# cgbur/llama2.zig

Hardware: AMD Instinct MI355X
Metric: tokens/s (argmax, -t 0) (higher is better)
Workload: dtype f32; 1 GPU; llama2-7b shape, fp32 llama2.c-v0 checkpoint (dim 4096, hidden 11008, L 32, H 32, kv 32, V 32000, S 2048), greedy from BOS, seeded synthetic weights; parallelism=1 GPU

## Files before the change

llama2.zig_amd/csrc/forward.cpp:

```cpp
#include <algorithm>
#include <cmath>
#include <cstdlib>
#include <cstring>
#include <mutex>

#include "batch_host.h"
#include "l2z_state.h"

namespace l2z {

struct Prof {
    std::vector<hipEvent_t> ev;
    std::vector<int> kind;
};

#define L2Z_LAUNCH(kind_id, expr)                                                         \
    do {                                                                                  \
        hipEvent_t _a = nullptr, _b = nullptr;                                            \
        if (prof) {                                                                       \
            L2Z_HIP(hipEventCreate(&_a));                                                 \
            L2Z_HIP(hipEventCreate(&_b));                                                 \
            L2Z_HIP(hipEventRecord(_a, st));                                              \
        }                                                                                 \
        L2Z_HIP(expr);                                                                    \
        if (prof) {                                                                       \
            L2Z_HIP(hipEventRecord(_b, st));                                              \
            prof->ev.push_back(_a);                                                       \
            prof->ev.push_back(_b);                                                       \
            prof->kind.push_back(kind_id);                                                \
        }                                                                                 \
    } while (0)

int check_pair(const l2z_config *config, const l2z_runstate *s, const l2z_weights *w, bool paged_ok, bool q8_ok)
{
    L2Z_CHECK(config && s && w, L2Z_ERR_INVALID, "null config / runstate / weights");
    L2Z_CHECK(q8_ok || !w->is_q8(), L2Z_ERR_INVALID,
              "int8 group-quantized weights (l2z_weights_init_q8) are taken by the single-sequence decode only: "
              "l2z_transformer, l2z_greedy_run, l2z_sample_run, l2z_time_kind, l2z_profile_forward");
    L2Z_CHECK(!w->is_q8() || (s->comm == nullptr && s->sh.world == 1), L2Z_ERR_INVALID,
              "int8 group-quantized weights are unsharded: the runstate belongs to a shard group");
    L2Z_CHECK(paged_ok || s->pool == nullptr, L2Z_ERR_INVALID,
              "a paged runstate (l2z_runstate_init_paged) is taken by the wide family only: l2z_prefill_batch, "
              "l2z_transformer_wide, l2z_wide_run, l2z_verify_wide");
    L2Z_CHECK(memcmp(config, &s->cfg, sizeof *config) == 0 &&
                  memcmp(config, &w->cfg, sizeof *config) == 0,
              L2Z_ERR_INVALID, "config does not match the one RunState / Weights were built with");
    L2Z_CHECK(s->device == w->device && s->sh.rank == w->sh.rank && s->sh.world == w->sh.world,
              L2Z_ERR_INVALID, "RunState and Weights live on different devices / shards");
    L2Z_CHECK(s->sh.scheme_b == w->sh.scheme_b, L2Z_ERR_INVALID,
              "RunState and Weights were built under different sharding schemes (L2Z_SCHEME_B changed in between)");
    return L2Z_OK;
}

namespace {

hipError_t set_state(l2z_runstate *s, const l2z_weights *w, int token, int pos)
{
    if (w->is_q8()) return launch_set_state_q8(token, pos, s->d_token, s->d_pos, w->q8_emb(), s->x, s->cfg.dim, s->stream);
    return launch_set_state(token, pos, s->d_token, s->d_pos, w->tok_emb, s->x, s->cfg.dim, s->stream);
}

int enqueue_forward_q8(l2z_runstate *s, const l2z_weights *w, StepKind step, Prof *prof, int only_stage, int variant,
                       int only_kind)
{
    L2Z_CHECK(only_stage < 0 && s->sh.world == 1, L2Z_ERR_INVALID, "int8 group-quantized weights: unsharded passes only");
    const bool with_step = step != STEP_NONE;
    const bool split = variant == ATTN_SPLIT || variant == ATTN_SPLIT_S;
    const l2z_config &c = s->cfg;
    const Shard &sh = s->sh;
    hipStream_t st = s->stream;
    const size_t dim = c.dim, hid = c.hidden_dim, kvd = sh.kvd_loc;
    const int mb = s->max_blocks, gs = w->q8_gs;
    const size_t gd = dim / gs, gh = hid / gs;
    auto kind = [&](int k) { return only_kind < 0 || only_kind == k; };
    for (int l = 0; l < c.n_layers; l++) {
        float *kc = s->key_cache + (size_t)l * c.seq_len * kvd;
        float *vc = s->value_cache + (size_t)l * c.seq_len * kvd;
        const size_t kvh_stride = (size_t)c.seq_len * sh.hs;
        if (kind(KIND_QKV)) {
            Q8MatvecArgs a = {};
            a.gs = gs;
            a.q0 = w->q_wq.q + (size_t)l * dim * dim; a.s0 = w->q_wq.s + (size_t)l * dim * gd;
            a.q1 = w->q_wk.q + (size_t)l * kvd * dim; a.s1 = w->q_wk.s + (size_t)l * kvd * gd;
            a.q2 = w->q_wv.q + (size_t)l * kvd * dim; a.s2 = w->q_wv.s + (size_t)l * kvd * gd;
            a.b.out0 = s->q; a.b.out1 = kc; a.b.out2 = vc;
            a.b.rows0 = c.dim; a.b.rows1 = sh.kvd_loc; a.b.rows2 = sh.kvd_loc;
            a.b.pos_stride1 = sh.hs; a.b.pos_stride2 = sh.hs; a.b.kv_head_stride = kvh_stride;
            a.b.n = c.dim; a.b.x = s->x; a.b.rms_w = w->rms_att + (size_t)l * dim;
            a.b.pos_ptr = s->d_pos; a.b.rope = s->rope; a.b.head_size = sh.hs; a.b.rope_segs = 2;
            L2Z_LAUNCH(KIND_QKV, launch_q8_matvec(a, EPI_ROPE, mb, g_cus, st));
        }
        if (kind(KIND_ATTN)) {
            AttnArgs a = {};
            a.q = s->q; a.kcache = kc; a.vcache = vc; a.xb = s->xb;
            a.pos_ptr = s->d_pos; a.head_size = sh.hs; a.kv_row = sh.hs; a.kv_head = kvh_stride;
            a.kv_mul = c.n_heads / c.n_kv_heads; a.seq_len = c.seq_len;
            a.tl_seq = s->tl_attn_seq++;
            if (split && s->attn_nch > 1 && attention_split_supported(a))
                L2Z_LAUNCH(KIND_ATTN, launch_attention_split(a, sh.heads_loc, s->attn_nch, s->d_attn_part, s->d_attn_cnt, st,
                                                             variant == ATTN_SPLIT_S));
            else
                L2Z_LAUNCH(KIND_ATTN, launch_attention(a, sh.heads_loc, st, variant == ATTN_SHORT ? 1 : 0));
        }
        if (kind(KIND_WO)) {
            Q8MatvecArgs a = {};
            a.gs = gs;
            a.q0 = w->q_wo.q + (size_t)l * dim * dim; a.s0 = w->q_wo.s + (size_t)l * dim * gd;
            a.b.out0 = s->x; a.b.resid = s->x; a.b.rows0 = c.dim; a.b.n = c.dim; a.b.x = s->xb;
            L2Z_LAUNCH(KIND_WO, launch_q8_matvec(a, EPI_RESID, mb, g_cus, st));
        }
        if (kind(KIND_FFN13)) {
            Q8MatvecArgs a = {};
            a.gs = gs;
            a.q0 = w->q_w13.q + (size_t)l * 2 * hid * dim; a.s0 = w->q_w13.s + (size_t)l * 2 * hid * gd;
            a.b.out0 = s->hb; a.b.rows0 = c.hidden_dim; a.b.rows1 = c.hidden_dim; a.b.n = c.dim; a.b.x = s->x;
            a.b.rms_w = w->rms_ffn + (size_t)l * dim;
            L2Z_LAUNCH(KIND_FFN13, launch_q8_matvec(a, EPI_SWIGLU, mb, g_cus, st));
        }
        if (kind(KIND_FFN2)) {
            Q8MatvecArgs a = {};
            a.gs = gs;
            a.q0 = w->q_w2.q + (size_t)l * dim * hid; a.s0 = w->q_w2.s + (size_t)l * dim * gh;
            a.b.out0 = s->x; a.b.resid = s->x; a.b.rows0 = c.dim; a.b.n = c.hidden_dim; a.b.x = s->hb;
            L2Z_LAUNCH(KIND_FFN2, launch_q8_matvec(a, EPI_RESID, mb, g_cus, st));
        }
    }
    if (kind(KIND_CLS)) {
        Q8MatvecArgs a = {};
        a.gs = gs;
        a.q0 = w->q_cls.q; a.s0 = w->q_cls.s;
        a.b.out0 = s->logits; a.b.rows0 = c.vocab_size; a.b.n = c.dim; a.b.x = s->x; a.b.rms_w = w->rms_final;
        a.b.part_val = s->d_part_val; a.b.part_idx = s->d_part_idx;
        int grid = 0;
        L2Z_LAUNCH(KIND_CLS, launch_q8_matvec(a, EPI_ARGMAX, mb, g_cus, st, &grid));
        s->n_part = grid;
        if (only_kind < 0) (with_step ? s->n_part_step : s->n_part_fwd) = s->n_part;
    }
    if (step == STEP_GREEDY && kind(KIND_ARGMAX)) {
        ArgmaxArgs a = {};
        a.logits = s->logits; a.vocab = c.vocab_size; a.token_ptr = s->d_token;
        if (s->n_part > 0) { a.part_val = s->d_part_val; a.part_idx = s->d_part_idx; a.n_part = s->n_part; }
        a.pos_ptr = s->d_pos; a.prompt = s->d_prompt; a.n_prompt_ptr = s->d_n_prompt;
        a.out_tokens = s->d_out_tokens; a.argmax_out = s->d_argmax; a.emb_q8 = w->q8_emb();
        a.x = s->x; a.dim = c.dim; a.advance = 1;
        L2Z_LAUNCH(KIND_ARGMAX, launch_argmax(a, st));
    }
    if (step == STEP_SAMPLE && kind(KIND_ARGMAX)) {
        L2Z_CHECK(s->d_smp_ctl != nullptr && s->d_smp_scratch != nullptr, L2Z_ERR_STATE,
                  "sampled step on a runstate l2z_sample_run has not prepared");
        SampleStepArgs a = {};
        a.logits = s->logits; a.vocab = c.vocab_size; a.seq_len = c.seq_len;
        a.params = (const SampleStepParams *)s->d_smp_ctl; a.coins = s->d_smp_ctl + 2; a.scratch = s->d_smp_scratch;
        a.token_ptr = s->d_token; a.pos_ptr = s->d_pos; a.prompt = s->d_prompt; a.n_prompt_ptr = s->d_n_prompt;
        a.out_tokens = s->d_out_tokens; a.emb_q8 = w->q8_emb(); a.x = s->x; a.dim = c.dim;
        L2Z_LAUNCH(KIND_ARGMAX, launch_sample_step(a, st));
    }
    return L2Z_OK;
}

}

int enqueue_forward(l2z_runstate *s, const l2z_weights *w, StepKind step, Prof *prof,
                    int only_stage, int variant, int only_kind)
{
    if (w->is_q8()) return enqueue_forward_q8(s, w, step, prof, only_stage, variant, only_kind);
    const bool with_step = step != STEP_NONE;
    const bool split = variant == ATTN_SPLIT || variant == ATTN_SPLIT_S;
    const l2z_config &c = s->cfg;
    const Shard &sh = s->sh;
    hipStream_t st = s->stream;
    const l2z_comm *lc = s->comm;
    const size_t dim = c.dim, hid = c.hidden_dim;
    const int mb = s->max_blocks;
    int stage = 0;
    auto want = [&]() { return only_stage < 0 || only_stage == stage; };
    auto kind = [&](int k) { return only_kind < 0 || only_kind == k; };
    const bool p2p = s->d_push != nullptr && only_stage < 0 && sh.world > 1;
    const bool consume = p2p && s->ll_consume;
    const bool can_push = p2p && consume;
    const bool sb = sh.scheme_b;
    const bool xchg = step == STEP_GREEDY && p2p && s->xchg_steps;
    const int n_g = s->n_gathers;
    int gi = 0;
    bool pushed = false;
    const int *ctl = lc ? lc->d_ctl : nullptr;
    auto gather = [&](float *buf, size_t count_per_rank) -> int {
        stage++;
        gi++;
        if (only_stage >= 0 || only_kind >= 0) return L2Z_OK;
        const bool was_pushed = pushed;
        pushed = false;
        if (consume) {
            L2Z_CHECK(was_pushed, L2Z_ERR_STATE, "consumer-side gather %d: the producer did not push", gi);
            if (gi < n_g) return L2Z_OK;
        }
        hipEvent_t ea = nullptr, eb = nullptr;
        const bool timed = prof != nullptr && s->comm != nullptr && s->comm->world > 1;
        if (timed) {
            L2Z_HIP(hipEventCreate(&ea));
            L2Z_HIP(hipEventCreate(&eb));
            L2Z_HIP(hipEventRecord(ea, st));
        }
        L2Z_TRY(comm_allgather_inplace(s->comm, buf, count_per_rank, gi, n_g, was_pushed, st));
        if (timed) {
            L2Z_HIP(hipEventRecord(eb, st));
            prof->ev.push_back(ea);
            prof->ev.push_back(eb);
            prof->kind.push_back(KIND_GATHER);
        }
        return L2Z_OK;
    };
    auto reduce = [&]() -> int {
        stage++;
        gi++;
        if (only_stage >= 0 || only_kind >= 0) return L2Z_OK;
        const bool was_pushed = pushed;
        pushed = false;
        hipEvent_t ea = nullptr, eb = nullptr;
        if (prof != nullptr) {
            L2Z_HIP(hipEventCreate(&ea));
            L2Z_HIP(hipEventCreate(&eb));
            L2Z_HIP(hipEventRecord(ea, st));
        }
        L2Z_TRY(comm_allreduce(s->comm, s->part, s->x, dim, gi, was_pushed, st));
        if (prof != nullptr) {
            L2Z_HIP(hipEventRecord(eb, st));
            prof->ev.push_back(ea);
            prof->ev.push_back(eb);
            prof->kind.push_back(KIND_GATHER);
        }
        return L2Z_OK;
    };
    auto x_in = [&](MatvecArgs &a, const float *plain, int g, size_t count_per_rank) {
        a.x = plain;
        if (consume && g >= 1) a.xin = comm_ll_in(s->comm, g, count_per_rank);
    };
    auto push_to = [&](MatvecArgs &a, int which) {
        if (!can_push) return;
        a.push = s->d_push + which;
        a.push_ctl = ctl;
        a.push_gi = comm_gi(lc, gi + 1);
    };
    auto col_shard = [&](MatvecArgs &a, const float *wcols, const float *x_loc, int n_pad, int *epi) {
        a.w0 = wcols;
        a.x = x_loc;
        a.n = n_pad;
        a.rows0 = c.dim;
        a.out0 = s->part;
        a.resid = sh.rank == 0 ? s->x : nullptr;
        *epi = sh.rank == 0 ? EPI_RESID : EPI_STORE;
        push_to(a, 1);
    };
    const bool pk = s->packed_w && !sb && sh.world == 1 && !consume;
    const auto pk_slot = [&](int k, int l, int j = 0) -> const l2z_weights::PkMat * {
        return pk && ((s->packed_kinds >> k) & 1) ? w->pk_slot(k, l, j) : nullptr;
    };
    for (int l = 0; l < c.n_layers; l++) {
        float *kc = s->key_cache + (size_t)l * c.seq_len * sh.kvd_loc;
        float *vc = s->value_cache + (size_t)l * c.seq_len * sh.kvd_loc;
        const size_t kvh_stride = (size_t)c.seq_len * sh.hs;
        const bool fused = s->fused_qkv_attn && !split && only_stage < 0;
        if (fused && kind(KIND_QKV)) {
            FusedQkvAttnArgs a = {};
            a.wq = w->wq + (size_t)l * dim * dim;
            a.wk = w->wk + (size_t)l * dim * dim;
            a.wv = w->wv + (size_t)l * dim * dim;
            a.rms_w = w->rms_att + (size_t)l * dim; a.x = s->x; a.q_out = s->q;
            a.kcache = kc; a.vcache = vc; a.xb = s->xb; a.pos_ptr = s->d_pos; a.rope = s->rope;
            a.n = c.dim; a.head_size = sh.hs; a.seq_len = c.seq_len; a.kv_dim = sh.kvd_loc;
            a.kv_row = sh.hs; a.kv_head = kvh_stride;
            L2Z_LAUNCH(KIND_QKV, launch_fused_qkv_attn(a, c.n_heads, st));
        }
        if (!fused && want() && kind(KIND_QKV)) {
            MatvecArgs a = {};
            a.w0 = w->wq + (size_t)l * sh.dim_loc * dim;
            a.w1 = w->wk + (size_t)l * sh.kvd_loc * dim;
            a.w2 = w->wv + (size_t)l * sh.kvd_loc * dim;
            a.out0 = s->q; a.out1 = kc; a.out2 = vc;
            a.rows0 = sh.dim_loc; a.rows1 = sh.kvd_loc; a.rows2 = sh.kvd_loc;
            a.pos_stride1 = sh.hs; a.pos_stride2 = sh.hs; a.kv_head_stride = kvh_stride;
            a.n = c.dim; a.rms_w = w->rms_att + (size_t)l * dim;
            x_in(a, s->x, gi, sh.dim_loc);
            a.pos_ptr = s->d_pos; a.rope = s->rope; a.head_size = sh.hs; a.rope_segs = 2;
            const auto *pq = pk_slot(KIND_QKV, l, 0), *pkk = pk_slot(KIND_QKV, l, 1), *pv = pk_slot(KIND_QKV, l, 2);
            if (pq && pkk && pv) {
                a.pk = pq->p; a.pk_e = pq->e;
                a.pk1 = pkk->p; a.pk_e1 = pkk->e;
                a.pk2 = pv->p; a.pk_e2 = pv->e;
            }
            L2Z_LAUNCH(KIND_QKV, launch_matvec(a, PRO_RMS, EPI_ROPE, mb, g_cus, st));
        }
        if (!fused && want() && kind(KIND_ATTN)) {
            AttnArgs a = {};
            a.q = s->q; a.kcache = kc; a.vcache = vc; a.xb = s->xb + sh.dim0;
            a.pos_ptr = s->d_pos; a.head_size = sh.hs; a.kv_row = sh.hs; a.kv_head = kvh_stride;
            a.kv_mul = c.n_heads / c.n_kv_heads; a.seq_len = c.seq_len;
            a.tl_seq = s->tl_attn_seq++;
            if (!sb && can_push && attention_push_supported(a)) {
                a.push = s->d_push + 0;
                a.push_ctl = ctl;
                a.push_gi = comm_gi(lc, gi + 1);
                pushed = true;
            }
            if (split && s->attn_nch > 1 && attention_split_supported(a))
                L2Z_LAUNCH(KIND_ATTN, launch_attention_split(a, sh.heads_loc, s->attn_nch,
                                                             s->d_attn_part, s->d_attn_cnt, st, variant == ATTN_SPLIT_S));
            else
                L2Z_LAUNCH(KIND_ATTN, launch_attention(a, sh.heads_loc, st, variant == ATTN_SHORT ? 1 : 0));
        }
        if (!sb) L2Z_TRY(gather(s->xb, sh.dim_loc));
        if (want() && kind(KIND_WO)) {
            MatvecArgs a = {};
            int epi = EPI_RESID;
            if (sb) {
                col_shard(a, w->wo + (size_t)l * dim * sh.dimc_pad, s->xb + sh.dim0, sh.dimc_pad, &epi);
            } else {
                a.w0 = w->wo + (size_t)l * sh.dim_loc * dim;
                a.out0 = s->x + sh.dim0; a.resid = s->x + sh.dim0;
                a.rows0 = sh.dim_loc; a.n = c.dim;
                x_in(a, s->xb, gi, sh.dim_loc);
                push_to(a, 1);
                if (const auto *p = pk_slot(KIND_WO, l)) { a.pk = p->p; a.pk_e = p->e; }
            }
            L2Z_LAUNCH(KIND_WO, launch_matvec(a, PRO_NONE, epi, mb, g_cus, st, nullptr, &pushed));
        }
        if (sb) L2Z_TRY(reduce());
        else L2Z_TRY(gather(s->x, sh.dim_loc));
        if (want() && kind(KIND_FFN13)) {
            MatvecArgs a = {};
            a.w0 = w->w1 + (size_t)l * sh.hid_loc * 2 * dim;
            a.w1 = w->w3 + (size_t)l * sh.hid_loc * 2 * dim;
            a.out0 = sb ? s->hb : s->hb + sh.hid0;
            a.rows0 = sh.hid_loc; a.rows1 = sh.hid_loc; a.n = c.dim;
            a.rms_w = w->rms_ffn + (size_t)l * dim;
            x_in(a, s->x, gi, sh.dim_loc);
            if (!sb) push_to(a, 2);
            if (const auto *p = pk_slot(KIND_FFN13, l)) { a.pk = p->p; a.pk_e = p->e; }
            L2Z_LAUNCH(KIND_FFN13, launch_matvec(a, PRO_RMS, EPI_SWIGLU, mb, g_cus, st, nullptr, &pushed));
        }
        if (!sb) L2Z_TRY(gather(s->hb, sh.hid_loc));
        if (want() && kind(KIND_FFN2)) {
            MatvecArgs a = {};
            int epi = EPI_RESID;
            if (sb) {
                col_shard(a, w->w2 + (size_t)l * dim * sh.hidc_pad, s->hb, sh.hidc_pad, &epi);
            } else {
                a.w0 = w->w2 + (size_t)l * sh.dim_loc * hid;
                a.out0 = s->x + sh.dim0; a.resid = s->x + sh.dim0;
                a.rows0 = sh.dim_loc; a.n = c.hidden_dim;
                x_in(a, s->hb, gi, sh.hid_loc);
                push_to(a, 1);
                if (const auto *p = pk_slot(KIND_FFN2, l)) { a.pk = p->p; a.pk_e = p->e; }
            }
            L2Z_LAUNCH(KIND_FFN2, launch_matvec(a, PRO_NONE, epi, mb, g_cus, st, nullptr, &pushed));
        }
        if (sb) L2Z_TRY(reduce());
        else L2Z_TRY(gather(s->x, sh.dim_loc));
    }
    if (want() && kind(KIND_CLS)) {
        MatvecArgs a = {};
        a.w0 = w->wcls; a.out0 = s->logits + sh.v0;
        a.rows0 = sh.v_loc; a.n = c.dim; a.rms_w = w->rms_final;
        x_in(a, s->x, gi, sh.dim_loc);
        a.part_val = s->d_part_val; a.part_idx = s->d_part_idx; a.row_offset = sh.v0;
        const bool fuse = (sh.world == 1 || xchg || (only_kind >= 0 && with_step && s->comm && !s->comm->nccl && !s->comm->p2p)) &&
                          matvec_vector_width(c.dim);
        int grid = 0;
        if (!xchg) push_to(a, 3);
        if (const auto *p = fuse ? pk_slot(KIND_CLS, 0) : nullptr) { a.pk = p->p; a.pk_e = p->e; }
        L2Z_LAUNCH(KIND_CLS, launch_matvec(a, PRO_RMS, fuse ? EPI_ARGMAX : EPI_STORE, mb, g_cus, st,
                                           &grid, &pushed));
        s->n_part = fuse ? grid : 0;
        if (only_stage < 0 && only_kind < 0) (with_step ? s->n_part_step : s->n_part_fwd) = s->n_part;
    }
    if (xchg) {
        stage++;
        gi++;
        pushed = false;
        if (only_kind < 0) s->logits_partial = true;
    } else {
        L2Z_TRY(gather(s->logits, sh.v_loc));
    }
    if (step == STEP_GREEDY && want() && kind(KIND_ARGMAX)) {
        ArgmaxArgs a = {};
        a.logits = s->logits; a.vocab = c.vocab_size; a.token_ptr = s->d_token;
        if (s->n_part > 0) { a.part_val = s->d_part_val; a.part_idx = s->d_part_idx; a.n_part = s->n_part; }
        a.pos_ptr = s->d_pos; a.prompt = s->d_prompt; a.n_prompt_ptr = s->d_n_prompt;
        a.out_tokens = s->d_out_tokens; a.argmax_out = s->d_argmax; a.tok_emb = w->tok_emb;
        a.x = s->x; a.dim = c.dim; a.advance = 1;
        if (xchg && only_kind < 0) {
            a.xchg = s->d_push + 3;
            a.xchg_gi = comm_gi(lc, n_g);
            a.epoch_ctl = lc->d_ctl;
            a.epoch_add = lc->solo ? 0 : n_g;
        }
        L2Z_LAUNCH(KIND_ARGMAX, launch_argmax(a, st));
    }
    if (step == STEP_SAMPLE && want() && kind(KIND_ARGMAX)) {
        L2Z_CHECK(sh.world == 1 && s->d_smp_ctl != nullptr && s->d_smp_scratch != nullptr, L2Z_ERR_STATE,
                  "sampled step on a runstate l2z_sample_run has not prepared");
        SampleStepArgs a = {};
        a.logits = s->logits; a.vocab = c.vocab_size; a.seq_len = c.seq_len;
        a.params = (const SampleStepParams *)s->d_smp_ctl; a.coins = s->d_smp_ctl + 2; a.scratch = s->d_smp_scratch;
        a.token_ptr = s->d_token; a.pos_ptr = s->d_pos; a.prompt = s->d_prompt; a.n_prompt_ptr = s->d_n_prompt;
        a.out_tokens = s->d_out_tokens; a.tok_emb = w->tok_emb; a.x = s->x; a.dim = c.dim;
        L2Z_LAUNCH(KIND_ARGMAX, launch_sample_step(a, st));
    }
    return L2Z_OK;
}

int attn_variant(const l2z_runstate *s, int pos)
{
    if (s->attn_nch > 1 && pos >= s->attn_split_pos) return pos < s->attn_split_wide_pos ? ATTN_SPLIT_S : ATTN_SPLIT;
    return pos < s->attn_short_pos ? ATTN_SHORT : ATTN_HEAD;
}

int build_graph(l2z_runstate *s, const l2z_weights *w, StepKind step, int variant,
                hipGraphExec_t *out)
{
    hipGraph_t graph = nullptr;
    L2Z_HIP(hipStreamBeginCapture(s->stream, hipStreamCaptureModeThreadLocal));
    int rc = enqueue_forward(s, w, step, nullptr, -1, variant);
    hipError_t e = hipStreamEndCapture(s->stream, &graph);
    if (rc != L2Z_OK) {
        if (graph) (void)hipGraphDestroy(graph);
        return rc;
    }
    L2Z_HIP(e);
    e = hipGraphInstantiate(out, graph, nullptr, nullptr, 0);
    (void)hipGraphDestroy(graph);
    L2Z_HIP(e);
    return L2Z_OK;
}

void drop_graphs(l2z_runstate *s)
{
    for (int v = 0; v < ATTN_VARIANTS; v++) {
        if (s->g_forward[v]) { (void)hipGraphExecDestroy(s->g_forward[v]); s->g_forward[v] = nullptr; }
        if (s->g_step[v]) { (void)hipGraphExecDestroy(s->g_step[v]); s->g_step[v] = nullptr; }
        if (s->g_sample[v]) { (void)hipGraphExecDestroy(s->g_sample[v]); s->g_sample[v] = nullptr; }
    }
    s->graph_w_uid = 0;
}

hipGraphExec_t *graph_slot(l2z_runstate *s, StepKind step, int variant)
{
    return step == STEP_SAMPLE ? &s->g_sample[variant] : step == STEP_GREEDY ? &s->g_step[variant] : &s->g_forward[variant];
}

int ensure_graph(l2z_runstate *s, const l2z_weights *w, int variant, StepKind step)
{
    if (!s->use_graphs) return L2Z_OK;
    int rc = L2Z_OK;
    if (s->graph_w_uid != w->uid) {
        drop_graphs(s);
        s->graph_w_uid = w->uid;
        const int edges[] = {0, s->attn_short_pos, s->attn_split_pos, s->attn_split_wide_pos, s->cfg.seq_len};
        bool reach[ATTN_VARIANTS] = {};
        for (int e : edges)
            for (int p = e - 1; p <= e; p++)
                if (p >= 0 && p < s->cfg.seq_len) reach[attn_variant(s, p)] = true;
        for (int v = 0; v < ATTN_VARIANTS && rc == L2Z_OK; v++) {
            if (!reach[v]) continue;
            rc = build_graph(s, w, STEP_NONE, v, &s->g_forward[v]);
            if (rc == L2Z_OK) rc = build_graph(s, w, STEP_GREEDY, v, &s->g_step[v]);
        }
    }
    hipGraphExec_t *slot = graph_slot(s, step, variant);
    if (rc == L2Z_OK && *slot) return L2Z_OK;
    if (rc != L2Z_OK || build_graph(s, w, step, variant, slot) != L2Z_OK) {
        fprintf(stderr, "llama2_hip: hipGraph capture failed (%s); launching eagerly\n", l2z_last_error());
        drop_graphs(s);
        s->use_graphs = false;
        (void)hipGetLastError();
    }
    return L2Z_OK;
}

int run_forward(l2z_runstate *s, const l2z_weights *w, StepKind step, int pos)
{
    const bool with_step = step != STEP_NONE;
    const int variant = attn_variant(s, pos);
    L2Z_CHECK(s->sh.world == 1 || (s->comm && (s->comm->nccl || s->comm->p2p)), L2Z_ERR_STATE,
              "sharded runstate without a transport: connect the group (RCCL id or "
              "l2z_comm_p2p_export/_connect), or drive emulated ranks with l2z_emu_transformer");
    L2Z_TRY(comm_check(s->comm));
    L2Z_TRY(ensure_graph(s, w, variant, step));
    s->logits_partial = step == STEP_GREEDY && s->xchg_steps && s->d_push != nullptr && s->sh.world > 1;
    if (s->use_graphs) {
        s->n_part = with_step ? s->n_part_step : s->n_part_fwd;
        L2Z_HIP(hipGraphLaunch(*graph_slot(s, step, variant), s->stream));
        return L2Z_OK;
    }
    return enqueue_forward(s, w, step, nullptr, -1, variant);
}

int ensure_logits(l2z_runstate *s)
{
    if (!s->logits_partial) return L2Z_OK;
    L2Z_TRY(comm_allgather_inplace(s->comm, s->logits, (size_t)s->sh.v_loc, 1, 1, false, s->stream));
    s->logits_partial = false;
    s->n_part = 0;
    return L2Z_OK;
}


}

using namespace l2z;

extern "C" int l2z_transformer(int token, int pos, const l2z_config *config, l2z_runstate *s,
                               const l2z_weights *w)
{
    L2Z_TRY(check_pair(config, s, w, false, true));
    L2Z_CHECK(token >= 0 && token < config->vocab_size, L2Z_ERR_STATE, "token %d out of range", token);
    L2Z_CHECK(pos >= 0 && pos < config->seq_len, L2Z_ERR_STATE, "pos %d out of range [0,%d)", pos,
              config->seq_len);
    L2Z_HIP(hipSetDevice(s->device));
    L2Z_HIP(set_state(s, w, token, pos));
    L2Z_TRY(run_forward(s, w, STEP_NONE, pos));
    s->host_pos = pos + 1;
    return L2Z_OK;
}

extern "C" int l2z_argmax(l2z_runstate *s, int *out_token)
{
    L2Z_CHECK(s && out_token, L2Z_ERR_INVALID, "l2z_argmax: null argument");
    L2Z_HIP(hipSetDevice(s->device));
    L2Z_TRY(ensure_logits(s));
    ArgmaxArgs a = {};
    a.logits = s->logits; a.vocab = s->cfg.vocab_size; a.argmax_out = s->d_argmax; a.advance = 0;
    if (s->n_part > 0) { a.part_val = s->d_part_val; a.part_idx = s->d_part_idx; a.n_part = s->n_part; }
    L2Z_HIP(launch_argmax(a, s->stream));
    L2Z_HIP(hipMemcpyAsync(out_token, s->d_argmax, sizeof(int), hipMemcpyDeviceToHost, s->stream));
    L2Z_HIP(hipStreamSynchronize(s->stream));
    return L2Z_OK;
}

extern "C" int l2z_logits_read(l2z_runstate *s, float *out_logits)
{
    L2Z_CHECK(s && out_logits, L2Z_ERR_INVALID, "l2z_logits_read: null argument");
    L2Z_HIP(hipSetDevice(s->device));
    L2Z_TRY(ensure_logits(s));
    L2Z_HIP(hipMemcpyAsync(out_logits, s->logits, (size_t)s->cfg.vocab_size * sizeof(float),
                           hipMemcpyDeviceToHost, s->stream));
    L2Z_HIP(hipStreamSynchronize(s->stream));
    L2Z_TRY(comm_check(s->comm));
    return L2Z_OK;
}

extern "C" int l2z_probs_read(l2z_runstate *s, float temperature, float *out_probs)
{
    L2Z_CHECK(s && out_probs, L2Z_ERR_INVALID, "l2z_probs_read: null argument");
    L2Z_CHECK(temperature > 0.0f, L2Z_ERR_INVALID, "l2z_probs_read: temperature %g (0 is the argmax path)", (double)temperature);
    L2Z_HIP(hipSetDevice(s->device));
    L2Z_TRY(ensure_logits(s));
    if (s->d_probs == nullptr) L2Z_HIP(hipMalloc(&s->d_probs, (size_t)s->cfg.vocab_size * sizeof(float)));
    L2Z_HIP(launch_probs(s->d_probs, s->logits, s->cfg.vocab_size, temperature, s->stream));
    const size_t bytes = (size_t)s->cfg.vocab_size * sizeof(float);
    if (s->h_stage == nullptr) L2Z_HIP(hipHostMalloc((void **)&s->h_stage, bytes, hipHostMallocDefault));
    L2Z_HIP(hipMemcpyAsync(s->h_stage, s->d_probs, bytes, hipMemcpyDeviceToHost, s->stream));
    L2Z_HIP(hipStreamSynchronize(s->stream));
    L2Z_TRY(comm_check(s->comm));
    memcpy(out_probs, s->h_stage, bytes);
    return L2Z_OK;
}

extern "C" int l2z_greedy_begin(l2z_runstate *s, const int32_t *prompt, int n_prompt)
{
    L2Z_CHECK(s != nullptr && n_prompt >= 0 && (n_prompt == 0 || prompt != nullptr),
              L2Z_ERR_INVALID, "l2z_greedy_begin: bad arguments");
    L2Z_CHECK(n_prompt <= s->cfg.seq_len, L2Z_ERR_INVALID, "prompt longer than seq_len");
    L2Z_CHECK(s->pool == nullptr, L2Z_ERR_INVALID, "l2z_greedy_begin: a paged runstate is taken by the wide family only");
    for (int i = 0; i < n_prompt; i++)
        L2Z_CHECK(prompt[i] >= 0 && prompt[i] < s->cfg.vocab_size, L2Z_ERR_INVALID,
                  "prompt[%d] = %d out of vocabulary", i, prompt[i]);
    L2Z_HIP(hipSetDevice(s->device));
    L2Z_HIP(hipStreamSynchronize(s->stream));
    if (n_prompt)
        L2Z_HIP(hipMemcpy(s->d_prompt, prompt, (size_t)n_prompt * sizeof(int), hipMemcpyHostToDevice));
    L2Z_HIP(hipMemcpy(s->d_n_prompt, &n_prompt, sizeof(int), hipMemcpyHostToDevice));
    s->h_prompt.assign(prompt, prompt + n_prompt);
    s->host_pos = 0;
    s->done = false;
    return L2Z_OK;
}

namespace l2z {
namespace {

int step_loop(const l2z_config *config, l2z_runstate *s, const l2z_weights *w, int n_steps, StepKind step,
              int32_t *out_tokens, int *out_n)
{
    *out_n = 0;
    L2Z_HIP(hipSetDevice(s->device));
    if (s->done) return L2Z_OK;
    int remaining = n_steps;
    if (remaining > config->seq_len - s->host_pos) remaining = config->seq_len - s->host_pos;
    if (remaining <= 0) return L2Z_OK;
    if (s->host_pos == 0) {
        L2Z_HIP(set_state(s, w, 1, 0));
    }
    const int kChunk = 64;
    int produced = 0;
    const int np = (int)s->h_prompt.size();
    if (s->host_pos == 0 && np >= kPrefillMinPrompt && remaining >= np && prefill_enabled() && !w->is_q8() &&
        prefill_usable(s) &&
        std::find(s->h_prompt.begin(), s->h_prompt.end(), 1) == s->h_prompt.end()) {
        std::vector<int32_t> in((size_t)np);
        in[0] = 1;
        for (int i = 1; i < np; i++) in[(size_t)i] = s->h_prompt[(size_t)i - 1];
        L2Z_TRY(prefill_tokens(s, w, in.data(), np, 0));
        L2Z_HIP(hipMemcpyAsync(s->d_out_tokens, s->d_prompt, (size_t)np * sizeof(int),
                               hipMemcpyDeviceToDevice, s->stream));
        L2Z_HIP(launch_set_state(s->h_prompt[(size_t)np - 1], np, s->d_token, s->d_pos, w->tok_emb,
                                 s->x, config->dim, s->stream));
        for (int i = 0; i < np; i++) out_tokens[i] = s->h_prompt[(size_t)i];
        produced = np;
        s->host_pos = np;
        remaining -= np;
    }
    while (remaining > 0 && !s->done) {
        const int n = remaining < kChunk ? remaining : kChunk;
        for (int i = 0; i < n; i++) L2Z_TRY(run_forward(s, w, step, s->host_pos + i));
        L2Z_HIP(hipMemcpyAsync(out_tokens + produced, s->d_out_tokens + s->host_pos,
                               (size_t)n * sizeof(int), hipMemcpyDeviceToHost, s->stream));
        L2Z_HIP(hipStreamSynchronize(s->stream));
        L2Z_TRY(comm_check(s->comm));
        int got = n;
        for (int i = 0; i < n; i++) {
            if (out_tokens[produced + i] == 1) {
                got = i + 1;
                s->done = true;
                break;
            }
        }
        produced += got;
        s->host_pos += got;
        remaining -= n;
    }
    *out_n = produced;
    return L2Z_OK;
}

}
}

extern "C" int l2z_greedy_run(const l2z_config *config, l2z_runstate *s, const l2z_weights *w,
                              int n_steps, int32_t *out_tokens, int *out_n)
{
    L2Z_TRY(check_pair(config, s, w, false, true));
    L2Z_CHECK(out_tokens && out_n && n_steps >= 0, L2Z_ERR_INVALID, "l2z_greedy_run: bad arguments");
    return step_loop(config, s, w, n_steps, STEP_GREEDY, out_tokens, out_n);
}

extern "C" int l2z_sample_run(const l2z_config *config, l2z_runstate *s, const l2z_weights *w, int n_steps,
                              float temperature, float top_p, const float *coins, int32_t *out_tokens, int *out_n)
{
    L2Z_TRY(no_device_check());
    L2Z_CHECK(out_tokens && out_n && n_steps >= 0, L2Z_ERR_INVALID, "l2z_sample_run: bad arguments");
    L2Z_TRY(check_pair(config, s, w, false, true));
    L2Z_CHECK(s->comm == nullptr && s->sh.world == 1, L2Z_ERR_INVALID,
              "l2z_sample_run: the runstate is a shard (a shard holds its own rows of the logits only)");
    L2Z_TRY(check_draw("l2z_sample_run", -1, temperature, top_p, coins));
    if (temperature > 0.0f) L2Z_TRY(check_coins("l2z_sample_run", coins, 0, n_steps));
    *out_n = 0;
    const int left = config->seq_len - s->host_pos;
    const int n = n_steps < left ? n_steps : left;
    if (s->done || n <= 0) return L2Z_OK;
    L2Z_HIP(hipSetDevice(s->device));
    const size_t ctl_bytes = (2 + (size_t)config->seq_len) * sizeof(float);
    if (s->d_smp_ctl == nullptr) {
        L2Z_HIP(hipMalloc((void **)&s->d_smp_ctl, ctl_bytes));
        L2Z_HIP(hipMemset(s->d_smp_ctl, 0, ctl_bytes));
    }
    if (s->h_smp_ctl == nullptr) L2Z_HIP(hipHostMalloc((void **)&s->h_smp_ctl, ctl_bytes, hipHostMallocDefault));
    if (s->d_smp_scratch == nullptr)
        L2Z_HIP(hipMalloc((void **)&s->d_smp_scratch, sample_scratch_floats(config->vocab_size) * sizeof(float)));
    s->h_smp_ctl[0] = temperature;
    s->h_smp_ctl[1] = top_p;
    L2Z_HIP(hipMemcpyAsync(s->d_smp_ctl, s->h_smp_ctl, 2 * sizeof(float), hipMemcpyHostToDevice, s->stream));
    if (temperature > 0.0f) {
        float *h = s->h_smp_ctl + 2 + s->host_pos;
        memcpy(h, coins, (size_t)n * sizeof(float));
        L2Z_HIP(hipMemcpyAsync(s->d_smp_ctl + 2 + s->host_pos, h, (size_t)n * sizeof(float), hipMemcpyHostToDevice, s->stream));
    }
    return step_loop(config, s, w, n_steps, STEP_SAMPLE, out_tokens, out_n);
}

extern "C" int l2z_profile_forward(int token, int pos, const l2z_config *config, l2z_runstate *s,
                                   const l2z_weights *w, double *ms_by_kind, int *launches_by_kind,
                                   int n_kinds)
{
    L2Z_TRY(check_pair(config, s, w, false, true));
    L2Z_CHECK(ms_by_kind && launches_by_kind && n_kinds >= KIND_COUNT, L2Z_ERR_INVALID,
              "l2z_profile_forward: need %d kind slots", (int)KIND_COUNT);
    L2Z_CHECK(token >= 0 && token < config->vocab_size && pos >= 0 && pos < config->seq_len,
              L2Z_ERR_STATE, "token/pos out of range");
    L2Z_HIP(hipSetDevice(s->device));
    L2Z_HIP(set_state(s, w, token, pos));
    Prof prof;
    int rc = enqueue_forward(s, w, STEP_GREEDY, &prof, -1, attn_variant(s, pos));
    hipError_t e = hipStreamSynchronize(s->stream);
    for (int k = 0; k < n_kinds; k++) { ms_by_kind[k] = 0.0; launches_by_kind[k] = 0; }
    if (rc == L2Z_OK && e == hipSuccess) {
        for (size_t i = 0; i < prof.kind.size(); i++) {
            float ms = 0.0f;
            if (hipEventElapsedTime(&ms, prof.ev[2 * i], prof.ev[2 * i + 1]) == hipSuccess) {
                ms_by_kind[prof.kind[i]] += ms;
                launches_by_kind[prof.kind[i]] += 1;
            }
        }
    }
    for (hipEvent_t ev : prof.ev) (void)hipEventDestroy(ev);
    s->host_pos = pos + 1;
    if (rc != L2Z_OK) return rc;
    L2Z_HIP(e);
    return L2Z_OK;
}

extern "C" int l2z_time_kind(int kind, int pos, const l2z_config *config, l2z_runstate *s,
                             const l2z_weights *w, int reps, double *avg_ms_per_launch, int *launches)
{
    L2Z_TRY(check_pair(config, s, w, false, true));
    L2Z_CHECK(kind >= 0 && kind < KIND_GATHER && avg_ms_per_launch && reps >= 1, L2Z_ERR_INVALID,
              "l2z_time_kind: bad arguments");
    L2Z_CHECK(s->sh.world == 1 || (s->comm && ((!s->comm->nccl && !s->comm->p2p) || s->comm->solo)), L2Z_ERR_INVALID,
              "l2z_time_kind: unsharded runstates, emulated or solo ranks only (a connected shard would wait for its peers)");
    L2Z_CHECK(pos >= 0 && pos < config->seq_len, L2Z_ERR_STATE, "pos out of range");
    L2Z_HIP(hipSetDevice(s->device));
    L2Z_HIP(set_state(s, w, 1, pos));
    hipEvent_t e0, e1;
    L2Z_HIP(hipEventCreate(&e0));
    L2Z_HIP(hipEventCreate(&e1));
    const int per_pass = kind == KIND_CLS || kind == KIND_ARGMAX ? 1 : config->n_layers;
    int rc = enqueue_forward(s, w, STEP_GREEDY, nullptr, -1, attn_variant(s, pos), kind);
    hipError_t e = hipEventRecord(e0, s->stream);
    for (int r = 0; r < reps && rc == L2Z_OK; r++) rc = enqueue_forward(s, w, STEP_GREEDY, nullptr, -1, attn_variant(s, pos), kind);
    if (e == hipSuccess) e = hipEventRecord(e1, s->stream);
    if (e == hipSuccess) e = hipEventSynchronize(e1);
    float ms = 0.0f;
    if (e == hipSuccess) e = hipEventElapsedTime(&ms, e0, e1);
    (void)hipEventDestroy(e0);
    (void)hipEventDestroy(e1);
    hipError_t e2 = set_state(s, w, 1, pos);
    if (e2 == hipSuccess) e2 = hipStreamSynchronize(s->stream);
    if (rc != L2Z_OK) return rc;
    L2Z_HIP(e);
    L2Z_HIP(e2);
    *avg_ms_per_launch = (double)ms / (double)(reps * per_pass);
    if (launches) *launches = reps * per_pass;
    return L2Z_OK;
}

extern "C" int l2z_emu_transformer(int n_ranks, l2z_runstate *const *ss,
                                   const l2z_weights *const *ws, int token, int pos)
{
    L2Z_CHECK(n_ranks >= 1 && ss && ws, L2Z_ERR_INVALID, "l2z_emu_transformer: bad arguments");
    const l2z_config &c = ss[0]->cfg;
    for (int r = 0; r < n_ranks; r++) {
        L2Z_TRY(check_pair(&c, ss[r], ws[r]));
        L2Z_CHECK(ss[r]->sh.world == n_ranks && ss[r]->sh.rank == r, L2Z_ERR_INVALID,
                  "l2z_emu_transformer: runstate %d is not rank %d of %d", r, r, n_ranks);
        L2Z_HIP(launch_set_state(token, pos, ss[r]->d_token, ss[r]->d_pos, ws[r]->tok_emb, ss[r]->x,
                                 c.dim, ss[r]->stream));
    }
    const bool sb = ss[0]->sh.scheme_b;
    const int n_stages = (sb ? 2 : 4) * c.n_layers + 1;
    for (int stage = 0; stage < n_stages; stage++) {
        for (int r = 0; r < n_ranks; r++)
            L2Z_TRY(enqueue_forward(ss[r], ws[r], STEP_NONE, nullptr, stage, attn_variant(ss[r], pos)));
        for (int r = 0; r < n_ranks; r++) L2Z_HIP(hipStreamSynchronize(ss[r]->stream));
        if (sb && stage < n_stages - 1) {
            const float *parts[kMaxWorld];
            L2Z_CHECK(n_ranks <= kMaxWorld, L2Z_ERR_INVALID, "l2z_emu_transformer: more than %d ranks", kMaxWorld);
            for (int r = 0; r < n_ranks; r++) parts[r] = ss[r]->part;
            for (int r = 0; r < n_ranks; r++) L2Z_HIP(launch_sum_parts(ss[r]->x, parts, n_ranks, c.dim, nullptr));
            L2Z_HIP(hipDeviceSynchronize());
            continue;
        }
        const Shard &sh0 = ss[0]->sh;
        size_t count;
        int which;
        if (stage == n_stages - 1) { which = 3; count = sh0.v_loc; }
        else if (stage % 4 == 0) { which = 0; count = sh0.dim_loc; }
        else if (stage % 4 == 2) { which = 2; count = sh0.hid_loc; }
        else { which = 1; count = sh0.dim_loc; }
        auto buf = [&](l2z_runstate *s) {
            return which == 0 ? s->xb : which == 1 ? s->x : which == 2 ? s->hb : s->logits;
        };
        for (int src = 0; src < n_ranks; src++)
            for (int dst = 0; dst < n_ranks; dst++)
                if (dst != src)
                    L2Z_HIP(hipMemcpy(buf(ss[dst]) + (size_t)src * count,
                                      buf(ss[src]) + (size_t)src * count, count * sizeof(float),
                                      hipMemcpyDeviceToDevice));
        L2Z_HIP(hipDeviceSynchronize());
    }
    for (int r = 0; r < n_ranks; r++) ss[r]->host_pos = pos + 1;
    return L2Z_OK;
}

extern "C" int l2z_kind_name(int kind, char *out, size_t cap)
{
    L2Z_CHECK(kind >= 0 && kind < KIND_COUNT && out && cap, L2Z_ERR_INVALID, "l2z_kind_name: bad kind");
    snprintf(out, cap, "%s", kKindNames[kind]);
    return L2Z_OK;
}
```

llama2.zig_amd/csrc/l2z_internal.h:

```cpp
#pragma once

#include <hip/hip_runtime.h>

#include <cstdarg>
#include <cstdint>
#include <cstdio>
#include <string>
#include <vector>

#include "../../include/llama2_hip.h"
#include "../../include/llama2_hip_test.h"

namespace l2z {

struct P2pArgs;

struct LLIn {
    const unsigned long long *slots;
    unsigned slot_floats;
    unsigned count;
    int gi;
    int *ctl;
    int *h_err;
    long long timeout_ticks;
};

void set_error(const char *fmt, ...);

#define L2Z_HIP(expr)                                                                    \
    do {                                                                                 \
        hipError_t _e = (expr);                                                          \
        if (_e != hipSuccess) {                                                          \
            ::l2z::set_error("%s failed: %s (%s:%d)", #expr, hipGetErrorString(_e),      \
                             __FILE__, __LINE__);                                        \
            return _e == hipErrorOutOfMemory ? L2Z_ERR_OOM                               \
                   : (_e == hipErrorNoDevice || _e == hipErrorInvalidDevice)             \
                       ? L2Z_ERR_NO_DEVICE                                               \
                       : L2Z_ERR_HIP;                                                    \
        }                                                                                \
    } while (0)

#define L2Z_CHECK(cond, code, ...)          \
    do {                                    \
        if (!(cond)) {                      \
            ::l2z::set_error(__VA_ARGS__);  \
            return (code);                  \
        }                                   \
    } while (0)

#define L2Z_TRY(expr)              \
    do {                           \
        int _s = (expr);           \
        if (_s != L2Z_OK) return _s; \
    } while (0)

template <class Sig> class FnRef;
template <class R, class... Args> class FnRef<R(Args...)> {
  public:
    template <class F>
    FnRef(const F &f) : f_(&f), call_([](const void *p, Args... args) -> R { return (*(const F *)p)(args...); }) {}
    R operator()(Args... args) const { return call_(f_, args...); }

  private:
    const void *f_;
    R (*call_)(const void *, Args...);
};


enum Prologue { PRO_NONE = 0, PRO_RMS = 1 };
enum Epilogue { EPI_STORE = 0, EPI_ROPE = 1, EPI_RESID = 2, EPI_SWIGLU = 3, EPI_ARGMAX = 4 };

constexpr int kMaxSeg = 3;

struct Q8Emb {
    const int8_t *q;
    const float *s;
    int gs;
};

struct ArgmaxArgs {
    const float *logits;
    int vocab;
    const float *part_val;
    const int *part_idx;
    int n_part;
    int *token_ptr;
    int *pos_ptr;
    const int *prompt;
    const int *n_prompt_ptr;
    int *out_tokens;
    int *argmax_out;
    const float *tok_emb;
    float *x;
    int dim;
    Q8Emb emb_q8;
    int advance;
    int *epoch_ctl;
    int epoch_add;
    const P2pArgs *xchg;
    int xchg_gi;
};

struct MatvecArgs {
    const float *w0, *w1, *w2;
    float *out0, *out1, *out2;
    int rows0, rows1, rows2;
    int pos_stride1, pos_stride2;
    size_t kv_head_stride;
    int n;
    const float *x;
    const float *rms_w;
    const float *resid;
    const int *pos_ptr;
    const float2 *rope;
    int head_size;
    int rope_segs;
    float *part_val;
    int *part_idx;
    int row_offset;
    const P2pArgs *push;
    const int *push_ctl;
    int push_gi;
    LLIn xin;
    const uint32_t *pk, *pk1, *pk2;
    int pk_e, pk_e1, pk_e2;
    int tl_slot;
};

struct Q8MatvecArgs {
    MatvecArgs b;
    const int8_t *q0, *q1, *q2;
    const float *s0, *s1, *s2;
    int gs;
    const int8_t *xq;
    const float *xs;
};
hipError_t launch_q8_matvec(const Q8MatvecArgs &a, int epi, int max_blocks_per_cu, int n_cus, hipStream_t st,
                            int *out_grid = nullptr);
hipError_t launch_q8_quantize(const float *src, size_t count, int gs, bool weight_rule, int8_t *q, float *s, hipStream_t st);
hipError_t launch_set_state_q8(int token, int pos, int *token_ptr, int *pos_ptr, const Q8Emb &emb, float *x, int dim,
                               hipStream_t st);

struct AttnArgs {
    const float *q;
    const float *kcache;
    const float *vcache;
    float *xb;
    const int *pos_ptr;
    int head_size;
    int kv_row;
    size_t kv_head;
    int kv_mul;
    int seq_len;
    const P2pArgs *push;
    const int *push_ctl;
    int push_gi;
    int tl_seq;
};


struct FusedQkvAttnArgs {
    const float *wq, *wk, *wv;
    const float *rms_w, *x;
    float *q_out;
    float *kcache, *vcache;
    float *xb;
    const int *pos_ptr;
    const float2 *rope;
    int n;
    int head_size, seq_len, kv_dim;
    int kv_row;
    size_t kv_head;
};
bool fused_qkv_attn_supported(int dim, int n_heads, int n_kv_heads, int seq_len, int n_cus);
hipError_t launch_fused_qkv_attn(const FusedQkvAttnArgs &a, int n_heads, hipStream_t st);

hipError_t launch_pk_stats(const float *m, size_t count, uint32_t *stats, hipStream_t st);
hipError_t launch_pk_pack(const float *m, int rows, int n, int e_base, uint32_t *pk, hipStream_t st);
hipError_t launch_pk_unpack(const uint32_t *pk, int rows, int n, int e_base, float *out, hipStream_t st);
hipError_t launch_matvec(const MatvecArgs &a, int pro, int epi, int max_blocks_per_cu, int n_cus,
                         hipStream_t st, int *out_grid = nullptr, bool *pushed = nullptr);
bool attention_push_supported(const AttnArgs &a);
int matvec_max_grid(int n_cus);
bool matvec_vector_width(int n);
hipError_t launch_stream_read(const float *p, size_t n_floats, float *out, int n_cus, hipStream_t st);
hipError_t launch_attention(const AttnArgs &a, int n_heads_local, hipStream_t st, int form = 0);
int attention_short_pos(int head_size, int seq_len);
int attention_split_chunks(int n_heads_local, int n_cus);
size_t attention_split_part_floats(int n_heads_local, int head_size, int nch);
bool attention_split_supported(const AttnArgs &a);
hipError_t launch_attention_split(const AttnArgs &a, int n_heads_local, int nch, float *part,
                                  int *arrivals, hipStream_t st, bool small = false);
int attention_split_wide_pos(int seq_len);
hipError_t launch_argmax(const ArgmaxArgs &a, hipStream_t st);
hipError_t launch_set_state(int token, int pos, int *token_ptr, int *pos_ptr, const float *tok_emb,
                            float *x, int dim, hipStream_t st);
hipError_t launch_rmsnorm(float *o, const float *x, const float *w, int n, hipStream_t st);
hipError_t launch_softmax(float *x, int n, hipStream_t st);
hipError_t launch_probs(float *probs, const float *logits, int n, float temperature, hipStream_t st);
hipError_t launch_dot(float *out, const float *x, const float *y, int n, hipStream_t st);
hipError_t launch_weighted_sum_rows(float *xout, int xout_len, const float *rows, int row_stride,
                                    const float *weights, int n_weights, hipStream_t st);
hipError_t launch_synth_fill(float *dst, uint64_t base_idx, uint64_t count, uint64_t seed,
                             float scale, float bias, hipStream_t st, uint64_t row_len = 0, uint64_t row_pitch = 0,
                             uint64_t idx_pitch = 0);
hipError_t launch_sum_parts(float *out, const float *const *parts, int n_parts, int n, hipStream_t st);
hipError_t launch_copy_rows(float *dst, size_t dpitch, const float *src, size_t rows, size_t cols, hipStream_t st);
size_t attention_lds_bytes(int head_size, int seq_len, bool vec);

struct SplitKWs {
    float *part;
    int *cnt;
    size_t part_floats;
    int cnt_ints;
    void *x3;
    size_t x3_bytes;
    void *x3b;
    size_t x3b_bytes;
};
struct DeferredSum {
    const float *part;
    int sk, feat, tm;
    bool valid;
};
enum PlanesReady { PLANES_SPLIT = 0, PLANES_READY = 1, PLANES_READY_B = 2 };
constexpr int kSplitKMaxTokens = 256;
constexpr int kPanelWsRows = 6 * kSplitKMaxTokens;
int prefill_split_k(long long n_whole, int P, int K, bool pair);
enum PrefillGemmEpi { PG_STORE = 0, PG_RESID = 1, PG_ROPE = 2, PG_ROPE_CACHE = 3, PG_CACHE = 4,
                      PG_SWIGLU = 5 };
bool x3_applies(long long n_whole, int K);
bool x3_stream_shape(long long n_whole, int P, int K);
int x3_stream_sk(long long n_whole, int P, int K);
enum GemmKind { GEMM_SINGLE = 0,
                GEMM_QKV,
                GEMM_W13,
                GEMM_KV };
struct GemmShape {
    int kind, epi;
    int P, N, K, ldx;
    int n_scale;
    long long n_launch_whole;
    int sk;
    int nq, nkv;
    int w13_one_matrix;
    size_t part_floats;
    int cnt_ints;
};
enum GemmFamily { GF_INVALID = -1, GF_NOT_SUPPORTED = -2, GF_NO_WORKSPACE = -3,
                  GF_STREAM = 1,
                  GF_SHORT,
                  GF_SPLIT_K,
                  GF_TWO_BLOCK,
                  GF_TILE };
enum TileForm { TILE_128x64 = 0, TILE_64x64, TILE_32x64, TILE_32x32, TILE_128x128 };
struct GemmPlan {
    int family;
    int epi;
    int K;
    int x3;
    int sk;
    int tile;
    int feat, tm, nbuf, one_round;
    int tms, paired;
};
GemmPlan prefill_gemm_plan(const GemmShape &s);
hipError_t launch_prefill_rmsnorm(float *o, int ldo, const float *x, const float *w, int n, int P,
                                  hipStream_t st,
                                  void *x3 = nullptr, int kp = 0,
                                  const DeferredSum *pending = nullptr,
                                  const int *rows = nullptr);
hipError_t launch_prefill_embed(float *x, const float *tok_emb, const int *tokens, int dim, int P,
                                hipStream_t st);
hipError_t launch_prefill_attention(const float *q, int ldq, const float *kcache, const float *vcache,
                                    float *out, int ldo, int pos0, int P, int n_heads, int head_size,
                                    int kv_row, size_t kv_head, int kv_mul, int seq_len, hipStream_t st,
                                    int n_heads_model = 0,
                                    int form = 0,
                                    void *x3 = nullptr, int kp = 0,
                                    bool *planes_written = nullptr);
constexpr int kRaggedMaxSeq = 16;
struct RaggedSeq {
    float *kc, *vc;
    int row0, rows;
    int pos0;
    int pad;
    const int32_t *pages;
};
__device__ __forceinline__ int kv_page_id(const int32_t *pages, int i)
{
    return ((const __attribute__((address_space(4))) int32_t *)pages)[i];
}
struct RaggedLayer {
    const float *q;
    int ldq;
    float *out;
    int ldo;
    int P, n_heads, head_size, kv_mul, seq_len;
    size_t layer_off, kv_head_stride;
    hipStream_t st;
    void *x3;
    int kp;
};
using RaggedAttention = FnRef<hipError_t(const RaggedLayer &, bool *planes_written)>;
struct RaggedChunk {
    const RaggedSeq *seq;
    const int *row_seq;
    const int *row_pos;
    const int2 *tiles;
    int n_seq, n_tiles;
    int seq_max;
    float *k, *v;
    size_t page_floats;
    const RaggedAttention *attention;
    const int *att_rows;
    int n_att_rows;
};
hipError_t launch_ragged_rope_scatter(float *q, int ldq, const RaggedChunk &rg, int P, int dim, int kv_dim, int head_size,
                                      const float2 *rope, size_t layer_off, size_t kv_head_stride, hipStream_t st);
hipError_t launch_ragged_attention(const RaggedLayer &L, const RaggedChunk &rg, bool *planes_written = nullptr);
enum PanelEpi { PANEL_STORE = 0, PANEL_RESID = 1, PANEL_SWIGLU = 2, PANEL_QKV = 3 };
struct PanelProduct {
    const float *x;
    int ldx;
    const float *w0, *w1, *w2;
    int rows0, rows1, rows2;
    int P, K;
    int mode;
    float *out;
    int ldo;
    const float *res;
    int ldres;
    float *outk, *outv;
    int ldkv, head_size, pos0;
    size_t kv_head_stride;
    const float2 *rope;
};
bool prefill_panel_shape(long long n_whole, int P, int K, long long widest_whole);
int prefill_panel_max_tokens();
int prefill_next_chunk_of(const l2z_config &c, int remaining);
hipError_t launch_prefill_panel(const PanelProduct &p, int n_cus, const SplitKWs *ws, hipStream_t st);
int prefill_tile_form(int N, int P, int pair);
constexpr int kScoreSeg = 4096;
struct ScoreArgs {
    const float *slab;
    int ld, n, col0, P;
    const int *targets;
    float *part_m, *part_s;
    int *part_i;
    float *tgt;
    int seg0, nseg;
    float *out_logprob;
    int *out_top1;
};
hipError_t launch_score_reduce(const ScoreArgs &a, hipStream_t st);
hipError_t launch_score_finish(const ScoreArgs &a, hipStream_t st);
size_t matvec_lds_bytes(int n);

}
```

llama2.zig_amd/csrc/l2z_state.h:

```cpp
#pragma once
#include <cstdint>
#include <vector>

#include "kv_pages.h"
#include "l2z_comm.h"
#include "l2z_internal.h"
#include "tunables.h"

namespace l2z {

struct BatchScratch;
struct WideScratch;

struct Shard {
    int rank = 0, world = 1;
    int hs = 0;
    int dim0 = 0, dim_loc = 0;
    int kvd_loc = 0;
    int heads_loc = 0;
    int hid0 = 0, hid_loc = 0;
    int v0 = 0, v_loc = 0;
    bool scheme_b = false;
    int dimc_pad = 0, hidc_pad = 0;
};
int pad_cols(int n);
int make_shard(const l2z_config &c, const l2z_comm *comm, Shard *out);

enum ShardKind { REPL, BY_Q_HEADS, BY_KV_HEADS, BY_HIDDEN, BY_DIM_ROWS, BY_VOCAB, SKIP };

struct TensorDesc {
    const char *name;
    size_t offset;
    size_t layers, rows, cols;
    ShardKind kind;
    float scale, bias;
    size_t count() const { return layers * rows * cols; }
};
std::vector<TensorDesc> tensor_table(const l2z_config &c, bool shared);
void shard_rows(const TensorDesc &d, const Shard &s, size_t *r0, size_t *r1);

extern int g_cus;
int ensure_device(int device);
int current_device_for(const l2z_comm *comm);

}

enum { KIND_QKV = 0, KIND_ATTN, KIND_WO, KIND_FFN13, KIND_FFN2, KIND_CLS, KIND_ARGMAX, KIND_GATHER, KIND_COUNT };

struct l2z_weights {
    uint64_t uid = 0;
    l2z_config cfg;
    int shared;
    int device;
    l2z::Shard sh;
    float *blob = nullptr;
    size_t blob_floats = 0;
    bool file_layout = false;
    std::vector<size_t> dev_off;
    const float *tok_emb = nullptr, *rms_att = nullptr, *rms_ffn = nullptr, *rms_final = nullptr;
    const float *wq = nullptr, *wk = nullptr, *wv = nullptr, *wo = nullptr;
    const float *w1 = nullptr, *w2 = nullptr, *w3 = nullptr, *wcls = nullptr;
    struct PkMat {
        const uint32_t *p = nullptr;
        int e = 0;
        const float *src = nullptr;
        int rows = 0, cols = 0;
    };
    struct PkKind {
        uint32_t *blob = nullptr;
        std::vector<PkMat> slots;
        int per_layer = 0;
        int packed = 0;
    };
    PkKind pk[KIND_COUNT];
    struct Q8Mat {
        const int8_t *q = nullptr;
        const float *s = nullptr;
    };
    int q8_gs = 0;
    uint8_t *q8_blob = nullptr;
    Q8Mat q_emb, q_wq, q_wk, q_wv, q_wo, q_w13, q_w2, q_cls;
    bool is_q8() const { return q8_gs != 0; }
    l2z::Q8Emb q8_emb() const { return l2z::Q8Emb{q_emb.q, q_emb.s, q8_gs}; }
    const PkMat *pk_slot(int kind, int layer, int j = 0) const
    {
        const PkKind &k = pk[kind];
        const size_t i = (size_t)layer * k.per_layer + j;
        return k.blob != nullptr && i < k.slots.size() && k.slots[i].p != nullptr ? &k.slots[i] : nullptr;
    }
};

struct l2z_kvpool {
    l2z_config cfg;
    int device = 0;
    l2z::KvPages alloc;
    float *k = nullptr, *v = nullptr;
    size_t page_floats = 0;
    int live = 0;
};

static const char *const kKindNames[KIND_COUNT] = {"qkv", "attn", "wo", "ffn13", "ffn2", "cls", "argmax", "gather"};
static_assert(KIND_COUNT == L2Z_N_KINDS, "include/llama2_hip_test.h L2Z_N_KINDS");

struct l2z_runstate {
    l2z_config cfg;
    int device;
    l2z::Shard sh;
    const l2z_comm *comm = nullptr;
    hipStream_t stream = nullptr;
    float *x = nullptr, *xb = nullptr, *hb = nullptr, *q = nullptr, *logits = nullptr;
    float *part = nullptr;
    float *key_cache = nullptr, *value_cache = nullptr;
    l2z_kvpool *pool = nullptr;
    l2z::KvSeq pg;
    int32_t *d_pages = nullptr, *h_pages = nullptr;
    bool pages_dirty = false;
    float2 *rope = nullptr;
    int *d_token = nullptr, *d_pos = nullptr, *d_prompt = nullptr, *d_n_prompt = nullptr;
    int *d_out_tokens = nullptr, *d_argmax = nullptr;
    float *pf_x = nullptr, *pf_xn = nullptr, *pf_q = nullptr, *pf_att = nullptr;
    float *pf_h1 = nullptr;
    int pf_ld_xn = 0, pf_ld_att = 0, pf_ld_h1 = 0;
    float *pf_stage = nullptr;
    float *pf_part = nullptr;
    int *pf_tokens = nullptr;
    l2z::DeferredSum pf_pending = {nullptr, 1, 128, 1, false};
    l2z::PlanesReady pf_planes_att = l2z::PLANES_SPLIT, pf_planes_h1 = l2z::PLANES_SPLIT;
    l2z::SplitKWs pf_sk = {nullptr, nullptr, 0, 0, nullptr, 0, nullptr, 0};
    int pf_cap = 0;
    void *sc_ws = nullptr, *sc_seq = nullptr;
    size_t sc_ws_bytes = 0;
    int sc_cap = 0, sc_slab_n = 0;
    int sc_slab_force = 0;
    float *d_probs = nullptr;
    float *h_stage = nullptr;
    float *d_smp_ctl = nullptr, *h_smp_ctl = nullptr, *d_smp_scratch = nullptr;
    float *d_part_val = nullptr;
    int *d_part_idx = nullptr;
    int n_part = 0;
    int n_part_step = 0, n_part_fwd = 0;
    float *d_attn_part = nullptr;
    int *d_attn_cnt = nullptr;
    int attn_nch = 0;
    int attn_split_pos = 0;
    int attn_short_pos = 0;
    int attn_split_wide_pos = 0;
    uint64_t graph_w_uid = 0;
    hipGraphExec_t g_forward[4] = {nullptr, nullptr, nullptr, nullptr}, g_step[4] = {nullptr, nullptr, nullptr, nullptr};
    hipGraphExec_t g_sample[4] = {nullptr, nullptr, nullptr, nullptr};
    bool use_graphs = true;
    int host_pos = 0;
    bool done = false;
    std::vector<int32_t> h_prompt;
    l2z::P2pArgs *d_push = nullptr;
    int n_gathers = 0;
    bool ll_consume = false;
    bool xchg_steps = false;
    bool logits_partial = false;
    bool fused_qkv_attn = false;
    int max_blocks = 0;
    bool packed_w = true;
    int packed_kinds = -1;
    int tl_attn_seq = 0;
    l2z::BatchScratch *bt = nullptr;
    float *rg_k = nullptr, *rg_v = nullptr;
    void *rg_tab = nullptr;
    int rg_cap = 0;
    l2z::WideScratch *wd = nullptr;
};

namespace l2z {

struct Prof;
int check_pair(const l2z_config *config, const l2z_runstate *s, const l2z_weights *w, bool paged_ok = false,
               bool q8_ok = false);
enum { ATTN_SHORT = 0, ATTN_HEAD = 1, ATTN_SPLIT_S = 2, ATTN_SPLIT = 3, ATTN_VARIANTS = 4 };
enum StepKind { STEP_NONE = 0, STEP_GREEDY = 1, STEP_SAMPLE = 2 };
int enqueue_forward(l2z_runstate *s, const l2z_weights *w, StepKind step, Prof *prof, int only_stage,
                    int variant, int only_kind = -1);
int attn_variant(const l2z_runstate *s, int pos);
int run_forward(l2z_runstate *s, const l2z_weights *w, StepKind step, int pos);
int ensure_logits(l2z_runstate *s);
void drop_graphs(l2z_runstate *s);

constexpr int kPrefillMinPrompt = L2Z_PREFILL_MIN_PROMPT;
bool prefill_enabled();
bool prefill_usable(const l2z_runstate *s);
bool prefill_shard_takes_the_unsharded_kernels(const l2z_config &c, const Shard &sh);
int prefill_check(const l2z_config *config, const l2z_runstate *s);
struct ScoreCall;
int prefill_tokens(l2z_runstate *s, const l2z_weights *w, const int32_t *tokens, int n_tokens, int pos0,
                   const ScoreCall *score = nullptr);

int prefill_scratch(l2z_runstate *s, int need);
int prefill_ragged_chunk(l2z_runstate *s, const l2z_weights *w, const int32_t *tokens, int P, const RaggedChunk &rg);
int prefill_last_logits(l2z_runstate *s, const l2z_weights *w);
int prefill_rows_logits(l2z_runstate *s, const l2z_weights *w, int P, float *out, int ldo, const int *rows = nullptr);
int ragged_alloc(l2z_runstate *s, int need);

int kv_check_kind(const char *fn, int n, l2z_runstate *const *states);
int kv_attach(const char *fn, int n, l2z_runstate *const *states, const int32_t *pos0, const int32_t *counts, int count);
int kv_upload(int n, l2z_runstate *const *states, hipStream_t st);
void kv_seq_base(const l2z_runstate *s, RaggedSeq *q);
inline size_t kv_page_floats(const l2z_runstate *s) { return s->pool != nullptr ? s->pool->page_floats : 0; }
int kv_release(l2z_runstate *s, int n_pos);
int kv_copy_rows(l2z_runstate *dst, const l2z_runstate *src, int r0, int n_pos);
void kv_runstate_free(l2z_runstate *s);

void batch_free(l2z_runstate *s);
void wide_free(l2z_runstate *s);
const float *wide_verify_row(const l2z_runstate *s, int row);
void wide_verify_forget(l2z_runstate *s);

}
```

llama2.zig_amd/csrc/matvec.hip:

```cpp
#include <type_traits>

#include "argmax_rule.h"
#include "matvec_device.h"
#include "packed_w.h"

namespace l2z {
namespace {

__device__ __forceinline__ void dot2_scalar(const float *__restrict__ pa,
                                            const float *__restrict__ pb, const float *xs, int n,
                                            float &ra, float &rb)
{
    const int lane = threadIdx.x & 63;
    float sa = 0.0f, sb = 0.0f;
    for (int j = lane; j < n; j += kWave) {
        const float xv = xs[j];
        sa = fmaf(pa[j], xv, sa);
        sb = fmaf(pb[j], xv, sb);
    }
    ra = wave_sum(sa);
    rb = wave_sum(sb);
}

template <int LPR>
struct MvGeom {
    static constexpr int RW = kWave / LPR;
    static constexpr int U = (LPR == 64) ? 4 : 6;
};

template <int LPR>
__device__ __forceinline__ void mv_load(const float *pa, const float *pb, int c0, int n4,
                                        v4f (&wa)[MvGeom<LPR>::U], v4f (&wb)[MvGeom<LPR>::U])
{
    constexpr int U = MvGeom<LPR>::U;
    const v4f *a4 = (const v4f *)pa, *b4 = (const v4f *)pb;
#pragma unroll
    for (int k = 0; k < U; k++) {
        int c = c0 + LPR * k;
        c = c < n4 ? c : n4 - 1;
        wa[k] = ldg_nt(a4 + c);
        wb[k] = ldg_nt(b4 + c);
    }
}

template <int LPR>
__device__ __forceinline__ void mv_consume(const v4f *xs4, int c0, const v4f (&wa)[MvGeom<LPR>::U],
                                           const v4f (&wb)[MvGeom<LPR>::U], v4f &acc_a, v4f &acc_b)
{
    constexpr int U = MvGeom<LPR>::U;
#pragma unroll
    for (int k = 0; k < U; k++) {
        const v4f xv = xs4[c0 + LPR * k];
        acc_a = fma4(wa[k], xv, acc_a);
        acc_b = fma4(wb[k], xv, acc_b);
    }
}

struct MvStep {
    bool unit_done, more;
    int u_next, b_next;
};

__device__ __forceinline__ MvStep mv_step(int u, int b, int n_batches, int ustride, int n_units)
{
    MvStep s;
    s.unit_done = (b + 1 == n_batches);
    s.u_next = s.unit_done ? u + ustride : u;
    s.b_next = s.unit_done ? 0 : b + 1;
    s.more = s.u_next < n_units;
    return s;
}

template <int PRO, int EPI, int LPR, int XC, bool LL>
__global__ __launch_bounds__(kBlock) void matvec_kernel(const MatvecArgs a)
{
    using G = MvGeom<LPR>;
    constexpr int U = G::U, RW = G::RW;
    extern __shared__ __attribute__((aligned(16))) float lds[];
    const MvLocals m = mv_locals<EPI>(a);
    const int n4 = m.n >> 2;
    const int n_batches = (n4 + LPR * U - 1) / (LPR * U);
    const int n4_pad = n_batches * (LPR * U);
    float *xs = lds;
    float *scratch = lds + 4 * n4_pad;
    const v4f *xs4 = (const v4f *)xs;

    const int lane = threadIdx.x & 63, wave = threadIdx.x >> 6;
    const int grp = lane / LPR, cl = lane % LPR;
    const int n_units = (m.n_pairs + RW - 1) / RW;
    const int ustride = gridDim.x * kWaves;

    XStage<PRO, XC, LL> xst;
    xst.issue(a.x, a.xin, a.rms_w, n4);
    int u = blockIdx.x * kWaves + wave;
    const bool has_unit = u < n_units;
    const float *pa, *pb;
    pair_rows<EPI>(m, (has_unit ? u : 0) * RW + grp, pa, pb);
    v4f wa[U], wb[U];
    EpiIn ein = epi_prefetch<EPI>(m, (has_unit ? u : 0) * RW + grp, cl == 0 && has_unit);
    EpiIn ein_next = ein;
    mv_load<LPR>(pa, pb, cl, n4, wa, wb);
    xst.finish(a.x, a.rms_w, m.n, n4_pad, xs, scratch);
    if (EPI != EPI_ARGMAX && !has_unit) return;

    v4f acc_a = {0.f, 0.f, 0.f, 0.f}, acc_b = {0.f, 0.f, 0.f, 0.f};
    ArgmaxCand best;
    int b = 0;
    while (has_unit) {
        mv_consume<LPR>(xs4, cl + b * (LPR * U), wa, wb, acc_a, acc_b);
        const MvStep s = mv_step(u, b, n_batches, ustride, n_units);
        if (s.more) {
            if (s.unit_done) {
                pair_rows<EPI>(m, s.u_next * RW + grp, pa, pb);
                ein_next = epi_prefetch<EPI>(m, s.u_next * RW + grp, cl == 0);
            }
            mv_load<LPR>(pa, pb, cl + s.b_next * (LPR * U), n4, wa, wb);
        }
        if (s.unit_done) {
            const float sa = lanes_sum(hsum4(acc_a), LPR);
            const float sb = lanes_sum(hsum4(acc_b), LPR);
            pair_epilogue<EPI>(m, u * RW + grp, sa, sb, cl == 0, ein);
            ein = ein_next;
            if (EPI == EPI_ARGMAX) {
                const int ra_ = 2 * (u * RW + grp), rb_ = ra_ + 1;
                if (ra_ < m.total_rows) argmax_take(best, sa, ra_ + a.row_offset);
                if (rb_ < m.total_rows) argmax_take(best, sb, rb_ + a.row_offset);
            }
            acc_a = v4f{0.f, 0.f, 0.f, 0.f};
            acc_b = v4f{0.f, 0.f, 0.f, 0.f};
        }
        if (!s.more) break;
        u = s.u_next;
        b = s.b_next;
    }
    if (EPI == EPI_ARGMAX) {
        argmax_wave_fold(best);
        __syncthreads();
        if (lane == 0) {
            scratch[wave] = best.v;
            scratch[kWaves + wave] = __int_as_float(best.i);
        }
        __syncthreads();
        if (threadIdx.x == 0) {
            ArgmaxCand c = {scratch[0], __float_as_int(scratch[kWaves])};
            for (int w = 1; w < kWaves; w++) argmax_merge(c, scratch[w], __float_as_int(scratch[kWaves + w]));
            a.part_val[blockIdx.x] = c.v;
            a.part_idx[blockIdx.x] = c.i;
        }
    }
}

struct PkRaw {
    v4u q4[7];
    uint32_t q1[3];
};

__device__ __forceinline__ void pk_load_raw(const uint32_t *src, int lane, int s, PkRaw &r)
{
    const int q = pk::lane_dw(s) / 4, rem = pk::lane_dw(s) % 4;
#pragma unroll
    for (int i = 0; i < 7; i++)
        if (i < q) r.q4[i] = __builtin_nontemporal_load((const v4u *)(src + i * 256 + lane * 4));
#pragma unroll
    for (int i = 0; i < 3; i++)
        if (i < rem) r.q1[i] = __builtin_nontemporal_load(src + q * 256 + i * 64 + lane);
}

template <int S>
__device__ __forceinline__ void pk_decode_lane(const PkRaw &r, int e31, v4f (&wa)[4], v4f (&wb)[4])
{
    constexpr int N = pk::lane_dw(S), Q = N / 4;
    uint32_t d[N > 0 ? N : 1], t[8 * S > 0 ? 8 * S : 1];
#pragma unroll
    for (int i = 0; i < N; i++) {
        if (i < 4 * Q) {
            const v4u v = r.q4[i / 4];
            d[i] = (i % 4 == 0) ? v.x : (i % 4 == 1) ? v.y : (i % 4 == 2) ? v.z : v.w;
        } else {
            d[i] = r.q1[i - 4 * Q];
        }
    }
    pk::decode_lane_t<S>(d, t);
#pragma unroll
    for (int k = 0; k < 4; k++) {
        if (k < S) {
            wa[k] = v4f{__builtin_amdgcn_ldexpf(__uint_as_float(t[8 * k]), e31), __builtin_amdgcn_ldexpf(__uint_as_float(t[8 * k + 1]), e31),
                        __builtin_amdgcn_ldexpf(__uint_as_float(t[8 * k + 2]), e31), __builtin_amdgcn_ldexpf(__uint_as_float(t[8 * k + 3]), e31)};
            wb[k] = v4f{__builtin_amdgcn_ldexpf(__uint_as_float(t[8 * k + 4]), e31), __builtin_amdgcn_ldexpf(__uint_as_float(t[8 * k + 5]), e31),
                        __builtin_amdgcn_ldexpf(__uint_as_float(t[8 * k + 6]), e31), __builtin_amdgcn_ldexpf(__uint_as_float(t[8 * k + 7]), e31)};
        } else {
            wa[k] = v4f{0.f, 0.f, 0.f, 0.f};
            wb[k] = v4f{0.f, 0.f, 0.f, 0.f};
        }
    }
}

constexpr int kRowU = 4;

template <int EPI, int XC>
struct RowF32 {
    static constexpr int kSets = 1;
    v4f wa[kRowU], wb[kRowU];
    const float *pa, *pb;
    int n4;

    __device__ __forceinline__ void init(const MvLocals &, int n4_, int) { n4 = n4_; }
    __device__ __forceinline__ void point(const MvLocals &m, int u) { pair_rows<EPI>(m, u, pa, pb); }
    template <int P>
    __device__ __forceinline__ void issue(int b)
    {
        const int tid = threadIdx.x, cb = b * (kBlock * kRowU);
        const v4f *a4 = (const v4f *)pa + cb + tid, *b4 = (const v4f *)pb + cb + tid;
        const int wbase = cb + (tid & ~63);
#pragma unroll
        for (int k = 0; k < kRowU; k++) {
            const bool in_row = wbase + kBlock * k < n4;
            if (XC == 12 && !in_row) {
                wa[k] = v4f{0.f, 0.f, 0.f, 0.f};
                wb[k] = v4f{0.f, 0.f, 0.f, 0.f};
                continue;
            }
            const int off = in_row ? kBlock * k : -(cb + (tid & ~63));
            wa[k] = ldg_nt(a4 + off);
            wb[k] = ldg_nt(b4 + off);
        }
    }
    template <int P>
    __device__ __forceinline__ void deliver() {}
};

template <int EPI, int XC>
struct RowPacked {
    static constexpr int kSets = 2;
    v4f wa[kRowU], wb[kRowU];
    PkRaw raw[kSets];
    int s_in[kSets], e31[kSets];
    const uint32_t *pp;
    size_t pdw, last_off;
    int e_pt, s_last, wave_u, n_batches;

    __device__ __forceinline__ void init(const MvLocals &, int n4, int n_batches_)
    {
        n_batches = n_batches_;
        wave_u = __builtin_amdgcn_readfirstlane(threadIdx.x >> 6);
        pdw = pk::pair_dw(n4);
        last_off = pk::chunk_off(n4, n_batches - 1, wave_u);
        s_last = pk::steps(n4, n_batches - 1, wave_u);
    }
    __device__ __forceinline__ void point(const MvLocals &m, int u)
    {
        int e;
        pp = pair_packed<EPI>(m, u, pdw, e);
        e_pt = e - 31;
    }
    template <int P>
    __device__ __forceinline__ void issue(int b)
    {
        const bool last = b + 1 == n_batches;
        const uint32_t *src = pp + (last ? last_off : (size_t)b * (4 * 64 * pk::kMaxLaneDw) + (size_t)wave_u * (64 * pk::kMaxLaneDw));
        s_in[P] = (XC == 4 || !last) ? 4 : s_last;
        e31[P] = e_pt;
        pk_load_raw(src, threadIdx.x & 63, XC == 4 ? 4 : s_in[P], raw[P]);
    }
    template <int P>
    __device__ __forceinline__ void deliver()
    {
        if constexpr (XC == 4) {
            pk_decode_lane<4>(raw[P], e31[P], wa, wb);
        } else {
            switch (s_in[P]) {
                case 4: pk_decode_lane<4>(raw[P], e31[P], wa, wb); break;
                case 3: pk_decode_lane<3>(raw[P], e31[P], wa, wb); break;
                case 2: pk_decode_lane<2>(raw[P], e31[P], wa, wb); break;
                case 1: pk_decode_lane<1>(raw[P], e31[P], wa, wb); break;
                default: pk_decode_lane<0>(raw[P], e31[P], wa, wb); break;
            }
        }
    }
};

#ifdef L2Z_TIMELINE
constexpr int kMtlSlots = 256, kMtlBlocks = 512;
__device__ long long g_mtl[kMtlSlots * kMtlBlocks * 8];
unsigned long long g_mtl_launches = 0;
#define L2Z_MTL(i) tl[i] = wall_clock64()
#else
#define L2Z_MTL(i) do { } while (0)
#endif

template <int PRO, int EPI, int XC, bool LL, bool PK = false>
__global__ __launch_bounds__(kBlock) void matvec_row_kernel(const MatvecArgs a)
{
    constexpr int U = kRowU;
    using Src = typename std::conditional<PK, RowPacked<EPI, XC>, RowF32<EPI, XC>>::type;
    constexpr int NS = Src::kSets;
    extern __shared__ __attribute__((aligned(16))) float lds[];
#ifdef L2Z_TIMELINE
    long long tl[8] = {0, 0, 0, 0, 0, 0, 0, 0};
#endif
    L2Z_MTL(0);
    MvLocals m_ = mv_locals<EPI>(a);
    if constexpr (PK) m_.push = nullptr;
    const MvLocals m = m_;
    const int n4 = m.n >> 2;
    const int n_batches = (n4 + kBlock * U - 1) / (kBlock * U);
    const int n4_pad = n_batches * (kBlock * U);
    float *xs = lds;
    float *scratch = lds + 4 * n4_pad;
    float *part = scratch + kScratch;
    const v4f *xs4 = (const v4f *)xs;
    const int tid = threadIdx.x, lane = tid & 63, wave = tid >> 6;
    const int n_units = m.n_pairs;
    const int ustride = gridDim.x;

    XStage<PRO, XC, LL> xst;
    xst.issue(a.x, a.xin, a.rms_w, n4);
    int u = blockIdx.x;
    Src src;
    src.init(m, n4, n_batches);
    src.point(m, u);
    EpiIn ein = epi_prefetch<EPI>(m, u, tid == 0);
    EpiIn ein_next = ein;
    src.template issue<0>(0);
    L2Z_MTL(1);
    xst.finish(a.x, a.rms_w, m.n, n4_pad, xs, scratch);
    L2Z_MTL(2);

    int iu = u, ib = 0;
    bool imore = true;
    auto advance = [&]() __attribute__((always_inline)) {
        const MvStep s = mv_step(iu, ib, n_batches, ustride, n_units);
        imore = s.more;
        if (s.more) {
            if (s.unit_done) src.point(m, s.u_next);
            iu = s.u_next;
            ib = s.b_next;
        }
    };
    advance();

    v4f acc_a = {0.f, 0.f, 0.f, 0.f}, acc_b = {0.f, 0.f, 0.f, 0.f};
    ArgmaxCand best;
    int b = 0, parity = 0;
    auto step = [&](auto set, auto ahead) __attribute__((always_inline)) -> bool {
        constexpr int P = decltype(set)::value;
        const MvStep s = mv_step(u, b, n_batches, ustride, n_units);
        auto prefetch_next = [&]() __attribute__((always_inline)) {
            if (s.more && s.unit_done) ein_next = epi_prefetch<EPI>(m, s.u_next, tid == 0);
        };
        if constexpr (NS > 1) {
            prefetch_next();
            if constexpr (decltype(ahead)::value) {
                if constexpr (EPI == EPI_SWIGLU) asm volatile("s_waitcnt vmcnt(0)" ::: "memory");
                src.template issue<(P + 1) % NS>(ib);
                advance();
            }
        }
        src.template deliver<P>();
#pragma unroll
        for (int k = 0; k < U; k++) {
            const v4f xv = xs4[b * (kBlock * U) + tid + kBlock * k];
            acc_a = fma4(src.wa[k], xv, acc_a);
            acc_b = fma4(src.wb[k], xv, acc_b);
        }
        if constexpr (NS == 1) {
            prefetch_next();
            if (imore) {
                src.template issue<0>(ib);
                advance();
            }
        }
#ifdef L2Z_TIMELINE
        tl[6]++;
#endif
        if (s.unit_done) {
            const float sa = wave_sum(hsum4(acc_a));
            const float sb = wave_sum(hsum4(acc_b));
            float *pp_ = part + parity * (2 * kWaves);
            if (lane == 0) {
                pp_[wave] = sa;
                pp_[kWaves + wave] = sb;
            }
            __syncthreads();
            if (tid == 0) {
                const float ta = ((pp_[0] + pp_[1]) + pp_[2]) + pp_[3];
                const float tb = ((pp_[kWaves] + pp_[kWaves + 1]) + pp_[kWaves + 2]) + pp_[kWaves + 3];
                pair_epilogue<EPI>(m, u, ta, tb, true, ein);
                if (EPI == EPI_ARGMAX) {
                    const int ra_ = 2 * u, rb_ = ra_ + 1;
                    argmax_take(best, ta, ra_ + a.row_offset);
                    if (rb_ < m.total_rows) argmax_take(best, tb, rb_ + a.row_offset);
                }
            }
            ein = ein_next;
            parity ^= 1;
            acc_a = v4f{0.f, 0.f, 0.f, 0.f};
            acc_b = v4f{0.f, 0.f, 0.f, 0.f};
#ifdef L2Z_TIMELINE
            if (tl[7]++ == 0) L2Z_MTL(3);
            L2Z_MTL(4);
#endif
        }
        u = s.u_next;
        b = s.b_next;
        return !s.more;
    };
    using Set0 = std::integral_constant<int, 0>;
    using Set1 = std::integral_constant<int, 1>;
    static_assert(NS == 1 || NS == 2, "register sets of a source");
    if constexpr (NS == 1) {
        while (!step(Set0{}, std::false_type{})) {}
    } else {
        while (true) {
            if (!imore) { step(Set0{}, std::false_type{}); break; }
            step(Set0{}, std::true_type{});
            if (!imore) { step(Set1{}, std::false_type{}); break; }
            step(Set1{}, std::true_type{});
        }
    }
    if (EPI == EPI_ARGMAX && tid == 0) {
        a.part_val[blockIdx.x] = best.v;
        a.part_idx[blockIdx.x] = best.i;
    }
#ifdef L2Z_TIMELINE
    L2Z_MTL(5);
    if (tid == 0 && (unsigned)a.tl_slot < (unsigned)kMtlSlots && blockIdx.x < kMtlBlocks) {
        long long *o = g_mtl + ((size_t)a.tl_slot * kMtlBlocks + blockIdx.x) * 8;
        for (int i = 0; i < 8; i++) o[i] = tl[i];
    }
#endif
}

template <int PRO, int EPI>
__global__ __launch_bounds__(kBlock) void matvec_scalar_kernel(const MatvecArgs a)
{
    extern __shared__ __attribute__((aligned(16))) float lds[];
    const MvLocals m = mv_locals<EPI>(a);
    float *xs = lds;
    float *scratch = lds + ((m.n + 3) & ~3);
    stage_x_scalar<PRO>(a.x, a.rms_w, m.n, xs, scratch);
    const int lane = threadIdx.x & 63, wave = threadIdx.x >> 6;
    for (int u = blockIdx.x * kWaves + wave; u < m.n_pairs; u += gridDim.x * kWaves) {
        const float *pa, *pb;
        pair_rows<EPI>(m, u, pa, pb);
        float sa, sb;
        dot2_scalar(pa, pb, xs, m.n, sa, sb);
        pair_epilogue<EPI>(m, u, sa, sb, lane == 0, epi_prefetch<EPI>(m, u, lane == 0));
    }
}

int lpr_for(int n4)
{
    int l = 8;
    while (l < 64 && l * 6 < n4) l <<= 1;
    return l;
}

struct MvLaunch {
    const void *fn;
    int lpr, u;
};

template <int PRO, int EPI, int LPR, int XC, bool LL>
MvLaunch mv_entry()
{
    return {reinterpret_cast<const void *>(&matvec_kernel<PRO, EPI, LPR, XC, LL>), LPR, MvGeom<LPR>::U};
}

template <int PRO, int EPI, bool LL>
MvLaunch mv_pick(int lpr, bool big_x)
{
    if (lpr == 8) return mv_entry<PRO, EPI, 8, 4, LL>();
    if (lpr == 16) return mv_entry<PRO, EPI, 16, 4, LL>();
    if (lpr == 32) return mv_entry<PRO, EPI, 32, 4, LL>();
    return big_x ? mv_entry<PRO, EPI, 64, 12, LL>() : mv_entry<PRO, EPI, 64, 4, LL>();
}

template <int PRO, int EPI, bool LL, bool PK = false>
const void *mv_row_fn(bool big_x)
{
    return big_x ? reinterpret_cast<const void *>(&matvec_row_kernel<PRO, EPI, 12, LL, PK>)
                 : reinterpret_cast<const void *>(&matvec_row_kernel<PRO, EPI, 4, LL, PK>);
}

#define L2Z_MV_COMBOS(X)                     \
    X(PRO_NONE, EPI_STORE,  0, 1, 0)         \
    X(PRO_NONE, EPI_RESID,  1, 1, 1)         \
    X(PRO_RMS,  EPI_STORE,  1, 1, 0)         \
    X(PRO_RMS,  EPI_ROPE,   1, 1, 1)         \
    X(PRO_RMS,  EPI_SWIGLU, 1, 1, 1)         \
    X(PRO_RMS,  EPI_ARGMAX, 1, 0, 1)
#define L2Z_IF_1(...) __VA_ARGS__
#define L2Z_IF_0(...)

const void *mv_row_pick_packed(int pro, int epi, bool big_x)
{
#define X(P, E, LL, SC, PK) L2Z_IF_##PK(if (pro == P && epi == E) return mv_row_fn<P, E, false, true>(big_x);)
    L2Z_MV_COMBOS(X)
#undef X
    return nullptr;
}

const void *mv_row_pick(int pro, int epi, bool big_x, bool ll)
{
#define X(P, E, LL, SC, PK)                                           \
    if (pro == P && epi == E && !ll) return mv_row_fn<P, E, false>(big_x); \
    L2Z_IF_##LL(if (pro == P && epi == E && ll) return mv_row_fn<P, E, true>(big_x);)
    L2Z_MV_COMBOS(X)
#undef X
    return nullptr;
}

MvLaunch mv_pick_pe(int pro, int epi, int lpr, bool big_x, bool vec, bool ll)
{
#define X(P, E, LL, SC, PK)                                                                \
    if (pro == P && epi == E && vec && !ll) return mv_pick<P, E, false>(lpr, big_x);       \
    L2Z_IF_##LL(if (pro == P && epi == E && vec && ll) return mv_pick<P, E, true>(lpr, big_x);) \
    L2Z_IF_##SC(if (pro == P && epi == E && !vec && !ll)                                   \
                    return MvLaunch{reinterpret_cast<const void *>(&matvec_scalar_kernel<P, E>), 0, 0};)
    L2Z_MV_COMBOS(X)
#undef X
    return {nullptr, 0, 0};
}
#undef L2Z_MV_COMBOS
#undef L2Z_IF_1
#undef L2Z_IF_0

__global__ __launch_bounds__(256) void stream_read_kernel(const v4f *__restrict__ p, size_t n4, float *out)
{
    constexpr int U = 8;
    size_t i = (size_t)blockIdx.x * 256 * U + threadIdx.x;
    const size_t stride = (size_t)gridDim.x * 256 * U;
    v4f acc = {0.f, 0.f, 0.f, 0.f};
    for (; i + 256 * (U - 1) < n4; i += stride) {
        v4f r[U];
#pragma unroll
        for (int k = 0; k < U; k++) r[k] = ldg_nt(p + i + 256 * k);
#pragma unroll
        for (int k = 0; k < U; k++) acc += r[k];
    }
    const float s = (acc.x + acc.y) + (acc.z + acc.w);
    if (s == 123.456f) out[blockIdx.x] = s;
}

}

size_t matvec_lds_bytes(int n) { return (size_t)(4 * ((n >> 2) + 1024) + kScratch + 4 * kWaves + 4) * sizeof(float); }

int matvec_max_grid(int n_cus) { return n_cus * 8; }

bool matvec_vector_width(int n) { return n > 0 && (n % 4) == 0; }

hipError_t launch_stream_read(const float *p, size_t n_floats, float *out, int n_cus, hipStream_t st)
{
    hipLaunchKernelGGL(stream_read_kernel, dim3(n_cus * 8), dim3(256), 0, st, (const v4f *)p, n_floats / 4, out);
    return hipGetLastError();
}

hipError_t launch_matvec(const MatvecArgs &a_in, int pro, int epi, int max_blocks_per_cu, int n_cus,
                         hipStream_t st, int *out_grid, bool *pushed)
{
    MatvecArgs a = a_in;
    if (max_blocks_per_cu > 8) max_blocks_per_cu = 8;
    bool vec = (a.n % 4) == 0 && aligned16(a.x) && aligned16(a.w0);
    if (a.rows1 > 0) vec = vec && aligned16(a.w1);
    if (a.rows2 > 0) vec = vec && aligned16(a.w2);
    if (pro == PRO_RMS) vec = vec && aligned16(a.rms_w);
    if (epi == EPI_SWIGLU && a.rows1 != a.rows0) return hipErrorInvalidValue;
    const int total_rows = a.rows0 + a.rows1 + a.rows2;
    const int n_pairs = (epi == EPI_SWIGLU) ? a.rows0 : (total_rows + 1) / 2;
    if (n_pairs <= 0 || a.n <= 0) return hipErrorInvalidValue;
    const int n4 = a.n >> 2;
    const int lpr = lpr_for(n4);
    if (epi == EPI_ARGMAX && (!vec || a.rows1 != 0 || a.rows2 != 0)) return hipErrorNotSupported;
    const Tunables &tn = tunables();
    const bool use_row = vec && n4 >= 1024 && (n4 % 64) == 0;
    const bool ll = a.xin.slots != nullptr;
    if (ll && !vec) return hipErrorNotSupported;
    if (a.pk != nullptr && (!use_row || ll || !pk::width_ok(a.n))) return hipErrorInvalidValue;
    if (a.pk != nullptr) a.push = nullptr;
    if (a.pk != nullptr && epi != EPI_SWIGLU &&
        ((a.rows1 > 0 && a.pk1 == nullptr) || (a.rows2 > 0 && a.pk2 == nullptr) || a.rows0 % 2 || a.rows1 % 2 || a.rows2 % 2))
        return hipErrorInvalidValue;
    MvLaunch k = {nullptr, 0, 0};
    size_t lds;
    int n_units;
    const auto padded = [n4](int batch) { return ((n4 + batch - 1) / batch) * batch; };
    if (use_row) {
        k.fn = a.pk != nullptr ? mv_row_pick_packed(pro, epi, a.n > 4096) : mv_row_pick(pro, epi, a.n > 4096, ll);
        lds = (size_t)(4 * padded(kBlock * kRowU) + kScratch + 4 * kWaves) * sizeof(float);
        n_units = n_pairs;
    } else if (vec) {
        k = mv_pick_pe(pro, epi, lpr, a.n > 4096, true, ll);
        if (k.fn == nullptr) return hipErrorInvalidValue;
        lds = (size_t)(4 * padded(k.lpr * k.u) + kScratch) * sizeof(float);
        const int rw = kWave / k.lpr;
        n_units = (n_pairs + rw - 1) / rw;
    } else {
        k = mv_pick_pe(pro, epi, lpr, a.n > 4096, false, ll);
        lds = (size_t)(((a.n + 3) & ~3) + kScratch) * sizeof(float);
        n_units = n_pairs;
    }
    if (k.fn == nullptr) return hipErrorInvalidValue;
    if (lds > 64 * 1024) {
        hipError_t e = hipFuncSetAttribute(k.fn, hipFuncAttributeMaxDynamicSharedMemorySize, (int)lds);
        if (e != hipSuccess) return e;
    }
    int occ = 0;
    if (hipOccupancyMaxActiveBlocksPerMultiprocessor(&occ, k.fn, kBlock, lds) != hipSuccess || occ < 1)
        occ = 1;
    if (occ > max_blocks_per_cu) occ = max_blocks_per_cu;
    if (use_row && occ > tn.row_blocks) occ = tn.row_blocks;
    int resident = occ * n_cus;
    if (tn.grid_cap > 0 && resident > tn.grid_cap) resident = tn.grid_cap;
    int grid;
    if (use_row) {
        grid = n_units;
        if (grid > resident) {
            const int per_block = (n_units + resident - 1) / resident;
            grid = (n_units + per_block - 1) / per_block;
        }
    } else {
        const int blocks_needed = (n_units + kWaves - 1) / kWaves;
        grid = blocks_needed;
        if (grid > resident) {
            const int per_wave = (n_units + resident * kWaves - 1) / (resident * kWaves);
            grid = (n_units + per_wave * kWaves - 1) / (per_wave * kWaves);
        }
    }
    if (out_grid) *out_grid = grid;
    if (!vec || epi == EPI_ROPE || a.rows2 != 0 || (epi != EPI_SWIGLU && a.rows1 != 0)) a.push = nullptr;
    if (pushed) *pushed = a.push != nullptr;
#ifdef L2Z_TIMELINE
    a.tl_slot = use_row ? (int)(g_mtl_launches++ % kMtlSlots) : -1;
#endif
    void *args[] = {&a};
    return hipLaunchKernel(k.fn, dim3(grid), dim3(kBlock), args, lds, st);
}

}

#ifdef L2Z_TIMELINE
extern "C" int l2z_matvec_timeline_dump(long long *out, unsigned long long *n_launches)
{
    if (hipDeviceSynchronize() != hipSuccess) return 1;
    if (hipMemcpyFromSymbol(out, HIP_SYMBOL(l2z::g_mtl), sizeof(long long) * l2z::kMtlSlots * l2z::kMtlBlocks * 8) != hipSuccess) return 1;
    *n_launches = l2z::g_mtl_launches;
    return 0;
}
#endif
```

llama2.zig_amd/csrc/matvec_device.h:

```cpp
#pragma once
#include "kernel_common.h"

namespace l2z {
namespace {

struct MvLocals {
    const float *w0, *w1, *w2;
    float *out0, *out1, *out2;
    const float *resid;
    const float2 *rope;
    int rows0, r01, total_rows, n_pairs, n, head_size, rope_segs, pos;
    size_t ps1, ps2;
    size_t kv_head_stride;
    const P2pArgs *push;
    int push_e;
    size_t push_base;
    const uint32_t *pk, *pk1, *pk2;
    int pk_e, pk_e1, pk_e2;
};

template <int EPI>
__device__ __forceinline__ MvLocals mv_locals(const MatvecArgs &a)
{
    MvLocals m;
    m.w0 = a.w0; m.w1 = a.w1; m.w2 = a.w2;
    m.out0 = a.out0; m.out1 = a.out1; m.out2 = a.out2;
    m.resid = a.resid; m.rope = a.rope;
    m.rows0 = a.rows0; m.r01 = a.rows0 + a.rows1; m.total_rows = a.rows0 + a.rows1 + a.rows2;
    m.n_pairs = (EPI == EPI_SWIGLU) ? a.rows0 : (m.total_rows + 1) >> 1;
    m.n = a.n; m.head_size = a.head_size; m.rope_segs = a.rope_segs;
    m.pos = (EPI == EPI_ROPE) ? *a.pos_ptr : 0;
    m.ps1 = (size_t)m.pos * (size_t)a.pos_stride1;
    m.ps2 = (size_t)m.pos * (size_t)a.pos_stride2;
    m.kv_head_stride = (EPI == EPI_ROPE) ? a.kv_head_stride : 0;
    m.push = a.push;
    m.push_e = m.push ? a.push_ctl[kCtlEpoch] + a.push_gi : 0;
    m.push_base = m.push ? (size_t)m.push->rank * m.push->count : 0;
    m.pk = a.pk; m.pk1 = a.pk1; m.pk2 = a.pk2;
    m.pk_e = a.pk_e; m.pk_e1 = a.pk_e1; m.pk_e2 = a.pk_e2;
    return m;
}

struct SegRow {
    bool past0, past1;
    int row;
    __device__ __forceinline__ int seg() const { return past1 ? 2 : (past0 ? 1 : 0); }
    template <typename T>
    __device__ __forceinline__ T pick(T v0, T v1, T v2) const
    {
        const T v = past0 ? v1 : v0;
        return past1 ? v2 : v;
    }
};

__device__ __forceinline__ SegRow seg_row(const MvLocals &m, int g)
{
    SegRow r;
    r.past0 = g >= m.rows0;
    r.past1 = g >= m.r01;
    r.row = g - (r.past1 ? m.r01 : (r.past0 ? m.rows0 : 0));
    return r;
}

template <int EPI>
__device__ __forceinline__ void pair_rows(const MvLocals &m, int p, const float *&pa, const float *&pb)
{
    if (p >= m.n_pairs) p = m.n_pairs - 1;
    if (EPI == EPI_SWIGLU) {
        pa = m.w0 + (size_t)(2 * p) * (size_t)m.n;
        pb = pa + m.n;
    } else {
        const int ga = 2 * p;
        const int gb = (ga + 1 < m.total_rows) ? ga + 1 : ga;
        const SegRow ra = seg_row(m, ga), rb = seg_row(m, gb);
        pa = ra.pick(m.w0, m.w1, m.w2) + (size_t)ra.row * (size_t)m.n;
        pb = rb.pick(m.w0, m.w1, m.w2) + (size_t)rb.row * (size_t)m.n;
    }
}

template <int EPI>
__device__ __forceinline__ const uint32_t *pair_packed(const MvLocals &m, int p, size_t pair_dw, int &e_base)
{
    if (p >= m.n_pairs) p = m.n_pairs - 1;
    if (EPI == EPI_ROPE) {
        const SegRow r = seg_row(m, 2 * p);
        e_base = r.pick(m.pk_e, m.pk_e1, m.pk_e2);
        return r.pick(m.pk, m.pk1, m.pk2) + (size_t)(r.row >> 1) * pair_dw;
    }
    e_base = m.pk_e;
    return m.pk + (size_t)p * pair_dw;
}

struct EpiIn {
    float ra, rb;
    float2 cs;
};

template <int EPI>
__device__ __forceinline__ EpiIn epi_prefetch(const MvLocals &m, int p, bool writer)
{
    EpiIn e;
    e.ra = 0.0f; e.rb = 0.0f; e.cs = make_float2(1.0f, 0.0f);
    if (!writer || p >= m.n_pairs) return e;
    if (EPI == EPI_RESID) {
        const int ga = 2 * p, gb = ga + 1;
        e.ra = m.resid[ga];
        if (gb < m.total_rows) e.rb = m.resid[gb];
    } else if (EPI == EPI_ROPE) {
        const SegRow ra = seg_row(m, 2 * p);
        if (ra.seg() < m.rope_segs) {
            const int hs = m.head_size;
            e.cs = m.rope[(size_t)m.pos * (size_t)(hs >> 1) + (size_t)((ra.row % hs) >> 1)];
        }
    }
    return e;
}

template <int EPI>
__device__ __forceinline__ void pair_epilogue(const MvLocals &m, int p, float sa, float sb, bool writer, const EpiIn &in)
{
    const bool valid_a = p < m.n_pairs;
    if (EPI == EPI_SWIGLU) {
        float v = sa;
        v = v * (1.0f / (1.0f + expf(-v)));
        v = v * sb;
        if (writer && valid_a) {
            m.out0[p] = v;
            if (m.push) p2p_ll_push(m.push, m.push_e, m.push_base + (size_t)p, v);
        }
        return;
    }
    const int ga = 2 * p, gb = ga + 1;
    const bool valid_b = valid_a && gb < m.total_rows;
    const SegRow ra = seg_row(m, ga), rb = seg_row(m, gb);
    const int row_a = ra.row, row_b = rb.row;
    float *oa = ra.pick(m.out0, m.out1 + m.ps1, m.out2 + m.ps2);
    float *ob = rb.pick(m.out0, m.out1 + m.ps1, m.out2 + m.ps2);
    if (EPI == EPI_ROPE) {
        float o0 = sa, o1 = sb;
        if (ra.seg() < m.rope_segs) {
            const float2 cs = in.cs;
            o0 = sa * cs.x - sb * cs.y;
            o1 = sa * cs.y + sb * cs.x;
        }
        if (writer && valid_a) {
            size_t ia = (size_t)row_a, ib = (size_t)row_b;
            if (m.kv_head_stride) {
                const int hs = m.head_size;
                if (ra.past0) ia = (size_t)(row_a / hs) * m.kv_head_stride + (size_t)(row_a % hs);
                if (rb.past0) ib = (size_t)(row_b / hs) * m.kv_head_stride + (size_t)(row_b % hs);
            }
            oa[ia] = o0;
            if (valid_b) ob[ib] = o1;
        }
    } else if (EPI == EPI_RESID) {
        if (writer && valid_a) {
            const float va = in.ra + sa, vb = in.rb + sb;
            oa[row_a] = va;
            if (valid_b) ob[row_b] = vb;
            if (m.push) {
                p2p_ll_push(m.push, m.push_e, m.push_base + (size_t)row_a, va);
                if (valid_b) p2p_ll_push(m.push, m.push_e, m.push_base + (size_t)row_b, vb);
            }
        }
    } else {
        if (writer && valid_a) {
            oa[row_a] = sa;
            if (valid_b) ob[row_b] = sb;
            if (m.push) {
                p2p_ll_push(m.push, m.push_e, m.push_base + (size_t)row_a, sa);
                if (valid_b) p2p_ll_push(m.push, m.push_e, m.push_base + (size_t)row_b, sb);
            }
        }
    }
}

}
}
```

llama2.zig_amd/csrc/packed_w.h:

```cpp
#pragma once
#include <cstddef>
#include <cstdint>

#ifndef __HIPCC__
#define __host__
#define __device__
#endif

namespace l2z {
namespace pk {

constexpr int kMaxLaneDw = 29;
constexpr int kBatchF4 = 1024;

__host__ __device__ constexpr int lane_dw(int s) { return (29 * s + 3) / 4; }
__host__ __device__ constexpr int plane_off(int s, int i, int lane)
{
    return i < lane_dw(s) / 4 * 4 ? (i / 4) * 256 + lane * 4 + i % 4 : lane_dw(s) / 4 * 256 + (i - lane_dw(s) / 4 * 4) * 64 + lane;
}

__host__ __device__ inline int steps(int n4, int b, int w)
{
    int s = 0;
    for (int k = 0; k < 4; k++) s += (b * kBatchF4 + 64 * w + 256 * k < n4) ? 1 : 0;
    return s;
}

__host__ __device__ inline size_t chunk_off(int n4, int b, int w)
{
    size_t o = (size_t)b * 4 * 64 * kMaxLaneDw;
    for (int v = 0; v < w; v++) o += (size_t)64 * lane_dw(steps(n4, b, v));
    return o;
}

__host__ __device__ inline size_t pair_dw(int n4)
{
    const int nb = (n4 + kBatchF4 - 1) / kBatchF4;
    return chunk_off(n4, nb - 1, 4);
}

__host__ __device__ constexpr bool width_ok(int n) { return n % 256 == 0 && n >= 4096; }

__host__ __device__ inline uint32_t encode_t(uint32_t v, int e_base)
{
    const uint32_t e = (v >> 23) & 0xffu;
    const uint32_t c = e == 0 ? 0u : e - (uint32_t)(e_base - 31);
    return (v & 0x807fffffu) | (c << 23);
}

__host__ __device__ inline bool encodable(uint32_t max_e, uint32_t min_e, uint32_t bad)
{
    return bad == 0 && (max_e == 0 || min_e + 30 >= max_e);
}

template <int S>
__host__ __device__ inline void encode_lane(const uint32_t *v, int e_base, uint32_t *d)
{
    constexpr int N = lane_dw(S), X = 8 * S - N;
#pragma unroll
    for (int i = 0; i < N; i++) d[i] = encode_t(v[i], e_base);
#pragma unroll
    for (int x = 0; x < X; x++) {
        const uint32_t t = encode_t(v[N + x], e_base);
        const uint32_t p = ((t << 1) | (t >> 31)) & 0x1fffffffu;
#pragma unroll
        for (int b = 0; b < 29; b++) {
            const int s = 29 * x + b;
            d[s / 3] |= ((p >> b) & 1u) << (28 + s % 3);
        }
    }
}

template <int S>
__host__ __device__ inline void decode_lane_t(const uint32_t *d, uint32_t *t)
{
    constexpr int N = lane_dw(S), X = 8 * S - N;
#pragma unroll
    for (int i = 0; i < N; i++) t[i] = d[i] & 0x8fffffffu;
#pragma unroll
    for (int x = 0; x < X; x++) {
        uint32_t p = 0;
#pragma unroll
        for (int q = (29 * x) / 3; q <= (29 * x + 28) / 3; q++) {
            const int lo = 29 * x > 3 * q ? 29 * x : 3 * q;
            const int hi = 29 * x + 29 < 3 * q + 3 ? 29 * x + 29 : 3 * q + 3;
            const uint32_t piece = (d[q] >> (28 + lo - 3 * q)) & ((1u << (hi - lo)) - 1u);
            p |= piece << (lo - 29 * x);
        }
        t[N + x] = (p >> 1) | (p << 31);
    }
}

}
}
```

llama2.zig_amd/csrc/packed_w.hip:

```cpp
#include "kernel_common.h"
#include "packed_w.h"

namespace l2z {
namespace {

__global__ __launch_bounds__(256) void pk_stats_kernel(const uint32_t *__restrict__ p, size_t count, uint32_t *stats)
{
    uint32_t mx = 0, mn = 255, bad = 0;
    for (size_t i = (size_t)blockIdx.x * 256 + threadIdx.x; i < count; i += (size_t)gridDim.x * 256) {
        const uint32_t v = p[i], e = (v >> 23) & 0xffu;
        if (e == 255u || (e == 0u && (v & 0x7fffffu) != 0u)) bad = 1;
        if (e != 0u) {
            mx = e > mx ? e : mx;
            mn = e < mn ? e : mn;
        }
    }
    for (int o = 32; o > 0; o >>= 1) {
        const uint32_t omx = __shfl_xor(mx, o, 64), omn = __shfl_xor(mn, o, 64), ob = __shfl_xor(bad, o, 64);
        mx = omx > mx ? omx : mx;
        mn = omn < mn ? omn : mn;
        bad |= ob;
    }
    if ((threadIdx.x & 63) == 0) {
        atomicMax(stats + 0, mx);
        atomicMin(stats + 1, mn);
        if (bad) atomicOr(stats + 2, 1u);
    }
}

template <int S>
__device__ __forceinline__ void pk_pack_lane(const uint32_t *ra, const uint32_t *rb, int c4, int e_base, uint32_t *dst)
{
    uint32_t v[8 * S > 0 ? 8 * S : 1], d[pk::lane_dw(S) > 0 ? pk::lane_dw(S) : 1];
#pragma unroll
    for (int k = 0; k < S; k++)
#pragma unroll
        for (int j = 0; j < 4; j++) {
            v[8 * k + j] = ra[4 * (c4 + 256 * k) + j];
            v[8 * k + 4 + j] = rb[4 * (c4 + 256 * k) + j];
        }
#pragma unroll
    for (int i = 0; i < pk::lane_dw(S); i++) d[i] = 0;
    pk::encode_lane<S>(v, e_base, d);
    const int lane = threadIdx.x & 63;
#pragma unroll
    for (int i = 0; i < pk::lane_dw(S); i++) dst[pk::plane_off(S, i, lane)] = d[i];
}

template <int S>
__device__ __forceinline__ void pk_unpack_lane(const uint32_t *src, int c4, int e_base, uint32_t *oa, uint32_t *ob)
{
    const int lane = threadIdx.x & 63;
    constexpr int N = pk::lane_dw(S);
    uint32_t d[N > 0 ? N : 1], t[8 * S > 0 ? 8 * S : 1];
#pragma unroll
    for (int i = 0; i < N; i++) d[i] = src[pk::plane_off(S, i, lane)];
    pk::decode_lane_t<S>(d, t);
#pragma unroll
    for (int k = 0; k < S; k++)
#pragma unroll
        for (int j = 0; j < 4; j++) {
            oa[4 * (c4 + 256 * k) + j] = __float_as_uint(__builtin_amdgcn_ldexpf(__uint_as_float(t[8 * k + j]), e_base - 31));
            ob[4 * (c4 + 256 * k) + j] = __float_as_uint(__builtin_amdgcn_ldexpf(__uint_as_float(t[8 * k + 4 + j]), e_base - 31));
        }
}

template <bool PACK>
__global__ __launch_bounds__(256) void pk_pack_kernel(const uint32_t *m, uint32_t *pk, uint32_t *out, int n, int e_base)
{
    const int n4 = n >> 2, q = blockIdx.x, b = blockIdx.y, w = threadIdx.x >> 6;
    const int s = pk::steps(n4, b, w);
    const size_t base = (size_t)q * pk::pair_dw(n4) + pk::chunk_off(n4, b, w);
    const int c4 = b * pk::kBatchF4 + threadIdx.x;
    const size_t ra = (size_t)(2 * q) * n, rb = ra + n;
    switch (s) {
#define L2Z_PK_CASE(S_)                                                            \
    case S_:                                                                       \
        if (PACK) pk_pack_lane<S_>(m + ra, m + rb, c4, e_base, pk + base);         \
        else pk_unpack_lane<S_>(pk + base, c4, e_base, out + ra, out + rb);        \
        break;
        L2Z_PK_CASE(1)
        L2Z_PK_CASE(2)
        L2Z_PK_CASE(3)
        L2Z_PK_CASE(4)
#undef L2Z_PK_CASE
        default: break;
    }
}

}

hipError_t launch_pk_stats(const float *m, size_t count, uint32_t *stats, hipStream_t st)
{
    size_t blocks = (count + 255) / 256;
    if (blocks > 256 * 16) blocks = 256 * 16;
    hipLaunchKernelGGL(pk_stats_kernel, dim3((unsigned)blocks), dim3(256), 0, st, (const uint32_t *)m, count, stats);
    return hipGetLastError();
}

hipError_t launch_pk_pack(const float *m, int rows, int n, int e_base, uint32_t *pk, hipStream_t st)
{
    if (!pk::width_ok(n) || rows <= 0 || rows % 2) return hipErrorInvalidValue;
    const dim3 grid(rows / 2, (n / 4 + pk::kBatchF4 - 1) / pk::kBatchF4);
    hipLaunchKernelGGL(pk_pack_kernel<true>, grid, dim3(256), 0, st, (const uint32_t *)m, pk, nullptr, n, e_base);
    return hipGetLastError();
}

hipError_t launch_pk_unpack(const uint32_t *pk, int rows, int n, int e_base, float *out, hipStream_t st)
{
    if (!pk::width_ok(n) || rows <= 0 || rows % 2) return hipErrorInvalidValue;
    const dim3 grid(rows / 2, (n / 4 + pk::kBatchF4 - 1) / pk::kBatchF4);
    hipLaunchKernelGGL(pk_pack_kernel<false>, grid, dim3(256), 0, st, nullptr, const_cast<uint32_t *>(pk),
                       (uint32_t *)out, n, e_base);
    return hipGetLastError();
}

}
```

llama2.zig_amd/csrc/tunables.cpp:

```cpp
#include "tunables.h"

#include <cstdlib>
#include <cstring>

namespace l2z {
namespace {

void env_int(const char *name, int *v)
{
    if (const char *e = getenv(name))
        if (*e) *v = atoi(e);
}

Tunables read_env()
{
    Tunables t;
    env_int("L2Z_GRID_CAP", &t.grid_cap);
    env_int("L2Z_ATTN_SPLIT", &t.attn_split);
    env_int("L2Z_ATTN_SPLIT_POS", &t.attn_split_pos);
    env_int("L2Z_FUSE_SMALL", &t.fuse_small);
    env_int("L2Z_SCHEME_B", &t.scheme_b);
    env_int("L2Z_NO_GRAPH", &t.no_graph);
    if (const char *e = getenv("L2Z_COMM")) t.prefer_rccl = strcmp(e, "rccl") == 0;
    env_int("L2Z_ARGMAX_XCHG", &t.argmax_xchg);
    env_int("L2Z_P2P_CONSUME", &t.p2p_consume);
    if (const char *e = getenv("L2Z_P2P_TIMEOUT_S"))
        if (*e) t.p2p_timeout_s = atoll(e);
    env_int("L2Z_P2P_BULK_MB", &t.p2p_bulk_mb);
    env_int("L2Z_PREFILL", &t.prefill);
    env_int("L2Z_PF_CHUNK", &t.pf_chunk);
    env_int("L2Z_PF_PANEL", &t.pf_panel);
    env_int("L2Z_PF_PANEL_MAX", &t.pf_panel_max);
    env_int("L2Z_PF_X3", &t.pf_x3);
    env_int("L2Z_PF_X3_STREAM_MIN", &t.pf_x3_stream_min);
    env_int("L2Z_PF_FUSE_PLANES", &t.pf_fuse_planes);
    env_int("L2Z_PACKED_W", &t.packed_w);
    env_int("L2Z_PACKED_KINDS", &t.packed_kinds);
    return t;
}

}

namespace {
Tunables &mutable_tunables()
{
    static Tunables t = read_env();
    return t;
}
}

const Tunables &tunables() { return mutable_tunables(); }

int prefill_chunk_tokens()
{
    int n = tunables().pf_chunk > 0 ? tunables().pf_chunk : 1024;
    if (n < 16) n = 16;
    if (n > 2048) n = 2048;
    return n;
}

int prefill_next_chunk(int remaining)
{
    if (tunables().pf_chunk > 0) return remaining < prefill_chunk_tokens() ? remaining : prefill_chunk_tokens();
    return remaining >= 1024 ? 1024 : remaining < 512 ? remaining : 512;
}

bool tunables_set(const char *name, long long v)
{
    Tunables &t = mutable_tunables();
    struct { const char *n; int *p; } ints[] = {
        {"L2Z_GRID_CAP", &t.grid_cap}, {"L2Z_ATTN_SPLIT", &t.attn_split}, {"L2Z_ATTN_SPLIT_POS", &t.attn_split_pos},
        {"L2Z_FUSE_SMALL", &t.fuse_small}, {"L2Z_NO_GRAPH", &t.no_graph}, {"L2Z_SCHEME_B", &t.scheme_b},
        {"L2Z_COMM_RCCL", &t.prefer_rccl}, {"L2Z_ARGMAX_XCHG", &t.argmax_xchg}, {"L2Z_P2P_CONSUME", &t.p2p_consume},
        {"L2Z_P2P_BULK_MB", &t.p2p_bulk_mb}, {"L2Z_PREFILL", &t.prefill}, {"L2Z_PF_CHUNK", &t.pf_chunk},
        {"L2Z_PF_PANEL", &t.pf_panel}, {"L2Z_PF_PANEL_MAX", &t.pf_panel_max},
        {"L2Z_PF_X3", &t.pf_x3}, {"L2Z_PF_X3_STREAM_MIN", &t.pf_x3_stream_min},
        {"L2Z_PF_FUSE_PLANES", &t.pf_fuse_planes}, {"L2Z_PACKED_W", &t.packed_w},
        {"L2Z_PACKED_KINDS", &t.packed_kinds}};
    for (auto &e : ints)
        if (strcmp(e.n, name) == 0) {
            *e.p = (int)v;
            return true;
        }
    if (strcmp(name, "L2Z_P2P_TIMEOUT_S") == 0) {
        t.p2p_timeout_s = v;
        return true;
    }
    return false;
}

}
```

llama2.zig_amd/csrc/tunables.h:

```cpp
#pragma once

namespace l2z {

struct Tunables {
    int grid_cap = 0;
    int attn_split = -1;
    int attn_split_pos = -1;
    int fuse_small = 1;
    int no_graph = 0;
    int prefer_rccl = 0;
    int p2p_consume = -1;
    int argmax_xchg = 1;
    long long p2p_timeout_s = 20;
    int scheme_b = 0;
    int p2p_bulk_mb = -1;
    int prefill = 1;
    int pf_chunk = 0;
    int pf_panel = 1;
    int pf_x3 = 1;
    int pf_x3_stream_min = 33;
    int pf_fuse_planes = 1;
    int packed_w = 1;
    int packed_kinds = -1;
    int pf_panel_max = -1;

    static constexpr int row_blocks = 2;
    static constexpr int max_blocks_per_cu = 8;
    static constexpr int p2p_push = 1;
    static constexpr int reduce_block = 128;
    static constexpr int pf_skinny_max = 64;
};

const Tunables &tunables();
int prefill_chunk_tokens();
int prefill_next_chunk(int remaining);
bool tunables_set(const char *env_name, long long value);

}
```

llama2.zig_amd/csrc/weights.cpp:

```cpp
#include <algorithm>
#include <atomic>
#include <cmath>
#include <cstdlib>
#include <cstring>
#include <mutex>

#include "l2z_state.h"
#include "packed_w.h"
#include "q8_layout.h"
#include "tunables.h"

namespace l2z {

static thread_local char g_err[512] = "";

void set_error(const char *fmt, ...)
{
    va_list ap;
    va_start(ap, fmt);
    vsnprintf(g_err, sizeof g_err, fmt, ap);
    va_end(ap);
}

int make_shard(const l2z_config &c, const l2z_comm *comm, Shard *out)
{
    Shard s;
    s.rank = comm ? comm->rank : 0;
    s.world = comm ? comm->world : 1;
    L2Z_CHECK(c.dim > 0 && c.hidden_dim > 0 && c.n_layers > 0 && c.n_heads > 0 &&
                  c.n_kv_heads > 0 && c.vocab_size > 0 && c.seq_len > 0,
              L2Z_ERR_INVALID, "config: all seven fields must be positive");
    L2Z_CHECK(c.dim % c.n_heads == 0, L2Z_ERR_INVALID, "config: dim %% n_heads != 0");
    L2Z_CHECK(c.n_heads % c.n_kv_heads == 0, L2Z_ERR_INVALID, "config: n_heads %% n_kv_heads != 0");
    s.hs = c.dim / c.n_heads;
    L2Z_CHECK(s.hs % 2 == 0, L2Z_ERR_INVALID, "config: head_size must be even (RoPE pairs)");
    const int kv_dim = (int)(((int64_t)c.dim * c.n_kv_heads) / c.n_heads);
    int64_t a, b;
    L2Z_TRY(l2z_shard_range(c.dim, s.hs, s.rank, s.world, &a, &b));
    s.dim0 = (int)a;
    s.dim_loc = (int)(b - a);
    s.heads_loc = s.dim_loc / s.hs;
    L2Z_TRY(l2z_shard_range(kv_dim, s.hs, s.rank, s.world, &a, &b));
    s.kvd_loc = (int)(b - a);
    L2Z_TRY(l2z_shard_range(c.hidden_dim, 1, s.rank, s.world, &a, &b));
    s.hid0 = (int)a;
    s.hid_loc = (int)(b - a);
    L2Z_TRY(l2z_shard_range(c.vocab_size, 1, s.rank, s.world, &a, &b));
    s.v0 = (int)a;
    s.v_loc = (int)(b - a);
    s.scheme_b = tunables().scheme_b != 0 && comm != nullptr && (s.world > 1 || comm->nccl != nullptr);
    s.dimc_pad = pad_cols(s.dim_loc);
    s.hidc_pad = pad_cols(s.hid_loc);
    *out = s;
    return L2Z_OK;
}

int pad_cols(int n)
{
    const int n4 = (n + 3) / 4;
    return n > 768 ? ((n4 + 63) / 64) * 256 : n4 * 4;
}

std::vector<TensorDesc> tensor_table(const l2z_config &c, bool shared)
{
    const size_t V = c.vocab_size, dim = c.dim, hid = c.hidden_dim, L = c.n_layers;
    const size_t S = c.seq_len, hs = dim / c.n_heads, kvd = (dim * c.n_kv_heads) / c.n_heads;
    const float s_dim = sqrtf(3.0f / (float)dim), s_hid = sqrtf(3.0f / (float)hid);
    const float s_emb = 2.0f * s_dim;
    std::vector<TensorDesc> t = {
        {"token_embedding_table", 0, 1, V, dim, REPL, s_emb, 0.0f},
        {"rms_att_weight", 0, L, 1, dim, REPL, 0.1f, 1.0f},
        {"wq", 0, L, dim, dim, BY_Q_HEADS, s_dim, 0.0f},
        {"wk", 0, L, kvd, dim, BY_KV_HEADS, s_dim, 0.0f},
        {"wv", 0, L, kvd, dim, BY_KV_HEADS, s_dim, 0.0f},
        {"wo", 0, L, dim, dim, BY_DIM_ROWS, s_dim, 0.0f},
        {"rms_ffn_weight", 0, L, 1, dim, REPL, 0.1f, 1.0f},
        {"w1", 0, L, hid, dim, BY_HIDDEN, s_dim, 0.0f},
        {"w2", 0, L, dim, hid, BY_DIM_ROWS, s_hid, 0.0f},
        {"w3", 0, L, hid, dim, BY_HIDDEN, s_dim, 0.0f},
        {"rms_final_weight", 0, 1, 1, dim, REPL, 0.1f, 1.0f},
        {"freq_cis_real", 0, 1, 1, S * hs / 2, SKIP, 1.0f, 0.0f},
        {"freq_cis_imag", 0, 1, 1, S * hs / 2, SKIP, 1.0f, 0.0f},
    };
    if (!shared) t.push_back({"wcls", 0, 1, V, dim, BY_VOCAB, s_emb, 0.0f});
    size_t off = 0;
    for (auto &d : t) {
        d.offset = off;
        off += d.count();
    }
    return t;
}

void shard_rows(const TensorDesc &d, const Shard &s, size_t *r0, size_t *r1)
{
    switch (d.kind) {
        case BY_Q_HEADS:
        case BY_DIM_ROWS: *r0 = s.dim0; *r1 = (size_t)s.dim0 + s.dim_loc; break;
        case BY_KV_HEADS: *r0 = (size_t)s.rank * s.kvd_loc; *r1 = *r0 + s.kvd_loc; break;
        case BY_HIDDEN: *r0 = s.hid0; *r1 = (size_t)s.hid0 + s.hid_loc; break;
        case BY_VOCAB: *r0 = s.v0; *r1 = (size_t)s.v0 + s.v_loc; break;
        default: *r0 = 0; *r1 = d.rows; break;
    }
}

int g_cus = 0;

int ensure_device(int device)
{
    int n = 0;
    hipError_t e = hipGetDeviceCount(&n);
    if (e != hipSuccess || n <= 0) {
        set_error("no HIP device available (%s); this library has no CPU fallback",
                  e == hipSuccess ? "device count is 0" : hipGetErrorString(e));
        return L2Z_ERR_NO_DEVICE;
    }
    L2Z_CHECK(device >= 0 && device < n, L2Z_ERR_NO_DEVICE, "device %d out of range (%d present)",
              device, n);
    L2Z_HIP(hipSetDevice(device));
    if (g_cus == 0) {
        hipDeviceProp_t p;
        L2Z_HIP(hipGetDeviceProperties(&p, device));
        g_cus = p.multiProcessorCount > 0 ? p.multiProcessorCount : 256;
    }
    return L2Z_OK;
}

int current_device_for(const l2z_comm *comm)
{
    if (comm) return comm->device;
    int d = 0;
    if (hipGetDevice(&d) != hipSuccess) d = 0;
    return d;
}

}

using namespace l2z;

namespace {

constexpr size_t kBlobSlackFloats = 1024;
bool is_w1(const TensorDesc &d) { return strcmp(d.name, "w1") == 0; }
bool is_w3(const TensorDesc &d) { return strcmp(d.name, "w3") == 0; }

bool col_shard(const l2z_weights *w, const TensorDesc &d, size_t *c0, size_t *cl, size_t *cpad)
{
    if (!w->sh.scheme_b || d.kind != BY_DIM_ROWS) return false;
    const bool is_wo = strcmp(d.name, "wo") == 0;
    *c0 = is_wo ? w->sh.dim0 : w->sh.hid0;
    *cl = is_wo ? w->sh.dim_loc : w->sh.hid_loc;
    *cpad = is_wo ? w->sh.dimc_pad : w->sh.hidc_pad;
    return true;
}

size_t slot_floats(const l2z_weights *w, const TensorDesc &d)
{
    size_t r0, r1;
    shard_rows(d, w->sh, &r0, &r1);
    if (d.kind == SKIP && !w->file_layout) return 0;
    if (is_w3(d)) return 0;
    size_t c0, cl, cpad;
    if (col_shard(w, d, &c0, &cl, &cpad)) return d.layers * d.rows * cpad;
    return d.layers * (r1 - r0) * d.cols * (is_w1(d) ? 2 : 1);
}

void carve_local(l2z_weights *w, const std::vector<TensorDesc> &tt)
{
    size_t off = 0, off_w1 = 0;
    const float *base = w->blob;
    w->dev_off.assign(tt.size(), 0);
    for (size_t i = 0; i < tt.size(); i++) {
        const auto &d = tt[i];
        if (is_w1(d)) off_w1 = off;
        w->dev_off[i] = is_w3(d) ? off_w1 + d.cols : off;
        const float *p = base + w->dev_off[i];
        const std::string n = d.name;
        if (n == "token_embedding_table") w->tok_emb = p;
        else if (n == "rms_att_weight") w->rms_att = p;
        else if (n == "wq") w->wq = p;
        else if (n == "wk") w->wk = p;
        else if (n == "wv") w->wv = p;
        else if (n == "wo") w->wo = p;
        else if (n == "rms_ffn_weight") w->rms_ffn = p;
        else if (n == "w1") w->w1 = p;
        else if (n == "w2") w->w2 = p;
        else if (n == "w3") w->w3 = p;
        else if (n == "rms_final_weight") w->rms_final = p;
        else if (n == "wcls") w->wcls = p;
        off += slot_floats(w, d);
    }
    if (w->shared) w->wcls = w->tok_emb + (size_t)w->sh.v0 * w->cfg.dim;
}

size_t local_floats(const l2z_weights *w, const std::vector<TensorDesc> &tt)
{
    size_t off = 0;
    for (const auto &d : tt) off += slot_floats(w, d);
    return off;
}

hipError_t upload(float *dst, const float *src, size_t n_floats)
{
    const size_t piece = (size_t)256 << 20;
    hipError_t e = hipSuccess;
    for (size_t o = 0; o < n_floats && e == hipSuccess; o += piece) {
        const size_t n = n_floats - o < piece ? n_floats - o : piece;
        e = hipMemcpy(dst + o, src + o, n * sizeof(float), hipMemcpyHostToDevice);
    }
    return e;
}

int weights_alloc(const l2z_config *config, int shared_weights, const l2z_comm *comm,
                  l2z_weights **out, std::vector<TensorDesc> *tt_out)
{
    L2Z_CHECK(config != nullptr && out != nullptr, L2Z_ERR_INVALID, "weights_init: null argument");
    const int dev = current_device_for(comm);
    L2Z_TRY(ensure_device(dev));
    Shard sh;
    L2Z_TRY(make_shard(*config, comm, &sh));
    static std::atomic<uint64_t> next_uid{1};
    l2z_weights *w = new l2z_weights();
    w->uid = next_uid.fetch_add(1);
    w->cfg = *config;
    w->shared = shared_weights ? 1 : 0;
    w->device = dev;
    w->sh = sh;
    w->file_layout = sh.world == 1 && !sh.scheme_b;
    *tt_out = tensor_table(*config, w->shared != 0);
    w->blob_floats = local_floats(w, *tt_out);
    hipError_t e = hipMalloc(&w->blob, (w->blob_floats + kBlobSlackFloats) * sizeof(float));
    if (e == hipSuccess) e = hipMemset(w->blob + w->blob_floats, 0, kBlobSlackFloats * sizeof(float));
    if (e != hipSuccess) {
        set_error("hipMalloc(%zu bytes) for weights failed: %s", w->blob_floats * sizeof(float),
                  hipGetErrorString(e));
        delete w;
        return e == hipErrorOutOfMemory ? L2Z_ERR_OOM : L2Z_ERR_HIP;
    }
    carve_local(w, *tt_out);
    *out = w;
    return L2Z_OK;
}

void build_packed_kind(l2z_weights *w, int kind, int per_layer, std::vector<l2z_weights::PkMat> slots)
{
    l2z_weights::PkKind &k = w->pk[kind];
    k.per_layer = per_layer;
    k.slots = std::move(slots);
    const size_t n = k.slots.size();
    std::vector<uint32_t> stats(3 * n);
    for (size_t i = 0; i < n; i++) {
        stats[3 * i] = 0;
        stats[3 * i + 1] = 255;
        stats[3 * i + 2] = 0;
    }
    uint32_t *d_stats = nullptr;
    hipError_t e = hipMalloc((void **)&d_stats, stats.size() * sizeof(uint32_t));
    if (e == hipSuccess) e = hipMemcpy(d_stats, stats.data(), stats.size() * sizeof(uint32_t), hipMemcpyHostToDevice);
    for (size_t i = 0; i < n && e == hipSuccess; i++)
        e = launch_pk_stats(k.slots[i].src, (size_t)k.slots[i].rows * k.slots[i].cols, d_stats + 3 * i, nullptr);
    if (e == hipSuccess) e = hipMemcpy(stats.data(), d_stats, stats.size() * sizeof(uint32_t), hipMemcpyDeviceToHost);
    if (d_stats) (void)hipFree(d_stats);
    const auto dwords = [&](size_t i) -> size_t {
        const auto &m = k.slots[i];
        if (m.rows % 2 || !pk::encodable(stats[3 * i], stats[3 * i + 1], stats[3 * i + 2])) return 0;
        return (size_t)(m.rows / 2) * pk::pair_dw(m.cols / 4);
    };
    size_t total = 0;
    for (size_t i = 0; i < n; i++) total += dwords(i);
    if (e == hipSuccess && total > 0) {
        e = hipMalloc((void **)&k.blob, total * sizeof(uint32_t));
        if (e != hipSuccess) k.blob = nullptr;
    }
    size_t off = 0;
    for (size_t i = 0; i < n && e == hipSuccess && k.blob; i++) {
        auto &m = k.slots[i];
        if (dwords(i) == 0) continue;
        e = launch_pk_pack(m.src, m.rows, m.cols, (int)stats[3 * i], k.blob + off, nullptr);
        m.p = k.blob + off;
        m.e = (int)stats[3 * i];
        k.packed++;
        off += dwords(i);
    }
    if (e == hipSuccess) e = hipDeviceSynchronize();
    if (e != hipSuccess) {
        (void)hipGetLastError();
        if (k.blob) (void)hipFree(k.blob);
        k.blob = nullptr;
        for (auto &m : k.slots) m.p = nullptr;
        k.packed = 0;
    }
}

void build_packed(l2z_weights *w)
{
    if (tunables().packed_w == 0 || !w->file_layout) return;
    const l2z_config &c = w->cfg;
    const size_t dim = c.dim, hid = c.hidden_dim, kvd = (size_t)c.dim / c.n_heads * c.n_kv_heads;
    const int L = c.n_layers;
    using Slots = std::vector<l2z_weights::PkMat>;
    const auto mat = [](const float *src, size_t rows, size_t cols) {
        l2z_weights::PkMat m;
        m.src = src; m.rows = (int)rows; m.cols = (int)cols;
        return m;
    };
    if (pk::width_ok(c.dim)) {
        Slots s13, sqkv, so, scls;
        for (int l = 0; l < L; l++) {
            s13.push_back(mat(w->w1 + (size_t)l * hid * 2 * dim, 2 * hid, dim));
            sqkv.push_back(mat(w->wq + (size_t)l * dim * dim, dim, dim));
            sqkv.push_back(mat(w->wk + (size_t)l * kvd * dim, kvd, dim));
            sqkv.push_back(mat(w->wv + (size_t)l * kvd * dim, kvd, dim));
            so.push_back(mat(w->wo + (size_t)l * dim * dim, dim, dim));
        }
        scls.push_back(mat(w->wcls, c.vocab_size, dim));
        build_packed_kind(w, KIND_FFN13, 1, std::move(s13));
        build_packed_kind(w, KIND_QKV, 3, std::move(sqkv));
        build_packed_kind(w, KIND_WO, 1, std::move(so));
        build_packed_kind(w, KIND_CLS, 1, std::move(scls));
    }
    if (pk::width_ok(c.hidden_dim)) {
        Slots s2;
        for (int l = 0; l < L; l++) s2.push_back(mat(w->w2 + (size_t)l * dim * hid, dim, hid));
        build_packed_kind(w, KIND_FFN2, 1, std::move(s2));
    }
}

}

extern "C" int l2z_abi_version(void) { return L2Z_ABI_VERSION; }
extern "C" const char *l2z_last_error(void) { return l2z::g_err; }

extern "C" int l2z_device_count(int *out_n)
{
    L2Z_CHECK(out_n != nullptr, L2Z_ERR_INVALID, "l2z_device_count: null out");
    int n = 0;
    hipError_t e = hipGetDeviceCount(&n);
    if (e != hipSuccess) n = 0;
    *out_n = n;
    return L2Z_OK;
}

extern "C" int l2z_device_info(int dev, char *name, size_t cap, int *out_cus, uint64_t *out_hbm)
{
    L2Z_TRY(ensure_device(dev));
    hipDeviceProp_t p;
    L2Z_HIP(hipGetDeviceProperties(&p, dev));
    if (name && cap) snprintf(name, cap, "%s (%s)", p.name[0] ? p.name : "AMD GPU", p.gcnArchName);
    if (out_cus) *out_cus = p.multiProcessorCount;
    if (out_hbm) *out_hbm = (uint64_t)p.totalGlobalMem;
    return L2Z_OK;
}

extern "C" int l2z_weights_init(const l2z_config *config, const float *data, size_t n_floats,
                                int shared_weights, const l2z_comm *comm, l2z_weights **out)
{
    L2Z_CHECK(data != nullptr, L2Z_ERR_INVALID, "l2z_weights_init: null data");
    std::vector<TensorDesc> tt;
    l2z_weights *w = nullptr;
    L2Z_TRY(weights_alloc(config, shared_weights, comm, &w, &tt));
    const size_t need = tt.back().offset + tt.back().count();
    if (n_floats < need) {
        set_error("l2z_weights_init: blob has %zu f32, config needs %zu", n_floats, need);
        l2z_weights_free(w);
        return L2Z_ERR_INVALID;
    }
    hipError_t e = hipSuccess;
    float *stage = nullptr;
    for (size_t i = 0; i < tt.size() && e == hipSuccess; i++) {
        const auto &d = tt[i];
        if (d.kind == SKIP && !w->file_layout) continue;
        size_t r0, r1;
        shard_rows(d, w->sh, &r0, &r1);
        const size_t rl = r1 - r0;
        float *dst = w->blob + w->dev_off[i];
        size_t c0, cl, cpad;
        if (col_shard(w, d, &c0, &cl, &cpad)) {
            e = hipMemset(dst, 0, d.layers * d.rows * cpad * sizeof(float));
            for (size_t l = 0; l < d.layers && e == hipSuccess; l++)
                e = hipMemcpy2D(dst + l * d.rows * cpad, cpad * sizeof(float), data + d.offset + l * d.rows * d.cols + c0,
                                d.cols * sizeof(float), cl * sizeof(float), d.rows, hipMemcpyHostToDevice);
            continue;
        }
        if (is_w1(d) || is_w3(d)) {
            const size_t piece_rows = std::max<size_t>(1, std::min<size_t>(rl, ((size_t)64 << 20) / (d.cols * sizeof(float))));
            if (stage == nullptr) e = hipMalloc((void **)&stage, 2 * piece_rows * d.cols * sizeof(float));
            size_t n_piece = 0;
            for (size_t l = 0; l < d.layers && e == hipSuccess; l++) {
                for (size_t r = 0; r < rl && e == hipSuccess; r += piece_rows, n_piece++) {
                    const size_t nr = std::min(piece_rows, rl - r);
                    float *sb = stage + (n_piece & 1) * piece_rows * d.cols;
                    e = upload(sb, data + d.offset + (l * d.rows + r0 + r) * d.cols, nr * d.cols);
                    if (e == hipSuccess) e = launch_copy_rows(dst + (l * rl + r) * 2 * d.cols, 2 * d.cols, sb, nr, d.cols, nullptr);
                }
            }
            if (e == hipSuccess) e = hipDeviceSynchronize();
        } else if (rl == d.rows) {
            e = upload(dst, data + d.offset, d.count());
        } else {
            for (size_t l = 0; l < d.layers && e == hipSuccess; l++)
                e = upload(dst + l * rl * d.cols, data + d.offset + (l * d.rows + r0) * d.cols, rl * d.cols);
        }
    }
    if (stage) (void)hipFree(stage);
    if (e != hipSuccess) {
        set_error("weight upload failed: %s", hipGetErrorString(e));
        l2z_weights_free(w);
        return L2Z_ERR_HIP;
    }
    build_packed(w);
    *out = w;
    return L2Z_OK;
}

extern "C" int l2z_weights_init_synthetic(const l2z_config *config, int shared_weights,
                                          uint64_t seed, const l2z_comm *comm, l2z_weights **out)
{
    std::vector<TensorDesc> tt;
    l2z_weights *w = nullptr;
    L2Z_TRY(weights_alloc(config, shared_weights, comm, &w, &tt));
    hipError_t e = hipSuccess;
    for (size_t i = 0; i < tt.size(); i++) {
        const auto &d = tt[i];
        if (d.kind == SKIP && !w->file_layout) continue;
        size_t r0, r1;
        shard_rows(d, w->sh, &r0, &r1);
        const size_t rl = r1 - r0;
        const bool pair = is_w1(d) || is_w3(d);
        size_t c0, cl, cpad;
        if (col_shard(w, d, &c0, &cl, &cpad)) {
            float *dst = w->blob + w->dev_off[i];
            e = hipMemsetAsync(dst, 0, d.layers * d.rows * cpad * sizeof(float), nullptr);
            for (size_t l = 0; l < d.layers && e == hipSuccess; l++)
                e = launch_synth_fill(dst + l * d.rows * cpad, d.offset + l * d.rows * d.cols + c0, d.rows * cl, seed, d.scale, d.bias,
                                      nullptr, cl, cpad, d.cols);
            continue;
        }
        for (size_t l = 0; l < d.layers && e == hipSuccess; l++) {
            const uint64_t base = d.offset + (l * d.rows + r0) * d.cols;
            e = launch_synth_fill(w->blob + w->dev_off[i] + l * rl * d.cols * (pair ? 2 : 1), base, rl * d.cols, seed, d.scale,
                                  d.bias, nullptr, pair ? d.cols : 0, pair ? 2 * d.cols : 0);
        }
    }
    if (e == hipSuccess) e = hipDeviceSynchronize();
    if (e != hipSuccess) {
        set_error("synthetic weight fill failed: %s", hipGetErrorString(e));
        l2z_weights_free(w);
        return L2Z_ERR_HIP;
    }
    build_packed(w);
    *out = w;
    return L2Z_OK;
}

extern "C" int l2z_weights_read(const l2z_weights *w, size_t offset, size_t count, float *out)
{
    L2Z_CHECK(w != nullptr && out != nullptr, L2Z_ERR_INVALID, "l2z_weights_read: null argument");
    L2Z_CHECK(!w->is_q8(), L2Z_ERR_INVALID, "l2z_weights_read: int8 group-quantized weights hold no f32 tensors (l2z_weights_q8_read)");
    L2Z_CHECK(w->file_layout, L2Z_ERR_INVALID, "l2z_weights_read: only for unsharded weights");
    L2Z_CHECK(offset + count <= w->blob_floats, L2Z_ERR_INVALID, "l2z_weights_read: out of range");
    L2Z_HIP(hipSetDevice(w->device));
    const std::vector<TensorDesc> tt = tensor_table(w->cfg, w->shared != 0);
    const size_t lo = offset, hi = offset + count;
    for (size_t i = 0; i < tt.size(); i++) {
        const auto &d = tt[i];
        const size_t t0 = std::max(lo, d.offset), t1 = std::min(hi, d.offset + d.count());
        if (t0 >= t1) continue;
        if (!(is_w1(d) || is_w3(d))) {
            L2Z_HIP(hipMemcpy(out + (t0 - lo), w->blob + w->dev_off[i] + (t0 - d.offset), (t1 - t0) * sizeof(float),
                              hipMemcpyDeviceToHost));
            continue;
        }
        for (size_t f = t0; f < t1;) {
            const size_t r = (f - d.offset) / d.cols, c = (f - d.offset) % d.cols;
            const float *src = w->blob + w->dev_off[i] + r * 2 * d.cols + c;
            const size_t whole = c == 0 ? (t1 - f) / d.cols : 0;
            if (whole > 0) {
                L2Z_HIP(hipMemcpy2D(out + (f - lo), d.cols * sizeof(float), src, 2 * d.cols * sizeof(float),
                                    d.cols * sizeof(float), whole, hipMemcpyDeviceToHost));
                f += whole * d.cols;
            } else {
                const size_t n = std::min(d.cols - c, t1 - f);
                L2Z_HIP(hipMemcpy(out + (f - lo), src, n * sizeof(float), hipMemcpyDeviceToHost));
                f += n;
            }
        }
    }
    return L2Z_OK;
}

extern "C" void l2z_weights_free(l2z_weights *w)
{
    if (!w) return;
    if (w->blob) (void)hipFree(w->blob);
    if (w->q8_blob) (void)hipFree(w->q8_blob);
    for (auto &k : w->pk)
        if (k.blob) (void)hipFree(k.blob);
    delete w;
}

namespace {

int packed_read_slot(const l2z_weights *w, int kind, int layer, int j, float *out, size_t n_floats)
{
    const l2z_weights::PkKind &k = w->pk[kind];
    L2Z_CHECK(layer >= 0 && j >= 0 && j < k.per_layer && (size_t)layer * k.per_layer + j < k.slots.size(), L2Z_ERR_INVALID,
              "l2z_weights_packed_read: no packed slot %d of layer %d of kind %s", j, layer, kKindNames[kind]);
    const l2z_weights::PkMat *pm = w->pk_slot(kind, layer, j);
    L2Z_CHECK(pm != nullptr, L2Z_ERR_STATE, "l2z_weights_packed_read: slot %d of layer %d of kind %s is not packed", j, layer,
              kKindNames[kind]);
    const size_t count = (size_t)pm->rows * pm->cols;
    L2Z_CHECK(n_floats >= count, L2Z_ERR_INVALID, "l2z_weights_packed_read: need %zu floats", count);
    L2Z_HIP(hipSetDevice(w->device));
    float *d = nullptr;
    L2Z_HIP(hipMalloc((void **)&d, count * sizeof(float)));
    hipError_t e = launch_pk_unpack(pm->p, pm->rows, pm->cols, pm->e, d, nullptr);
    if (e == hipSuccess) e = hipMemcpy(out, d, count * sizeof(float), hipMemcpyDeviceToHost);
    (void)hipFree(d);
    L2Z_HIP(e);
    return L2Z_OK;
}

}

extern "C" int l2z_weights_packed_count(const l2z_weights *w, int *n_packed, int *n_candidates)
{
    return l2z_weights_packed_count_kind(w, KIND_FFN13, n_packed, n_candidates);
}

extern "C" int l2z_weights_packed_read(const l2z_weights *w, int layer, float *out, size_t n_floats)
{
    L2Z_CHECK(w != nullptr && out != nullptr, L2Z_ERR_INVALID, "l2z_weights_packed_read: null argument");
    return packed_read_slot(w, KIND_FFN13, layer, 0, out, n_floats);
}

extern "C" int l2z_weights_packed_count_kind(const l2z_weights *w, int kind, int *n_packed, int *n_candidates)
{
    L2Z_CHECK(w != nullptr && n_packed != nullptr && n_candidates != nullptr, L2Z_ERR_INVALID,
              "l2z_weights_packed_count: null argument");
    L2Z_CHECK(kind >= 0 && kind < KIND_COUNT, L2Z_ERR_INVALID, "l2z_weights_packed_count_kind: bad kind %d", kind);
    *n_packed = w->pk[kind].packed;
    *n_candidates = (int)w->pk[kind].slots.size();
    return L2Z_OK;
}

extern "C" int l2z_weights_packed_read_kind(const l2z_weights *w, int kind, int layer, int slot, float *out, size_t n_floats)
{
    L2Z_CHECK(w != nullptr && out != nullptr, L2Z_ERR_INVALID, "l2z_weights_packed_read: null argument");
    L2Z_CHECK(kind >= 0 && kind < KIND_COUNT, L2Z_ERR_INVALID, "l2z_weights_packed_read_kind: bad kind %d", kind);
    return packed_read_slot(w, kind, layer, slot, out, n_floats);
}

namespace {

enum { Q8S_EMB = 0, Q8S_WQ, Q8S_WK, Q8S_WV, Q8S_WO, Q8S_W13, Q8S_W2, Q8S_CLS, Q8S_COUNT };

struct Q8Slot {
    size_t values;
    size_t q_off, s_off;
};

size_t align256(size_t v) { return (v + 255) & ~(size_t)255; }

int q8_layout_of(const char *fn, const l2z_config *c, int shared, int gs, uint64_t n_bytes, bool with_body, q8::Layout *lay)
{
    const q8::Dims d = {c->dim, c->hidden_dim, c->n_layers, c->n_heads, c->n_kv_heads, c->vocab_size, c->seq_len};
    const int st = with_body ? q8::layout_checked(d, shared != 0, gs, n_bytes, lay) : q8::layout(d, shared != 0, gs, lay);
    L2Z_CHECK(st == q8::LAYOUT_OK, L2Z_ERR_INVALID, "%s: %s (dim %d, hidden_dim %d, group_size %d, %llu bytes)", fn,
              q8::status_text(st), c->dim, c->hidden_dim, gs, (unsigned long long)n_bytes);
    return L2Z_OK;
}

int q8_alloc(const l2z_config *config, int shared, int gs, const q8::Layout &lay, l2z_weights **out)
{
    const int dev = current_device_for(nullptr);
    L2Z_TRY(ensure_device(dev));
    Shard sh;
    L2Z_TRY(make_shard(*config, nullptr, &sh));
    static std::atomic<uint64_t> next_uid{uint64_t(1) << 32};
    l2z_weights *w = new l2z_weights();
    w->uid = next_uid.fetch_add(1);
    w->cfg = *config;
    w->shared = shared ? 1 : 0;
    w->device = dev;
    w->sh = sh;
    w->file_layout = false;
    w->q8_gs = gs;
    const size_t L = config->n_layers, dim = config->dim;
    Q8Slot sl[Q8S_COUNT] = {};
    sl[Q8S_EMB].values = lay.t[q8::T_EMB].values();
    sl[Q8S_WQ].values = lay.t[q8::T_WQ].values();
    sl[Q8S_WK].values = lay.t[q8::T_WK].values();
    sl[Q8S_WV].values = lay.t[q8::T_WV].values();
    sl[Q8S_WO].values = lay.t[q8::T_WO].values();
    sl[Q8S_W13].values = 2 * lay.t[q8::T_W1].values();
    sl[Q8S_W2].values = lay.t[q8::T_W2].values();
    sl[Q8S_CLS].values = lay.t[q8::T_CLS].present ? lay.t[q8::T_CLS].values() : 0;
    size_t off = 0;
    const size_t o_att = off; off = align256(off + L * dim * 4);
    const size_t o_ffn = off; off = align256(off + L * dim * 4);
    const size_t o_fin = off; off = align256(off + dim * 4);
    for (auto &s : sl) {
        s.q_off = off; off = align256(off + s.values);
        s.s_off = off; off = align256(off + s.values / (size_t)gs * 4);
    }
    hipError_t e = hipMalloc((void **)&w->q8_blob, off);
    if (e != hipSuccess) {
        set_error("hipMalloc(%zu bytes) for int8 weights failed: %s", off, hipGetErrorString(e));
        delete w;
        return e == hipErrorOutOfMemory ? L2Z_ERR_OOM : L2Z_ERR_HIP;
    }
    w->rms_att = (const float *)(w->q8_blob + o_att);
    w->rms_ffn = (const float *)(w->q8_blob + o_ffn);
    w->rms_final = (const float *)(w->q8_blob + o_fin);
    l2z_weights::Q8Mat *mats[Q8S_COUNT] = {&w->q_emb, &w->q_wq, &w->q_wk, &w->q_wv, &w->q_wo, &w->q_w13, &w->q_w2, &w->q_cls};
    for (int i = 0; i < Q8S_COUNT; i++) {
        if (sl[i].values == 0) continue;
        mats[i]->q = (const int8_t *)(w->q8_blob + sl[i].q_off);
        mats[i]->s = (const float *)(w->q8_blob + sl[i].s_off);
    }
    if (sl[Q8S_CLS].values == 0) w->q_cls = w->q_emb;
    *out = w;
    return L2Z_OK;
}

struct Q8Place {
    const l2z_weights::Q8Mat *m;
    int interleave;
};
Q8Place q8_place(const l2z_weights *w, int t)
{
    switch (t) {
        case q8::T_EMB: return {&w->q_emb, 0};
        case q8::T_WQ: return {&w->q_wq, 0};
        case q8::T_WK: return {&w->q_wk, 0};
        case q8::T_WV: return {&w->q_wv, 0};
        case q8::T_WO: return {&w->q_wo, 0};
        case q8::T_W1: return {&w->q_w13, 1};
        case q8::T_W2: return {&w->q_w2, 0};
        case q8::T_W3: return {&w->q_w13, 2};
        default: return {&w->q_cls, 0};
    }
}

hipError_t q8_copy_tensor(const l2z_weights *w, const q8::Mat &m, int t, size_t layer0, size_t layers, int8_t *host_q,
                          float *host_s, bool to_device)
{
    const Q8Place pl = q8_place(w, t);
    const size_t gs = (size_t)w->q8_gs, row_q = m.cols, row_s = m.cols / gs * 4, rows = m.rows;
    const hipMemcpyKind kind = to_device ? hipMemcpyHostToDevice : hipMemcpyDeviceToHost;
    hipError_t e = hipSuccess;
    for (size_t l = 0; l < layers && e == hipSuccess; l++) {
        const size_t il = pl.interleave ? 2 : 1, first = pl.interleave ? (size_t)(pl.interleave - 1) : 0;
        char *dq = (char *)pl.m->q + ((layer0 + l) * rows * il + first) * row_q;
        char *ds = (char *)pl.m->s + ((layer0 + l) * rows * il + first) * row_s;
        char *hq = (char *)host_q + l * rows * row_q, *hs = (char *)host_s + l * rows * row_s;
        if (to_device) {
            e = hipMemcpy2D(dq, il * row_q, hq, row_q, row_q, rows, kind);
            if (e == hipSuccess) e = hipMemcpy2D(ds, il * row_s, hs, row_s, row_s, rows, kind);
        } else {
            e = hipMemcpy2D(hq, row_q, dq, il * row_q, row_q, rows, kind);
            if (e == hipSuccess) e = hipMemcpy2D(hs, row_s, ds, il * row_s, row_s, rows, kind);
        }
    }
    return e;
}

}

extern "C" int l2z_weights_init_q8(const l2z_config *config, const void *body, size_t n_bytes, int shared_classifier,
                                   int group_size, const l2z_comm *comm, l2z_weights **out)
{
    L2Z_CHECK(config != nullptr && body != nullptr && out != nullptr, L2Z_ERR_INVALID, "l2z_weights_init_q8: null argument");
    L2Z_CHECK(comm == nullptr, L2Z_ERR_INVALID, "l2z_weights_init_q8: int8 group-quantized weights are unsharded (comm must be null)");
    q8::Layout lay;
    L2Z_TRY(q8_layout_of("l2z_weights_init_q8", config, shared_classifier, group_size, n_bytes, true, &lay));
    l2z_weights *w = nullptr;
    L2Z_TRY(q8_alloc(config, shared_classifier, group_size, lay, &w));
    const char *b = (const char *)body;
    const size_t L = config->n_layers, dim = config->dim;
    hipError_t e = hipMemcpy((void *)w->rms_att, b + lay.rms_att_off, L * dim * 4, hipMemcpyHostToDevice);
    if (e == hipSuccess) e = hipMemcpy((void *)w->rms_ffn, b + lay.rms_ffn_off, L * dim * 4, hipMemcpyHostToDevice);
    if (e == hipSuccess) e = hipMemcpy((void *)w->rms_final, b + lay.rms_final_off, dim * 4, hipMemcpyHostToDevice);
    for (int t = 0; t < q8::T_COUNT && e == hipSuccess; t++) {
        const q8::Mat &m = lay.t[t];
        if (!m.present) continue;
        e = q8_copy_tensor(w, m, t, 0, m.layers, (int8_t *)(b + m.q_off), (float *)(b + m.s_off), true);
    }
    if (e != hipSuccess) {
        set_error("l2z_weights_init_q8: upload failed: %s", hipGetErrorString(e));
        l2z_weights_free(w);
        return L2Z_ERR_HIP;
    }
    *out = w;
    return L2Z_OK;
}

extern "C" int l2z_weights_init_q8_from(const l2z_weights *src, int group_size, l2z_weights **out)
{
    L2Z_CHECK(src != nullptr && out != nullptr, L2Z_ERR_INVALID, "l2z_weights_init_q8_from: null argument");
    L2Z_CHECK(!src->is_q8() && src->file_layout, L2Z_ERR_INVALID,
              "l2z_weights_init_q8_from: the source must be an unsharded f32 weights object");
    q8::Layout lay;
    L2Z_TRY(q8_layout_of("l2z_weights_init_q8_from", &src->cfg, src->shared, group_size, 0, false, &lay));
    L2Z_HIP(hipSetDevice(src->device));
    l2z_weights *w = nullptr;
    L2Z_TRY(q8_alloc(&src->cfg, src->shared, group_size, lay, &w));
    const size_t L = src->cfg.n_layers, dim = src->cfg.dim;
    hipError_t e = hipMemcpy((void *)w->rms_att, src->rms_att, L * dim * 4, hipMemcpyDeviceToDevice);
    if (e == hipSuccess) e = hipMemcpy((void *)w->rms_ffn, src->rms_ffn, L * dim * 4, hipMemcpyDeviceToDevice);
    if (e == hipSuccess) e = hipMemcpy((void *)w->rms_final, src->rms_final, dim * 4, hipMemcpyDeviceToDevice);
    const auto quant = [&](const float *f, const l2z_weights::Q8Mat &m, size_t values) {
        if (e == hipSuccess) e = launch_q8_quantize(f, values, group_size, true, (int8_t *)m.q, (float *)m.s, nullptr);
    };
    quant(src->tok_emb, w->q_emb, lay.t[q8::T_EMB].values());
    quant(src->wq, w->q_wq, lay.t[q8::T_WQ].values());
    quant(src->wk, w->q_wk, lay.t[q8::T_WK].values());
    quant(src->wv, w->q_wv, lay.t[q8::T_WV].values());
    quant(src->wo, w->q_wo, lay.t[q8::T_WO].values());
    quant(src->w1, w->q_w13, 2 * lay.t[q8::T_W1].values());
    quant(src->w2, w->q_w2, lay.t[q8::T_W2].values());
    if (lay.t[q8::T_CLS].present) quant(src->wcls, w->q_cls, lay.t[q8::T_CLS].values());
    if (e == hipSuccess) e = hipDeviceSynchronize();
    if (e != hipSuccess) {
        set_error("l2z_weights_init_q8_from: quantization failed: %s", hipGetErrorString(e));
        l2z_weights_free(w);
        return L2Z_ERR_HIP;
    }
    *out = w;
    return L2Z_OK;
}

extern "C" int l2z_weights_q8_read(const l2z_weights *w, const char *tensor_name, int layer, int8_t *out_q, float *out_s)
{
    L2Z_CHECK(w != nullptr && tensor_name != nullptr && out_q != nullptr && out_s != nullptr, L2Z_ERR_INVALID,
              "l2z_weights_q8_read: null argument");
    L2Z_CHECK(w->is_q8(), L2Z_ERR_INVALID, "l2z_weights_q8_read: not int8 group-quantized weights");
    q8::Layout lay;
    L2Z_TRY(q8_layout_of("l2z_weights_q8_read", &w->cfg, w->shared, w->q8_gs, 0, false, &lay));
    const int t = q8::tensor_by_name(tensor_name);
    L2Z_CHECK(t >= 0, L2Z_ERR_INVALID, "l2z_weights_q8_read: no quantized tensor \"%s\"", tensor_name);
    const q8::Mat &m = lay.t[t];
    L2Z_CHECK(layer >= 0 && (uint64_t)layer < m.layers, L2Z_ERR_INVALID, "l2z_weights_q8_read: layer %d of %s", layer, tensor_name);
    L2Z_HIP(hipSetDevice(w->device));
    L2Z_HIP(q8_copy_tensor(w, m, t, (size_t)layer, 1, out_q, out_s, false));
    return L2Z_OK;
}
```

Measured before the change: 242.0 tokens/s.

## Add lossless 28-bit packed weight format with escape records for matvec

Introduces a 28-bit-per-weight packed encoding that narrows the exponent range relative to a per-matrix base. The rare out-of-range values are stored exactly in a small per-row-pair escape record. A new row-kernel variant decodes this format and patches escapes, and weight building picks 28-bit per slot when escape counts fit. It is enabled by default for selected kinds and aims to cut weight bandwidth in the memory-bound decode, at the cost of extra decode ALU work and wave-uniform escape handling.

```diff
diff --git a/llama2.zig_amd/csrc/forward.cpp b/llama2.zig_amd/csrc/forward.cpp
--- a/llama2.zig_amd/csrc/forward.cpp
+++ b/llama2.zig_amd/csrc/forward.cpp
@@ -284,9 +284,9 @@
             a.pos_ptr = s->d_pos; a.rope = s->rope; a.head_size = sh.hs; a.rope_segs = 2;
             const auto *pq = pk_slot(KIND_QKV, l, 0), *pkk = pk_slot(KIND_QKV, l, 1), *pv = pk_slot(KIND_QKV, l, 2);
             if (pq && pkk && pv) {
-                a.pk = pq->p; a.pk_e = pq->e;
-                a.pk1 = pkk->p; a.pk_e1 = pkk->e;
-                a.pk2 = pv->p; a.pk_e2 = pv->e;
+                a.pk = pq->p; a.pk_e = pq->e; a.pk_rec = pq->rec;
+                a.pk1 = pkk->p; a.pk_e1 = pkk->e; a.pk_rec1 = pkk->rec;
+                a.pk2 = pv->p; a.pk_e2 = pv->e; a.pk_rec2 = pv->rec;
             }
             L2Z_LAUNCH(KIND_QKV, launch_matvec(a, PRO_RMS, EPI_ROPE, mb, g_cus, st));
         }
@@ -320,7 +320,7 @@
                 a.rows0 = sh.dim_loc; a.n = c.dim;
                 x_in(a, s->xb, gi, sh.dim_loc);
                 push_to(a, 1);
-                if (const auto *p = pk_slot(KIND_WO, l)) { a.pk = p->p; a.pk_e = p->e; }
+                if (const auto *p = pk_slot(KIND_WO, l)) { a.pk = p->p; a.pk_e = p->e; a.pk_rec = p->rec; }
             }
             L2Z_LAUNCH(KIND_WO, launch_matvec(a, PRO_NONE, epi, mb, g_cus, st, nullptr, &pushed));
         }
@@ -335,7 +335,7 @@
             a.rms_w = w->rms_ffn + (size_t)l * dim;
             x_in(a, s->x, gi, sh.dim_loc);
             if (!sb) push_to(a, 2);
-            if (const auto *p = pk_slot(KIND_FFN13, l)) { a.pk = p->p; a.pk_e = p->e; }
+            if (const auto *p = pk_slot(KIND_FFN13, l)) { a.pk = p->p; a.pk_e = p->e; a.pk_rec = p->rec; }
             L2Z_LAUNCH(KIND_FFN13, launch_matvec(a, PRO_RMS, EPI_SWIGLU, mb, g_cus, st, nullptr, &pushed));
         }
         if (!sb) L2Z_TRY(gather(s->hb, sh.hid_loc));
@@ -350,7 +350,7 @@
                 a.rows0 = sh.dim_loc; a.n = c.hidden_dim;
                 x_in(a, s->hb, gi, sh.hid_loc);
                 push_to(a, 1);
-                if (const auto *p = pk_slot(KIND_FFN2, l)) { a.pk = p->p; a.pk_e = p->e; }
+                if (const auto *p = pk_slot(KIND_FFN2, l)) { a.pk = p->p; a.pk_e = p->e; a.pk_rec = p->rec; }
             }
             L2Z_LAUNCH(KIND_FFN2, launch_matvec(a, PRO_NONE, epi, mb, g_cus, st, nullptr, &pushed));
         }
@@ -367,7 +367,7 @@
                           matvec_vector_width(c.dim);
         int grid = 0;
         if (!xchg) push_to(a, 3);
-        if (const auto *p = fuse ? pk_slot(KIND_CLS, 0) : nullptr) { a.pk = p->p; a.pk_e = p->e; }
+        if (const auto *p = fuse ? pk_slot(KIND_CLS, 0) : nullptr) { a.pk = p->p; a.pk_e = p->e; a.pk_rec = p->rec; }
         L2Z_LAUNCH(KIND_CLS, launch_matvec(a, PRO_RMS, fuse ? EPI_ARGMAX : EPI_STORE, mb, g_cus, st,
                                            &grid, &pushed));
         s->n_part = fuse ? grid : 0;
diff --git a/llama2.zig_amd/csrc/l2z_internal.h b/llama2.zig_amd/csrc/l2z_internal.h
--- a/llama2.zig_amd/csrc/l2z_internal.h
+++ b/llama2.zig_amd/csrc/l2z_internal.h
@@ -124,6 +124,7 @@
     LLIn xin;
     const uint32_t *pk, *pk1, *pk2;
     int pk_e, pk_e1, pk_e2;
+    const uint32_t *pk_rec, *pk_rec1, *pk_rec2;
     int tl_slot;
 };
 
@@ -178,6 +179,9 @@
 hipError_t launch_pk_stats(const float *m, size_t count, uint32_t *stats, hipStream_t st);
 hipError_t launch_pk_pack(const float *m, int rows, int n, int e_base, uint32_t *pk, hipStream_t st);
 hipError_t launch_pk_unpack(const uint32_t *pk, int rows, int n, int e_base, float *out, hipStream_t st);
+hipError_t launch_pk28_count(const float *m, int rows, int n, int e_base, uint32_t *max_esc, hipStream_t st);
+hipError_t launch_pk28_pack(const float *m, int rows, int n, int e_base, uint32_t *pk, uint32_t *rec, hipStream_t st);
+hipError_t launch_pk28_unpack(const uint32_t *pk, const uint32_t *rec, int rows, int n, int e_base, float *out, hipStream_t st);
 hipError_t launch_matvec(const MatvecArgs &a, int pro, int epi, int max_blocks_per_cu, int n_cus,
                          hipStream_t st, int *out_grid = nullptr, bool *pushed = nullptr);
 bool attention_push_supported(const AttnArgs &a);
diff --git a/llama2.zig_amd/csrc/l2z_state.h b/llama2.zig_amd/csrc/l2z_state.h
--- a/llama2.zig_amd/csrc/l2z_state.h
+++ b/llama2.zig_amd/csrc/l2z_state.h
@@ -63,6 +63,8 @@
     struct PkMat {
         const uint32_t *p = nullptr;
         int e = 0;
+        const uint32_t *rec = nullptr;
+        int bits() const { return p == nullptr ? 0 : rec != nullptr ? 28 : 29; }
         const float *src = nullptr;
         int rows = 0, cols = 0;
     };
diff --git a/llama2.zig_amd/csrc/matvec.hip b/llama2.zig_amd/csrc/matvec.hip
--- a/llama2.zig_amd/csrc/matvec.hip
+++ b/llama2.zig_amd/csrc/matvec.hip
@@ -279,6 +279,76 @@
     }
 };
 
+struct PkRaw28 {
+    v4u q4[7];
+    uint32_t rec;
+};
+
+template <int EPI>
+struct RowPacked28 {
+    static constexpr int kSets = 2;
+    v4f wa[kRowU], wb[kRowU];
+    PkRaw28 raw[kSets];
+    int e15[kSets];
+    const uint32_t *pp, *pr;
+    int e_pt, wave_u;
+
+    __device__ __forceinline__ void init(const MvLocals &, int, int) { wave_u = __builtin_amdgcn_readfirstlane(threadIdx.x >> 6); }
+    __device__ __forceinline__ void point(const MvLocals &m, int u)
+    {
+        int e;
+        pp = pair_packed28<EPI>(m, u, pk28::kPairDw, pk28::kRecDw, e, pr);
+        e_pt = e - 15;
+    }
+    template <int P>
+    __device__ __forceinline__ void issue(int)
+    {
+        const int lane = threadIdx.x & 63;
+        const uint32_t *src = pp + (size_t)wave_u * pk28::kChunkDw + lane * 4;
+#pragma unroll
+        for (int i = 0; i < 7; i++) raw[P].q4[i] = __builtin_nontemporal_load((const v4u *)(src + i * 256));
+        raw[P].rec = pr[lane & (pk28::kRecDw - 1)];
+        e15[P] = e_pt;
+    }
+    template <int P>
+    __device__ __forceinline__ void deliver()
+    {
+        uint32_t d[pk28::kLaneDw], t[32];
+#pragma unroll
+        for (int i = 0; i < pk28::kLaneDw; i++) {
+            const v4u v = raw[P].q4[i / 4];
+            d[i] = (i % 4 == 0) ? v.x : (i % 4 == 1) ? v.y : (i % 4 == 2) ? v.z : v.w;
+        }
+        pk28::decode_lane_t(d, t);
+        const int e = e15[P];
+#pragma unroll
+        for (int k = 0; k < 4; k++) {
+            wa[k] = v4f{__builtin_amdgcn_ldexpf(__uint_as_float(t[8 * k]), e), __builtin_amdgcn_ldexpf(__uint_as_float(t[8 * k + 1]), e),
+                        __builtin_amdgcn_ldexpf(__uint_as_float(t[8 * k + 2]), e), __builtin_amdgcn_ldexpf(__uint_as_float(t[8 * k + 3]), e)};
+            wb[k] = v4f{__builtin_amdgcn_ldexpf(__uint_as_float(t[8 * k + 4]), e), __builtin_amdgcn_ldexpf(__uint_as_float(t[8 * k + 5]), e),
+                        __builtin_amdgcn_ldexpf(__uint_as_float(t[8 * k + 6]), e), __builtin_amdgcn_ldexpf(__uint_as_float(t[8 * k + 7]), e)};
+        }
+        const uint32_t rv = raw[P].rec;
+        if (__builtin_amdgcn_readfirstlane(rv) != pk28::kNoEsc) {
+            const uint32_t tid = threadIdx.x;
+#pragma unroll 1
+            for (int n = 0; n < pk28::kMaxEsc; n++) {
+                const uint32_t pos = __builtin_amdgcn_readlane(rv, 2 * n), bits = __builtin_amdgcn_readlane(rv, 2 * n + 1);
+                if (pos == pk28::kNoEsc) break;
+                const uint32_t sel = (pos >> 5) == tid ? (pos & 31u) : 32u;
+                const float f = __uint_as_float(bits);
+#pragma unroll
+                for (int k = 0; k < 4; k++)
+#pragma unroll
+                    for (int j = 0; j < 4; j++) {
+                        wa[k][j] = sel == (uint32_t)(8 * k + j) ? f : wa[k][j];
+                        wb[k][j] = sel == (uint32_t)(8 * k + 4 + j) ? f : wb[k][j];
+                    }
+            }
+        }
+    }
+};
+
 #ifdef L2Z_TIMELINE
 constexpr int kMtlSlots = 256, kMtlBlocks = 512;
 __device__ long long g_mtl[kMtlSlots * kMtlBlocks * 8];
@@ -288,11 +358,13 @@
 #define L2Z_MTL(i) do { } while (0)
 #endif
 
-template <int PRO, int EPI, int XC, bool LL, bool PK = false>
+template <int PRO, int EPI, int XC, bool LL, int PK = 0>
 __global__ __launch_bounds__(kBlock) void matvec_row_kernel(const MatvecArgs a)
 {
+    static_assert(PK == 0 || PK == 29 || (PK == 28 && XC == 4), "packed forms of the row kernel");
     constexpr int U = kRowU;
-    using Src = typename std::conditional<PK, RowPacked<EPI, XC>, RowF32<EPI, XC>>::type;
+    using Src = typename std::conditional<PK == 28, RowPacked28<EPI>,
+                                          typename std::conditional<PK == 29, RowPacked<EPI, XC>, RowF32<EPI, XC>>::type>::type;
     constexpr int NS = Src::kSets;
     extern __shared__ __attribute__((aligned(16))) float lds[];
 #ifdef L2Z_TIMELINE
@@ -300,7 +372,7 @@
 #endif
     L2Z_MTL(0);
     MvLocals m_ = mv_locals<EPI>(a);
-    if constexpr (PK) m_.push = nullptr;
+    if constexpr (PK != 0) m_.push = nullptr;
     const MvLocals m = m_;
     const int n4 = m.n >> 2;
     const int n_batches = (n4 + kBlock * U - 1) / (kBlock * U);
@@ -476,7 +548,7 @@
     return big_x ? mv_entry<PRO, EPI, 64, 12, LL>() : mv_entry<PRO, EPI, 64, 4, LL>();
 }
 
-template <int PRO, int EPI, bool LL, bool PK = false>
+template <int PRO, int EPI, bool LL, int PK = 0>
 const void *mv_row_fn(bool big_x)
 {
     return big_x ? reinterpret_cast<const void *>(&matvec_row_kernel<PRO, EPI, 12, LL, PK>)
@@ -495,7 +567,16 @@
 
 const void *mv_row_pick_packed(int pro, int epi, bool big_x)
 {
-#define X(P, E, LL, SC, PK) L2Z_IF_##PK(if (pro == P && epi == E) return mv_row_fn<P, E, false, true>(big_x);)
+#define X(P, E, LL, SC, PK) L2Z_IF_##PK(if (pro == P && epi == E) return mv_row_fn<P, E, false, 29>(big_x);)
+    L2Z_MV_COMBOS(X)
+#undef X
+    return nullptr;
+}
+
+const void *mv_row_pick_packed28(int pro, int epi)
+{
+#define X(P, E, LL, SC, PK) \
+    L2Z_IF_##PK(if (pro == P && epi == E) return reinterpret_cast<const void *>(&matvec_row_kernel<P, E, 4, false, 28>);)
     L2Z_MV_COMBOS(X)
 #undef X
     return nullptr;
@@ -579,6 +660,11 @@
     if (ll && !vec) return hipErrorNotSupported;
     if (a.pk != nullptr && (!use_row || ll || !pk::width_ok(a.n))) return hipErrorInvalidValue;
     if (a.pk != nullptr) a.push = nullptr;
+    const bool pk28_form = a.pk_rec != nullptr;
+    if (pk28_form && (a.pk == nullptr || !pk28::width_ok(a.n))) return hipErrorInvalidValue;
+    if (a.pk != nullptr && epi != EPI_SWIGLU &&
+        ((a.rows1 > 0 && (a.pk_rec1 != nullptr) != pk28_form) || (a.rows2 > 0 && (a.pk_rec2 != nullptr) != pk28_form)))
+        return hipErrorInvalidValue;
     if (a.pk != nullptr && epi != EPI_SWIGLU &&
         ((a.rows1 > 0 && a.pk1 == nullptr) || (a.rows2 > 0 && a.pk2 == nullptr) || a.rows0 % 2 || a.rows1 % 2 || a.rows2 % 2))
         return hipErrorInvalidValue;
@@ -587,7 +673,8 @@
     int n_units;
     const auto padded = [n4](int batch) { return ((n4 + batch - 1) / batch) * batch; };
     if (use_row) {
-        k.fn = a.pk != nullptr ? mv_row_pick_packed(pro, epi, a.n > 4096) : mv_row_pick(pro, epi, a.n > 4096, ll);
+        k.fn = pk28_form ? mv_row_pick_packed28(pro, epi)
+               : a.pk != nullptr ? mv_row_pick_packed(pro, epi, a.n > 4096) : mv_row_pick(pro, epi, a.n > 4096, ll);
         lds = (size_t)(4 * padded(kBlock * kRowU) + kScratch + 4 * kWaves) * sizeof(float);
         n_units = n_pairs;
     } else if (vec) {
diff --git a/llama2.zig_amd/csrc/matvec_device.h b/llama2.zig_amd/csrc/matvec_device.h
--- a/llama2.zig_amd/csrc/matvec_device.h
+++ b/llama2.zig_amd/csrc/matvec_device.h
@@ -17,6 +17,7 @@
     size_t push_base;
     const uint32_t *pk, *pk1, *pk2;
     int pk_e, pk_e1, pk_e2;
+    const uint32_t *pk_rec, *pk_rec1, *pk_rec2;
 };
 
 template <int EPI>
@@ -38,6 +39,7 @@
     m.push_base = m.push ? (size_t)m.push->rank * m.push->count : 0;
     m.pk = a.pk; m.pk1 = a.pk1; m.pk2 = a.pk2;
     m.pk_e = a.pk_e; m.pk_e1 = a.pk_e1; m.pk_e2 = a.pk_e2;
+    m.pk_rec = a.pk_rec; m.pk_rec1 = a.pk_rec1; m.pk_rec2 = a.pk_rec2;
     return m;
 }
 
@@ -88,6 +90,23 @@
         return r.pick(m.pk, m.pk1, m.pk2) + (size_t)(r.row >> 1) * pair_dw;
     }
     e_base = m.pk_e;
+    return m.pk + (size_t)p * pair_dw;
+}
+
+template <int EPI>
+__device__ __forceinline__ const uint32_t *pair_packed28(const MvLocals &m, int p, size_t pair_dw, size_t rec_dw, int &e_base,
+                                                         const uint32_t *&rec)
+{
+    if (p >= m.n_pairs) p = m.n_pairs - 1;
+    if (EPI == EPI_ROPE) {
+        const SegRow r = seg_row(m, 2 * p);
+        const size_t q = (size_t)(r.row >> 1);
+        e_base = r.pick(m.pk_e, m.pk_e1, m.pk_e2);
+        rec = r.pick(m.pk_rec, m.pk_rec1, m.pk_rec2) + q * rec_dw;
+        return r.pick(m.pk, m.pk1, m.pk2) + q * pair_dw;
+    }
+    e_base = m.pk_e;
+    rec = m.pk_rec + (size_t)p * rec_dw;
     return m.pk + (size_t)p * pair_dw;
 }
 
diff --git a/llama2.zig_amd/csrc/packed_w.h b/llama2.zig_amd/csrc/packed_w.h
--- a/llama2.zig_amd/csrc/packed_w.h
+++ b/llama2.zig_amd/csrc/packed_w.h
@@ -92,4 +92,123 @@
 }
 
 }
-}
+
+namespace pk28 {
+
+constexpr int kLaneDw = 28;
+constexpr int kChunkDw = 64 * kLaneDw;
+constexpr int kPairDw = 4 * kChunkDw;
+constexpr int kMaxEsc = 8;
+constexpr int kRecDw = 2 * kMaxEsc;
+constexpr uint32_t kNoEsc = 0xffffffffu;
+
+__host__ __device__ constexpr bool width_ok(int n) { return n == 4 * pk::kBatchF4; }
+__host__ __device__ constexpr int plane_off(int i, int lane) { return (i / 4) * 256 + lane * 4 + i % 4; }
+__host__ __device__ constexpr uint32_t esc_pos(int wave, int lane, int i) { return (uint32_t)(wave << 11 | lane << 5 | i); }
+
+__host__ __device__ inline bool is_escape(uint32_t v, int e_base)
+{
+    const int e = (int)((v >> 23) & 0xffu);
+    return e != 0 && e < e_base - 14;
+}
+
+__host__ __device__ inline uint32_t encode_t(uint32_t v, int e_base)
+{
+    const uint32_t e = (v >> 23) & 0xffu;
+    if (is_escape(v, e_base)) return 0u;
+    const uint32_t c = e == 0 ? 0u : e - (uint32_t)(e_base - 15);
+    return (v & 0x807fffffu) | (c << 23);
+}
+
+__host__ __device__ inline uint32_t encode_lane(const uint32_t *v, int e_base, uint32_t *d)
+{
+    uint32_t esc = 0;
+#pragma unroll
+    for (int i = 0; i < 32; i++) esc |= (is_escape(v[i], e_base) ? 1u : 0u) << i;
+#pragma unroll
+    for (int i = 0; i < kLaneDw; i++) d[i] = encode_t(v[i], e_base);
+#pragma unroll
+    for (int x = 0; x < 4; x++) {
+        const uint32_t t = encode_t(v[kLaneDw + x], e_base);
+        const uint32_t p = ((t << 1) | (t >> 31)) & 0x0fffffffu;
+#pragma unroll
+        for (int q = 0; q < 7; q++) d[7 * x + q] |= ((p >> (4 * q)) & 0xfu) << 27;
+    }
+    return esc;
+}
+
+__host__ __device__ inline void decode_lane_t(const uint32_t *d, uint32_t *t)
+{
+#pragma unroll
+    for (int i = 0; i < kLaneDw; i++) t[i] = d[i] & 0x87ffffffu;
+#pragma unroll
+    for (int x = 0; x < 4; x++) {
+        uint32_t p = 0;
+#pragma unroll
+        for (int q = 0; q < 7; q++) p |= ((d[7 * x + q] >> 27) & 0xfu) << (4 * q);
+        t[kLaneDw + x] = (p >> 1) | (p << 31);
+    }
+}
+
+__host__ __device__ inline uint32_t value_of_t(uint32_t t, int e_base)
+{
+    const uint32_t c = (t >> 23) & 0xffu;
+    return c == 0 ? (t & 0x80000000u) : ((t & 0x807fffffu) | ((c + (uint32_t)(e_base - 15)) << 23));
+}
+
+__host__ __device__ inline void record_clear(uint32_t *rec)
+{
+    for (int k = 0; k < kMaxEsc; k++) {
+        rec[2 * k] = kNoEsc;
+        rec[2 * k + 1] = 0u;
+    }
+}
+
+inline int encode_pair(const uint32_t *ra, const uint32_t *rb, int e_base, uint32_t *stream, uint32_t *rec)
+{
+    int n_esc = 0;
+    record_clear(rec);
+    for (int w = 0; w < 4; w++)
+        for (int lane = 0; lane < 64; lane++) {
+            uint32_t v[32], d[kLaneDw];
+            for (int k = 0; k < 4; k++)
+                for (int j = 0; j < 4; j++) {
+                    const int col = 4 * (64 * w + lane + 256 * k) + j;
+                    v[8 * k + j] = ra[col];
+                    v[8 * k + 4 + j] = rb[col];
+                }
+            const uint32_t esc = encode_lane(v, e_base, d);
+            for (int i = 0; i < kLaneDw; i++) stream[w * kChunkDw + plane_off(i, lane)] = d[i];
+            for (int i = 0; i < 32; i++)
+                if ((esc >> i) & 1u) {
+                    if (n_esc < kMaxEsc) {
+                        rec[2 * n_esc] = esc_pos(w, lane, i);
+                        rec[2 * n_esc + 1] = v[i];
+                    }
+                    n_esc++;
+                }
+        }
+    return n_esc;
+}
+
+inline void decode_pair(const uint32_t *stream, const uint32_t *rec, int e_base, uint32_t *ra, uint32_t *rb)
+{
+    for (int w = 0; w < 4; w++)
+        for (int lane = 0; lane < 64; lane++) {
+            uint32_t d[kLaneDw], t[32];
+            for (int i = 0; i < kLaneDw; i++) d[i] = stream[w * kChunkDw + plane_off(i, lane)];
+            decode_lane_t(d, t);
+            for (int i = 0; i < 32; i++) t[i] = value_of_t(t[i], e_base);
+            for (int k = 0; k < kMaxEsc; k++)
+                if (rec[2 * k] != kNoEsc && (rec[2 * k] >> 5) == (uint32_t)(64 * w + lane)) t[rec[2 * k] & 31u] = rec[2 * k + 1];
+            for (int k = 0; k < 4; k++)
+                for (int j = 0; j < 4; j++) {
+                    const int col = 4 * (64 * w + lane + 256 * k) + j;
+                    ra[col] = t[8 * k + j];
+                    rb[col] = t[8 * k + 4 + j];
+                }
+        }
+}
+
+}
+}
diff --git a/llama2.zig_amd/csrc/packed_w.hip b/llama2.zig_amd/csrc/packed_w.hip
--- a/llama2.zig_amd/csrc/packed_w.hip
+++ b/llama2.zig_amd/csrc/packed_w.hip
@@ -88,6 +88,90 @@
     }
 }
 
+
+
+__device__ __forceinline__ void pk28_lane_values(const uint32_t *ra, const uint32_t *rb, uint32_t (&v)[32])
+{
+#pragma unroll
+    for (int k = 0; k < 4; k++)
+#pragma unroll
+        for (int j = 0; j < 4; j++) {
+            v[8 * k + j] = ra[4 * (threadIdx.x + 256 * k) + j];
+            v[8 * k + 4 + j] = rb[4 * (threadIdx.x + 256 * k) + j];
+        }
+}
+
+__global__ __launch_bounds__(256) void pk28_count_kernel(const uint32_t *m, int e_base, uint32_t *max_esc)
+{
+    __shared__ uint32_t part[4];
+    const uint32_t *pr = m + (size_t)blockIdx.x * (2 * 4096);
+    uint32_t n = 0;
+    for (int i = threadIdx.x; i < 2 * 4096; i += 256) n += pk28::is_escape(pr[i], e_base) ? 1u : 0u;
+    for (int o = 32; o > 0; o >>= 1) n += __shfl_xor(n, o, 64);
+    if ((threadIdx.x & 63) == 0) part[threadIdx.x >> 6] = n;
+    __syncthreads();
+    if (threadIdx.x == 0) {
+        const uint32_t t = part[0] + part[1] + part[2] + part[3];
+        if (t > 0) atomicMax(max_esc, t);
+    }
+}
+
+__global__ __launch_bounds__(256) void pk28_pack_kernel(const uint32_t *m, uint32_t *pk, uint32_t *rec, int e_base)
+{
+    __shared__ uint32_t cnt[256];
+    __shared__ uint32_t r[pk28::kRecDw];
+    const int q = blockIdx.x, tid = threadIdx.x, lane = tid & 63, w = tid >> 6;
+    const uint32_t *ra = m + (size_t)(2 * q) * 4096, *rb = ra + 4096;
+    uint32_t v[32], d[pk28::kLaneDw];
+    pk28_lane_values(ra, rb, v);
+    const uint32_t esc = pk28::encode_lane(v, e_base, d);
+    uint32_t *dst = pk + (size_t)q * pk28::kPairDw + w * pk28::kChunkDw;
+#pragma unroll
+    for (int i = 0; i < pk28::kLaneDw; i++) dst[pk28::plane_off(i, lane)] = d[i];
+    cnt[tid] = __popc(esc);
+    if (tid < pk28::kRecDw) r[tid] = (tid & 1) ? 0u : pk28::kNoEsc;
+    __syncthreads();
+    if (esc != 0u) {
+        uint32_t at = 0;
+        for (int t = 0; t < tid; t++) at += cnt[t];
+#pragma unroll
+        for (int i = 0; i < 32; i++)
+            if ((esc >> i) & 1u) {
+                if (at < (uint32_t)pk28::kMaxEsc) {
+                    r[2 * at] = pk28::esc_pos(w, lane, i);
+                    r[2 * at + 1] = v[i];
+                }
+                at++;
+            }
+    }
+    __syncthreads();
+    if (tid < pk28::kRecDw) rec[(size_t)q * pk28::kRecDw + tid] = r[tid];
+}
+
+__global__ __launch_bounds__(256) void pk28_unpack_kernel(const uint32_t *pk, const uint32_t *rec, uint32_t *out, int e_base)
+{
+    const int q = blockIdx.x, tid = threadIdx.x, lane = tid & 63, w = tid >> 6;
+    const uint32_t *src = pk + (size_t)q * pk28::kPairDw + w * pk28::kChunkDw;
+    uint32_t d[pk28::kLaneDw], t[32];
+#pragma unroll
+    for (int i = 0; i < pk28::kLaneDw; i++) d[i] = src[pk28::plane_off(i, lane)];
+    pk28::decode_lane_t(d, t);
+    uint32_t *oa = out + (size_t)(2 * q) * 4096, *ob = oa + 4096;
+#pragma unroll
+    for (int k = 0; k < 4; k++)
+#pragma unroll
+        for (int j = 0; j < 4; j++) {
+            oa[4 * (tid + 256 * k) + j] = __float_as_uint(__builtin_amdgcn_ldexpf(__uint_as_float(t[8 * k + j]), e_base - 15));
+            ob[4 * (tid + 256 * k) + j] = __float_as_uint(__builtin_amdgcn_ldexpf(__uint_as_float(t[8 * k + 4 + j]), e_base - 15));
+        }
+    for (int k = 0; k < pk28::kMaxEsc; k++) {
+        const uint32_t pos = rec[(size_t)q * pk28::kRecDw + 2 * k];
+        if (pos == pk28::kNoEsc || (pos >> 5) != (uint32_t)tid) continue;
+        const int i = pos & 31u;
+        ((i & 4) ? ob : oa)[4 * (tid + 256 * (i >> 3)) + (i & 3)] = rec[(size_t)q * pk28::kRecDw + 2 * k + 1];
+    }
+}
+
 }
 
 hipError_t launch_pk_stats(const float *m, size_t count, uint32_t *stats, hipStream_t st)
@@ -115,4 +199,25 @@
     return hipGetLastError();
 }
 
-}
+hipError_t launch_pk28_count(const float *m, int rows, int n, int e_base, uint32_t *max_esc, hipStream_t st)
+{
+    if (!pk28::width_ok(n) || rows <= 0 || rows % 2) return hipErrorInvalidValue;
+    hipLaunchKernelGGL(pk28_count_kernel, dim3(rows / 2), dim3(256), 0, st, (const uint32_t *)m, e_base, max_esc);
+    return hipGetLastError();
+}
+
+hipError_t launch_pk28_pack(const float *m, int rows, int n, int e_base, uint32_t *pk, uint32_t *rec, hipStream_t st)
+{
+    if (!pk28::width_ok(n) || rows <= 0 || rows % 2) return hipErrorInvalidValue;
+    hipLaunchKernelGGL(pk28_pack_kernel, dim3(rows / 2), dim3(256), 0, st, (const uint32_t *)m, pk, rec, e_base);
+    return hipGetLastError();
+}
+
+hipError_t launch_pk28_unpack(const uint32_t *pk, const uint32_t *rec, int rows, int n, int e_base, float *out, hipStream_t st)
+{
+    if (!pk28::width_ok(n) || rows <= 0 || rows % 2) return hipErrorInvalidValue;
+    hipLaunchKernelGGL(pk28_unpack_kernel, dim3(rows / 2), dim3(256), 0, st, pk, rec, (uint32_t *)out, e_base);
+    return hipGetLastError();
+}
+
+}
diff --git a/llama2.zig_amd/csrc/tunables.cpp b/llama2.zig_amd/csrc/tunables.cpp
--- a/llama2.zig_amd/csrc/tunables.cpp
+++ b/llama2.zig_amd/csrc/tunables.cpp
@@ -36,6 +36,8 @@
     env_int("L2Z_PF_FUSE_PLANES", &t.pf_fuse_planes);
     env_int("L2Z_PACKED_W", &t.packed_w);
     env_int("L2Z_PACKED_KINDS", &t.packed_kinds);
+    env_int("L2Z_PACKED_BITS", &t.packed_bits);
+    env_int("L2Z_PACKED28_KINDS", &t.packed28_kinds);
     return t;
 }
 
@@ -76,7 +78,8 @@
         {"L2Z_PF_PANEL", &t.pf_panel}, {"L2Z_PF_PANEL_MAX", &t.pf_panel_max},
         {"L2Z_PF_X3", &t.pf_x3}, {"L2Z_PF_X3_STREAM_MIN", &t.pf_x3_stream_min},
         {"L2Z_PF_FUSE_PLANES", &t.pf_fuse_planes}, {"L2Z_PACKED_W", &t.packed_w},
-        {"L2Z_PACKED_KINDS", &t.packed_kinds}};
+        {"L2Z_PACKED_KINDS", &t.packed_kinds}, {"L2Z_PACKED_BITS", &t.packed_bits},
+        {"L2Z_PACKED28_KINDS", &t.packed28_kinds}};
     for (auto &e : ints)
         if (strcmp(e.n, name) == 0) {
             *e.p = (int)v;
diff --git a/llama2.zig_amd/csrc/tunables.h b/llama2.zig_amd/csrc/tunables.h
--- a/llama2.zig_amd/csrc/tunables.h
+++ b/llama2.zig_amd/csrc/tunables.h
@@ -22,6 +22,8 @@
     int pf_fuse_planes = 1;
     int packed_w = 1;
     int packed_kinds = -1;
+    int packed_bits = 28;
+    int packed28_kinds = 40;
     int pf_panel_max = -1;
 
     static constexpr int row_blocks = 2;
diff --git a/llama2.zig_amd/csrc/weights.cpp b/llama2.zig_amd/csrc/weights.cpp
--- a/llama2.zig_amd/csrc/weights.cpp
+++ b/llama2.zig_amd/csrc/weights.cpp
@@ -259,11 +259,38 @@
     for (size_t i = 0; i < n && e == hipSuccess; i++)
         e = launch_pk_stats(k.slots[i].src, (size_t)k.slots[i].rows * k.slots[i].cols, d_stats + 3 * i, nullptr);
     if (e == hipSuccess) e = hipMemcpy(stats.data(), d_stats, stats.size() * sizeof(uint32_t), hipMemcpyDeviceToHost);
+    const auto fits = [&](size_t i) {
+        return k.slots[i].rows % 2 == 0 && pk::encodable(stats[3 * i], stats[3 * i + 1], stats[3 * i + 2]);
+    };
+    std::vector<int> bits(n, 29);
+    const Tunables &tn = tunables();
+    const auto cand28 = [&](size_t i) {
+        return tn.packed_bits == 28 && ((tn.packed28_kinds >> kind) & 1) && fits(i) && pk28::width_ok(k.slots[i].cols);
+    };
+    std::vector<uint32_t> esc(n, 0);
+    bool any28 = false;
+    for (size_t i = 0; i < n; i++) any28 = any28 || cand28(i);
+    if (e == hipSuccess && any28) {
+        e = hipMemset(d_stats, 0, n * sizeof(uint32_t));
+        for (size_t i = 0; i < n && e == hipSuccess; i++)
+            if (cand28(i)) e = launch_pk28_count(k.slots[i].src, k.slots[i].rows, k.slots[i].cols, (int)stats[3 * i], d_stats + i, nullptr);
+        if (e == hipSuccess) e = hipMemcpy(esc.data(), d_stats, n * sizeof(uint32_t), hipMemcpyDeviceToHost);
+        for (size_t i = 0; i < n; i++)
+            if (cand28(i) && esc[i] <= (uint32_t)pk28::kMaxEsc) bits[i] = 28;
+        for (size_t i = 0; per_layer > 1 && i + per_layer <= n; i += per_layer) {
+            bool all = true;
+            for (int j = 0; j < per_layer; j++) all = all && bits[i + j] == 28;
+            for (int j = 0; j < per_layer && !all; j++) bits[i + j] = 29;
+        }
+    }
     if (d_stats) (void)hipFree(d_stats);
+    const auto stream_dw = [&](size_t i) -> size_t {
+        const auto &m = k.slots[i];
+        if (!fits(i)) return 0;
+        return (size_t)(m.rows / 2) * (bits[i] == 28 ? (size_t)pk28::kPairDw : pk::pair_dw(m.cols / 4));
+    };
     const auto dwords = [&](size_t i) -> size_t {
-        const auto &m = k.slots[i];
-        if (m.rows % 2 || !pk::encodable(stats[3 * i], stats[3 * i + 1], stats[3 * i + 2])) return 0;
-        return (size_t)(m.rows / 2) * pk::pair_dw(m.cols / 4);
+        return stream_dw(i) + (stream_dw(i) && bits[i] == 28 ? (size_t)(k.slots[i].rows / 2) * pk28::kRecDw : 0);
     };
     size_t total = 0;
     for (size_t i = 0; i < n; i++) total += dwords(i);
@@ -275,7 +302,13 @@
     for (size_t i = 0; i < n && e == hipSuccess && k.blob; i++) {
         auto &m = k.slots[i];
         if (dwords(i) == 0) continue;
-        e = launch_pk_pack(m.src, m.rows, m.cols, (int)stats[3 * i], k.blob + off, nullptr);
+        if (bits[i] == 28) {
+            uint32_t *rec = k.blob + off + stream_dw(i);
+            e = launch_pk28_pack(m.src, m.rows, m.cols, (int)stats[3 * i], k.blob + off, rec, nullptr);
+            m.rec = rec;
+        } else {
+            e = launch_pk_pack(m.src, m.rows, m.cols, (int)stats[3 * i], k.blob + off, nullptr);
+        }
         m.p = k.blob + off;
         m.e = (int)stats[3 * i];
         k.packed++;
@@ -286,7 +319,7 @@
         (void)hipGetLastError();
         if (k.blob) (void)hipFree(k.blob);
         k.blob = nullptr;
-        for (auto &m : k.slots) m.p = nullptr;
+        for (auto &m : k.slots) m.p = m.rec = nullptr;
         k.packed = 0;
     }
 }
@@ -513,7 +546,8 @@
     L2Z_HIP(hipSetDevice(w->device));
     float *d = nullptr;
     L2Z_HIP(hipMalloc((void **)&d, count * sizeof(float)));
-    hipError_t e = launch_pk_unpack(pm->p, pm->rows, pm->cols, pm->e, d, nullptr);
+    hipError_t e = pm->rec != nullptr ? launch_pk28_unpack(pm->p, pm->rec, pm->rows, pm->cols, pm->e, d, nullptr)
+                                      : launch_pk_unpack(pm->p, pm->rows, pm->cols, pm->e, d, nullptr);
     if (e == hipSuccess) e = hipMemcpy(out, d, count * sizeof(float), hipMemcpyDeviceToHost);
     (void)hipFree(d);
     L2Z_HIP(e);
@@ -540,6 +574,18 @@
     L2Z_CHECK(kind >= 0 && kind < KIND_COUNT, L2Z_ERR_INVALID, "l2z_weights_packed_count_kind: bad kind %d", kind);
     *n_packed = w->pk[kind].packed;
     *n_candidates = (int)w->pk[kind].slots.size();
+    return L2Z_OK;
+}
+
+extern "C" int l2z_weights_packed_bits_kind(const l2z_weights *w, int kind, int layer, int slot, int *bits)
+{
+    L2Z_CHECK(w != nullptr && bits != nullptr, L2Z_ERR_INVALID, "l2z_weights_packed_bits_kind: null argument");
+    L2Z_CHECK(kind >= 0 && kind < KIND_COUNT, L2Z_ERR_INVALID, "l2z_weights_packed_bits_kind: bad kind %d", kind);
+    const l2z_weights::PkKind &k = w->pk[kind];
+    L2Z_CHECK(layer >= 0 && slot >= 0 && slot < k.per_layer && (size_t)layer * k.per_layer + slot < k.slots.size(), L2Z_ERR_INVALID,
+              "l2z_weights_packed_bits_kind: no slot %d of layer %d of kind %s", slot, layer, kKindNames[kind]);
+    const l2z_weights::PkMat *pm = w->pk_slot(kind, layer, slot);
+    *bits = pm != nullptr ? pm->bits() : 0;
     return L2Z_OK;
 }
 
```

Measured after the change: 245.9 tokens/s (median of 6 runs). +1.6%, better.
